# NDLOHGRP/pyReCoDe

Hardware: AMD Instinct MI355X
Metric: frames/sec + GB/s in, 4096x4096 uint16 @1% sparsity, 1/2/4/8 GPU (higher is better)
Workload: dtype u16; 1 GPU; 4096x4096 uint16, 1.00% sparsity, L1 + LZ4 frame, source_bit_depth 16, batch 64 frames/GPU/step, 256-frame stack/GPU in HBM; parallelism=dp1 (contiguous frame blocks per rank; single process: no collective), gather_every=0, gathers_issued_in_all=0, launch=single process, collective_ranks=1

## Files before the change

pyrecode_amd/csrc/rc_api.hip:

```cpp
#include "rc_host.h"
#include "rc_deflate_model.h"

thread_local std::string g_last_error;
WorkerPool *g_pool = new WorkerPool;
Util g_utils[RC_MAX_DEV];
thread_local Util *t_util = nullptr;


struct rc_ctx {
    int device = 0;
    hipStream_t own_stream = nullptr, stream = nullptr;
    uint32_t nx = 0, ny = 0, depth = 0, level = 0, op_mode = 0, scheme = 0, clevel = 0, max_batch = 0;
    uint32_t emit = rc::EMIT_RAW;
    rc::Scratch sets[2];
    int cur = 0;
    int last = 0;
    const rc::Scratch &geo() const { return sets[0]; }
    const rc::Scratch &recent() const { return sets[last]; }
    DevMem dmem, model_mem[2];
    PinMem hmem;
    hipStream_t pstream = nullptr;
    hipStream_t pstream_b = nullptr;
    hipStream_t last_ps = nullptr;
    bool two_chains = false;
    hipEvent_t ev_red[2] = {}, ev_post[2] = {}, ev_in[2] = {};
    bool post_pending[2] = {false, false};
    bool pipelined = false;
    bool thr_set = false;
    bool keep_bitmap = true;
    uint32_t src_bytes = 2;
    uint32_t *thr32 = nullptr;
    uint32_t last_n = 0;
    DevBuf d_frames, d_out, d_dark;
    uint64_t *d_rec_off = nullptr;
    uint32_t *d_md = nullptr;
    void *d_ztab = nullptr;
    rc::ValueStage values = rc::VALUES_NONE;
    bool values_on = false;
    bool modelled = false, model_ready = false;
    rc::ZstdModel *d_model = nullptr, *h_model = nullptr;
    rc::ZstdSample *d_sample = nullptr, *h_sample = nullptr;
    rc::DeflateModel *d_dzm = nullptr, *h_dzm = nullptr;
    uint32_t *d_dzhist = nullptr, *h_dzhist = nullptr;
    uint32_t l2_sum = 0;
    rc::u32x2 *d_l2_node[2] = {};
    uint16_t *d_l2_base[2] = {};
    rc::BatchStatus *h_status = nullptr;
    rc::BatchStatus *d_first_err = nullptr;
    uint32_t batch_seq = 0;
    const uint8_t *prev_out = nullptr, *prev_rec = nullptr, *prev_md = nullptr;
    uint64_t prev_out_cap = 0;
    uint32_t prev_n = 0;
    hipEvent_t ev[5] = {};
    float stage_ms[5] = {};
    bool profiling = false;
    uint32_t prof_every = 1, prof_phase = 0;
    bool profile_all = getenv("RC_PROFILE_ALL_STAGES") != nullptr;
    struct PipeSlot {
        uint8_t *d_in = nullptr;
        uint8_t *d_out = nullptr;
        uint64_t *d_rec = nullptr, *h_rec = nullptr;
        uint32_t *d_md = nullptr, *h_md = nullptr;
        rc::BatchStatus *h_stat = nullptr;
        hipEvent_t ev_h2d = nullptr, ev_done = nullptr, ev_fetch = nullptr, ev_val = nullptr;
        uint32_t *d_val = nullptr, *h_val = nullptr;
        bool has_val = false;
        uint32_t n = 0;
        bool zero_copy = false;
        enum State { FREE, SUBMITTED, RESULT_TAKEN, FETCHING } state = FREE;
    } pipe[RC_PIPE_SLOTS];
    hipStream_t copy_stream = nullptr, d2h_stream = nullptr;
    uint32_t val_gap = 0, val_x0 = 0, val_y0 = 0, val_w = 0, val_h = 0;
    std::vector<hipEvent_t> prof_ev;
    size_t prof_used = 0;
    double prof_sum_ms[5] = {};
    uint64_t prof_batches = 0;
};

RC_EXPORT int rc_abi_version(void) { return RC_ABI_VERSION; }

RC_EXPORT const char *rc_strerror(int status)
{
    switch (status) {
    case RC_OK: return "ok";
    case RC_ERR_BAD_ARG: return "bad argument";
    case RC_ERR_OUT_TOO_SMALL: return "output buffer too small";
    case RC_ERR_DEVICE: return "GPU / HIP error";
    case RC_ERR_UNSUPPORTED: return "not implemented on device";
    case RC_ERR_RECORD_TOO_LARGE: return "Buffer size smaller than compressed data size";
    case RC_ERR_CORRUPT: return "corrupt input stream";
    case RC_ERR_WORKSPACE: return "out of device memory for the ctx's workspace";
    default: return "unknown status";
    }
}
RC_EXPORT const char *rc_last_error(void) { return g_last_error.c_str(); }

RC_EXPORT int rc_device_count(int *count)
{
    if (!count) return fail(RC_ERR_BAD_ARG, "count is NULL");
    int n = 0;
    if (hipGetDeviceCount(&n) != hipSuccess) {
        (void)hipGetLastError();
        n = 0;
    }
    *count = n;
    return RC_OK;
}
RC_EXPORT int rc_scheme_on_device(uint32_t scheme)
{
    return (scheme == RC_SCHEME_LZ4 || scheme == RC_SCHEME_ZSTD || scheme == RC_SCHEME_BLOSC_LZ4 || scheme == RC_SCHEME_ZLIB_DEVICE) ? 1 : 0;
}

static int alloc_set(rc_ctx *c, rc::Scratch &sc, DevMem &model_mem)
{
    using namespace rc;
    DevMem &m = c->dmem;
    const uint64_t B = c->max_batch, T = sc.ntiles;
    RC_ALLOC(m, sc.bitmap, B * sc.nb_stride + 64);
    RC_ALLOC(m, sc.tile_cnt, B * T * 4);
    RC_ALLOC(m, sc.tile_off, B * T * 4);
    RC_ALLOC(m, sc.tile_next, B * T * 4);
    RC_ALLOC(m, sc.frame_nnz, B * 4);
    RC_ALLOC(m, sc.frame_cbytes, B * 4);
    RC_ALLOC(m, sc.scan_part, B * ((T + 255) / 256) * 32);
    RC_ALLOC(m, sc.status, sizeof(BatchStatus));
    if (c->level != 3) RC_ALLOC(m, sc.pix_slots, B * T * TILE_PX * 2 + 64);
    if (c->emit != EMIT_RAW) {
        if (c->level == 1) {
            sc.comb = c->emit == EMIT_ZSTD ? COMB_AT_BLK_SLOT : COMB_BEHIND_BLOCK;
            sc.blk_stride = 1536;
        }
        RC_ALLOC(m, sc.blk_slots, B * T * (uint64_t)sc.blk_stride + 256);
        RC_ALLOC(m, sc.blk_size, B * T * 4);
        RC_ALLOC(m, sc.blk_off, B * T * 4);
        if (c->emit == EMIT_DEFLATE) {
            RC_ALLOC(m, sc.blk_aux, B * T * 4);
            RC_ALLOC(m, sc.zl_acc, B * 32);
            HIP_TRY(hipMemset(sc.zl_acc, 0, B * 32));
        }
    }
    if (c->values != VALUES_NONE) {
        const ValueGeom g = value_geom(c->values);
        sc.pixraw_stride = ((sc.N * 2 + 15) & ~15ull) + 32;
        sc.nchunk_max = (uint32_t)((sc.N * 2 + g.chunk - 1) / g.chunk) + 1;
        RC_ALLOC(model_mem, sc.pixraw, B * sc.pixraw_stride + 64);
        RC_ALLOC(model_mem, sc.pix_chunks, B * (uint64_t)sc.nchunk_max * g.slot + 64);
        if (c->values == VALUES_DEFLATE_HUFF) RC_ALLOC(model_mem, sc.chunk_aux, B * (uint64_t)(sc.nchunk_max + 1) * 8);
        RC_ALLOC(model_mem, sc.chunk_size, B * (uint64_t)sc.nchunk_max * 4);
        RC_ALLOC(model_mem, sc.chunk_off, B * (uint64_t)sc.nchunk_max * 4);
        RC_ALLOC(model_mem, sc.frame_pbytes, B * 4);
        HIP_TRY(hipMemset(sc.frame_pbytes, 0, B * 4));
    }
    HIP_TRY(hipMemset(sc.frame_nnz, 0, B * 4));
    HIP_TRY(hipMemset(sc.frame_cbytes, 0, B * 4));
    HIP_TRY(hipMemset(sc.status, 0, sizeof(BatchStatus)));
    return RC_OK;
}

static void free_value_stage(rc_ctx *c)
{
    c->values = rc::VALUES_NONE;
    c->values_on = false;
    for (int k = 0; k < 2; ++k) {
        rc::Scratch &set = c->sets[k];
        c->model_mem[k].release_all();
        set.pixraw = nullptr; set.pix_chunks = nullptr; set.chunk_aux = nullptr; set.chunk_size = nullptr; set.chunk_off = nullptr;
        set.frame_pbytes = nullptr; set.pixraw_stride = 0; set.nchunk_max = 0;
    }
}

static int ctx_alloc(rc_ctx *c)
{
    using namespace rc;
    const uint64_t B = c->max_batch;
    RC_ON_DEVICE(c->device);
    HIP_TRY(hipStreamCreateWithFlags(&c->own_stream, hipStreamNonBlocking));
    HIP_TRY(hipStreamCreateWithFlags(&c->pstream, hipStreamNonBlocking));
    {
        int lo = 0, hi = 0;
        HIP_TRY(hipDeviceGetStreamPriorityRange(&lo, &hi));
        HIP_TRY(hipStreamCreateWithPriority(&c->pstream_b, hipStreamNonBlocking, hi));
    }
    c->last_ps = c->pstream;
    c->stream = c->own_stream;
    DevMem &m = c->dmem;
    int r;
    RC_ALLOC(m, c->sets[0].thr, c->geo().N * 2);
    RC_ALLOC(m, c->d_first_err, sizeof(BatchStatus));
    HIP_TRY(hipMemset(c->d_first_err, 0, sizeof(BatchStatus)));
    c->sets[0].first_err = c->d_first_err;
    c->sets[1] = c->sets[0];
    for (int k = 0; k < 2; ++k)
        if ((r = alloc_set(c, c->sets[k], c->model_mem[k])) != RC_OK) return r;
    c->two_chains = false;
    if (c->level == 2) {
        const uint64_t ids = (uint64_t)c->geo().ntiles * rc::TILE_PX;
        RC_ALLOC(m, c->d_l2_node[0], B * ids * 8);
        HIP_TRY(hipMemset(c->d_l2_node[0], 0, B * ids * 8));
        RC_ALLOC(m, c->d_l2_base[0], B * (uint64_t)c->geo().ntiles * 64 * 2);
        for (int i = 0; i < 2; ++i) {
            Scratch &set = c->sets[i];
            set.l2_node = c->d_l2_node[0]; set.l2_ids_per_frame = ids; set.l2_base = c->d_l2_base[0];
        }
    }
    if (c->emit == EMIT_ZSTD) {
        if ((r = zstd_encoder_tables(m, c->d_ztab)) != RC_OK) return r;
        c->modelled = c->clevel != 0;
        if (c->modelled) {
            RC_ALLOC(m, c->d_model, sizeof(ZstdModel));
            RC_ALLOC(m, c->d_sample, sizeof(ZstdSample));
            RC_ALLOC(c->hmem, c->h_model, sizeof(ZstdModel));
            RC_ALLOC(c->hmem, c->h_sample, sizeof(ZstdSample));
        }
    }
    if (c->values == VALUES_DEFLATE_HUFF) {
        RC_ALLOC(m, c->d_dzm, sizeof(DeflateModel));
        RC_ALLOC(m, c->d_dzhist, 256 * 4);
        RC_ALLOC(c->hmem, c->h_dzm, sizeof(DeflateModel));
        RC_ALLOC(c->hmem, c->h_dzhist, 256 * 4);
    }
    RC_ALLOC(m, c->d_rec_off, (B + 1) * 8);
    RC_ALLOC(m, c->d_md, B * 3 * 4);
    RC_ALLOC(c->hmem, c->h_status, 2 * sizeof(BatchStatus));
    for (auto &e : c->ev) HIP_TRY(hipEventCreate(&e));
    for (auto &e : c->ev_red) HIP_TRY(hipEventCreateWithFlags(&e, hipEventDisableTiming));
    for (auto &e : c->ev_post) HIP_TRY(hipEventCreateWithFlags(&e, hipEventDisableTiming));
    for (auto &e : c->ev_in) HIP_TRY(hipEventCreateWithFlags(&e, hipEventDisableTiming));
    return RC_OK;
}

RC_EXPORT rc_ctx *rc_ctx_create(uint32_t nx, uint32_t ny, uint32_t src_bit_depth, uint32_t reduction_level,
                                uint32_t op_mode, uint32_t scheme, uint32_t clevel, int device_id, uint32_t max_batch,
                                int *status)
{
    int dummy;
    if (!status) status = &dummy;
    *status = RC_OK;
    if (nx == 0 || ny == 0 || max_batch == 0 || max_batch > 65535u || op_mode > 1) {
        *status = fail(RC_ERR_BAD_ARG, "nx, ny, max_batch must be > 0, max_batch <= 65535 and op_mode 0 or 1");
        return nullptr;
    }
    if ((uint64_t)nx * ny >= (1ull << 32)) {
        *status = fail(RC_ERR_BAD_ARG, "nx*ny must be < 2^32");
        return nullptr;
    }
    if ((uint64_t)nx * ny * 2 >= (1ull << 32)) {
        *status = fail(RC_ERR_UNSUPPORTED, "a raw frame of 4 GiB or more (nx*ny*bytes_per_pixel >= 2^32) does not fit the format's u32 size fields");
        return nullptr;
    }
    if (reduction_level < 1 || reduction_level > 3) {
        *status = fail(RC_ERR_UNSUPPORTED, "reduction_level 4 (centroiding) is not implemented on device");
        return nullptr;
    }
    if (reduction_level == 2 && nx > 65535u) {
        *status = fail(RC_ERR_UNSUPPORTED, "reduction_level 2 needs nx <= 65535");
        return nullptr;
    }
    if (src_bit_depth < 1 || src_bit_depth > 32) {
        *status = fail(RC_ERR_UNSUPPORTED, "source_bit_depth must be 1..32 (uint8 / uint16 / uint32 source frames)");
        return nullptr;
    }
    int ndev = 0;
    if (hipGetDeviceCount(&ndev) != hipSuccess || device_id < 0 || device_id >= ndev) {
        (void)hipGetLastError();
        *status = fail(RC_ERR_DEVICE, "no such HIP device (this library has no CPU path)");
        return nullptr;
    }
    rc_ctx *c = new (std::nothrow) rc_ctx();
    if (!c) {
        *status = fail(RC_ERR_DEVICE, "out of host memory");
        return nullptr;
    }
    c->device = device_id;
    c->nx = nx; c->ny = ny; c->depth = src_bit_depth; c->level = reduction_level; c->op_mode = op_mode;
    c->scheme = scheme; c->clevel = clevel; c->max_batch = max_batch;
    c->emit = (op_mode == 1 && rc_scheme_on_device(scheme)) ? scheme : rc::EMIT_RAW;
    c->values = rc::value_stage_of(c->emit, clevel, reduction_level);
    rc::Scratch &sc = c->sets[0];
    sc.N = (uint64_t)nx * ny;
    sc.ntiles = (uint32_t)((sc.N + rc::TILE_PX - 1) / rc::TILE_PX);
    sc.nb = (sc.N + 7) / 8;
    sc.nb_stride = (uint64_t)sc.ntiles * rc::TILE_BM;
    sc.max_batch = max_batch;
    sc.guarded_loads = getenv("RC_REDUCE_GUARDED_LOADS") != nullptr;
    int rcode = ctx_alloc(c);
    if (rcode != RC_OK) {
        *status = rcode;
        std::string keep = g_last_error;
        rc_ctx_destroy(c);
        g_last_error = keep;
        return nullptr;
    }
    return c;
}

RC_EXPORT int rc_ctx_destroy(rc_ctx *c)
{
    if (!c) return RC_OK;
    DeviceGuard dev_guard_;
    (void)dev_guard_.enter(c->device);
    for (hipStream_t st : {c->stream, c->pstream, c->pstream_b, c->own_stream, c->copy_stream, c->d2h_stream})
        if (st) (void)hipStreamSynchronize(st);
    c->dmem.release_all();
    for (DevMem &m : c->model_mem) m.release_all();
    c->hmem.release_all();
    for (auto &p : c->pipe)
        for (hipEvent_t e : {p.ev_h2d, p.ev_done, p.ev_fetch, p.ev_val})
            if (e) (void)hipEventDestroy(e);
    for (hipEvent_t e : {c->ev_red[0], c->ev_red[1], c->ev_post[0], c->ev_post[1], c->ev_in[0], c->ev_in[1]})
        if (e) (void)hipEventDestroy(e);
    for (auto &e : c->ev)
        if (e) (void)hipEventDestroy(e);
    for (auto &e : c->prof_ev) (void)hipEventDestroy(e);
    for (hipStream_t st : {c->copy_stream, c->d2h_stream, c->pstream, c->pstream_b, c->own_stream})
        if (st) (void)hipStreamDestroy(st);
    delete c;
    return RC_OK;
}

RC_EXPORT int rc_ctx_set_stream(rc_ctx *c, void *hip_stream)
{
    if (!c) return fail(RC_ERR_BAD_ARG, "ctx is NULL");
    c->stream = hip_stream ? reinterpret_cast<hipStream_t>(hip_stream) : c->own_stream;
    return RC_OK;
}

RC_EXPORT int rc_set_threshold(rc_ctx *c, const void *thr)
{
    if (!c || !thr) return fail(RC_ERR_BAD_ARG, "ctx / thr is NULL");
    if (c->depth > 16 && c->src_bytes != 4) return fail(RC_ERR_BAD_ARG, "src_bit_depth > 16 means uint32 sources: rc_ctx_set_source_bytes(ctx, 4) first");
    RC_ON_DEVICE(c->device);
    HIP_TRY(hipMemcpyAsync(c->src_bytes == 4 ? (void *)c->thr32 : (void *)c->geo().thr, thr, c->geo().N * (c->src_bytes == 4 ? 4 : 2),
                           is_device_ptr(thr) ? hipMemcpyDeviceToDevice : hipMemcpyHostToDevice,
                           c->stream));
    HIP_TRY(hipStreamSynchronize(c->stream));
    c->thr_set = true;
    return RC_OK;
}

RC_EXPORT int rc_set_dark(rc_ctx *c, const void *dark, int64_t epsilon)
{
    if (!c || !dark) return fail(RC_ERR_BAD_ARG, "ctx / dark is NULL");
    RC_ON_DEVICE(c->device);
    const void *src = dark;
    const uint64_t bytes = c->geo().N * c->src_bytes;
    if (!is_device_ptr(dark)) {
        int r = c->d_dark.ensure(c->dmem, bytes);
        if (r != RC_OK) return r;
        HIP_TRY(hipMemcpyAsync(c->d_dark.p, dark, bytes, hipMemcpyHostToDevice, c->stream));
        src = c->d_dark.p;
    }
    if (c->depth > 16 && c->src_bytes != 4) return fail(RC_ERR_BAD_ARG, "src_bit_depth > 16 means uint32 sources: rc_ctx_set_source_bytes(ctx, 4) first");
    if (c->src_bytes == 4) rc::launch_threshold32(static_cast<const uint32_t *>(src), epsilon, c->geo().N, c->thr32, c->stream);
    else rc::launch_threshold(src, epsilon, c->geo().N, c->geo().thr, c->stream, c->src_bytes);
    HIP_TRY(hipGetLastError());
    HIP_TRY(hipStreamSynchronize(c->stream));
    c->thr_set = true;
    return RC_OK;
}

RC_EXPORT int rc_ctx_set_source_bytes(rc_ctx *c, uint32_t bytes_per_pixel)
{
    if (!c) return fail(RC_ERR_BAD_ARG, "ctx is NULL");
    if (bytes_per_pixel != 1 && bytes_per_pixel != 2 && bytes_per_pixel != 4) return fail(RC_ERR_BAD_ARG, "rc_ctx_set_source_bytes: 1 (uint8), 2 (uint16) or 4 (uint32)");
    if (bytes_per_pixel == 1 && c->depth > 8) return fail(RC_ERR_BAD_ARG, "rc_ctx_set_source_bytes: uint8 sources need src_bit_depth <= 8");
    if (bytes_per_pixel == 2 && c->depth > 16) return fail(RC_ERR_BAD_ARG, "rc_ctx_set_source_bytes: uint16 sources need src_bit_depth <= 16");
    if (c->batch_seq || c->thr_set) return fail(RC_ERR_BAD_ARG, "rc_ctx_set_source_bytes: call before rc_set_dark / rc_set_threshold and the first batch");
    if (c->geo().N * bytes_per_pixel >= (1ull << 32))
        return fail(RC_ERR_UNSUPPORTED, "rc_ctx_set_source_bytes: a raw frame of 4 GiB or more (nx*ny*bytes_per_pixel >= 2^32) does not fit the format's u32 size fields");
    if (bytes_per_pixel == 4) {
        if (c->depth <= 16) return fail(RC_ERR_BAD_ARG, "rc_ctx_set_source_bytes: uint32 sources are what source_bit_depth > 16 means (misc.py:41-49)");
        if (c->level == 2) return fail(RC_ERR_UNSUPPORTED, "rc_ctx_set_source_bytes: reduction level 2 is not implemented for uint32 sources");
        if (c->emit == rc::EMIT_DEFLATE) return fail(RC_ERR_UNSUPPORTED, "rc_ctx_set_source_bytes: the device DEFLATE encoder is not implemented for uint32 sources (use RC_SCHEME_ZLIB: the host's zlib)");
        RC_ON_DEVICE(c->device);
        uint32_t *thr32 = nullptr;
        uint16_t *slots[2] = {nullptr, nullptr};
        bool ok = c->dmem.try_alloc(thr32, c->geo().N * 4) == hipSuccess;
        for (int k = 0; ok && k < 2 && c->level != 3; ++k)
            ok = c->dmem.try_alloc(slots[k], (uint64_t)c->max_batch * c->geo().ntiles * rc::TILE_PX * 4 + 64) == hipSuccess;
        if (!ok) {
            (void)hipGetLastError();
            c->dmem.free_one(thr32);
            for (uint16_t *&p : slots) c->dmem.free_one(p);
            return fail(RC_ERR_DEVICE, "rc_ctx_set_source_bytes: out of device memory for the uint32 threshold / residual slots");
        }
        if (c->depth % 8 == 0) c->depth = 32;
        c->modelled = false;
        free_value_stage(c);
        c->thr32 = thr32;
        for (int k = 0; k < 2; ++k) {
            rc::Scratch *set = &c->sets[k];
            set->pix_slot_bytes = rc::TILE_PX * 4;
            set->comb = rc::COMB_OFF;
            if (c->level != 3) {
                c->dmem.free_one(set->pix_slots);
                set->pix_slots = slots[k];
            }
        }
    }
    c->src_bytes = bytes_per_pixel;
    return RC_OK;
}
RC_EXPORT uint32_t rc_ctx_source_bytes(const rc_ctx *c) { return c ? c->src_bytes : 0; }

RC_EXPORT uint64_t rc_out_capacity(const rc_ctx *c, uint32_t n) { return c ? (uint64_t)n * c->geo().N * c->src_bytes : 0; }

RC_EXPORT uint32_t rc_md_fields(const rc_ctx *c)
{
    if (!c) return 0;
    const bool comp = c->emit != rc::EMIT_RAW;
    if (c->level != 3) return comp ? 3 : 1;
    return comp ? 1 : 0;
}

static int fit_value_model(rc_ctx *c, const void *frames_dev, uint32_t n)
{
    using namespace rc;
    const bool dz = c->values == VALUES_DEFLATE_HUFF;
    hipStream_t s = c->stream;
    const Scratch &sc = c->sets[c->cur];
    const uint32_t ns = n < 2 ? n : 2;
    void *d_sample = dz ? (void *)c->d_dzhist : c->d_sample, *h_sample = dz ? (void *)c->h_dzhist : c->h_sample;
    void *d_model = dz ? (void *)c->d_dzm : c->d_model, *h_model = dz ? (void *)c->h_dzm : c->h_model;
    const size_t sample_bytes = dz ? 256 * 4 : sizeof(ZstdSample), model_bytes = dz ? sizeof(DeflateModel) : sizeof(ZstdModel);
    for (int k = 0; k < 2; ++k)
        if (c->post_pending[k]) HIP_TRY(hipStreamWaitEvent(s, c->ev_post[k], 0));
    HIP_TRY(hipMemsetAsync(d_sample, 0, sample_bytes, s));
    if (dz) {
        launch_reduce(sc, frames_dev, ns, 1u, CODEC_DEFLATE, true, c->depth, s, nullptr, c->src_bytes);
        launch_scans(sc, ns, true, true, s);
        RecordParams rp;
        rp.level = 1u; rp.emit = c->emit; rp.depth = c->depth; rp.first_frame_id = 0; rp.packed_slots = 1u;
        rp.frame_bytes = c->geo().N * c->src_bytes;
        rp.pix_mode = PIX_MODE_FLAT;
        launch_assemble(sc, rp, ns, nullptr, nullptr, c->batch_seq, s);
        launch_pd_hist(sc, ns, c->depth, c->d_dzhist, s);
    } else {
        launch_reduce(sc, frames_dev, ns, c->level == 3 ? 3u : 1u, CODEC_ZSTD_FAST, true, c->depth, s, nullptr, c->src_bytes);
        launch_zstd_sample(sc, ns, c->level == 1, c->depth, c->d_sample, s);
    }
    HIP_TRY(hipGetLastError());
    HIP_TRY(hipMemcpyAsync(h_sample, d_sample, sample_bytes, hipMemcpyDeviceToHost, s));
    HIP_TRY(hipStreamSynchronize(s));
    if (dz) {
        dm_build_model(c->h_dzhist, c->h_dzm);
        c->values_on = c->h_dzm->usable != 0;
    } else {
        zstd_model_from_sample(c->h_sample, c->h_model, c->clevel == 1 ? 50u : (c->clevel == 2 ? 20u : 0u));
        if (c->values == VALUES_NONE || !zm_code_pays(c->h_sample->pix, c->h_model->pix_code)) c->h_model->valid &= ~ZM_PIX_CODE;
        c->values_on = (c->h_model->valid & ZM_PIX_CODE) != 0;
    }
    HIP_TRY(hipMemcpyAsync(d_model, h_model, model_bytes, hipMemcpyHostToDevice, s));
    HIP_TRY(hipStreamSynchronize(s));
    for (Scratch &set : c->sets) {
        if (dz) { set.dz_model = c->d_dzm; continue; }
        const ZstdModel &M = *c->h_model;
        set.zm_model = c->d_model;
        set.zm_lit_code = c->d_model->lit_code;
        set.zm_valid = M.valid;
        set.zm_budget = zm_block_budget(M, BLK_SLOT);
        set.zm_seq_bits = (M.valid & ZM_SEQ_TABLES) ? M.seq.ll_log + M.seq.ml_log : 12u;
    }
    c->model_ready = true;
    return RC_OK;
}

static uint32_t fused_codec(uint32_t emit, uint32_t clevel, bool modelled, uint32_t src_bytes)
{
    using namespace rc;
    switch (emit) {
    case EMIT_ZSTD: return modelled && src_bytes != 4 ? CODEC_ZSTD_MODELLED : CODEC_ZSTD_FAST;
    case EMIT_LZ4: return clevel != 0 ? CODEC_LZ4_EVENTS : CODEC_LZ4_RUNS;
    case EMIT_BLOSC: return CODEC_BLOSC;
    case EMIT_DEFLATE: return CODEC_DEFLATE;
    default: return CODEC_NONE;
    }
}

static int enqueue_batch(rc_ctx *c, const void *frames_dev, uint32_t n, uint32_t first_frame_id, uint8_t *out_dev,
                         uint64_t out_cap, uint64_t *rec_off_dev, uint32_t *md_dev, bool timed)
{
    using namespace rc;
    hipStream_t s = c->stream;
    if ((c->modelled || c->values == VALUES_DEFLATE_HUFF) && !c->model_ready) {
        int r = fit_value_model(c, frames_dev, n);
        if (r != RC_OK) return r;
    }
    RecordParams rp;
    rp.level = c->level == 3 ? 3u : 1u;
    rp.emit = c->emit; rp.depth = c->depth; rp.first_frame_id = first_frame_id;
    rp.packed_slots = 1u;
    rp.frame_bytes = c->geo().N * c->src_bytes;
    hipEvent_t *ev = nullptr;
    if (timed) ev = c->ev;
    else if (c->profiling && (c->prof_phase++ % c->prof_every) == 0) {
        if (c->prof_used + 5 > c->prof_ev.size()) {
            for (int i = 0; i < 5; ++i) {
                hipEvent_t e;
                HIP_TRY(hipEventCreate(&e));
                c->prof_ev.push_back(e);
            }
        }
        ev = c->prof_ev.data() + c->prof_used;
        c->prof_used += 5;
    }
    const int k = c->cur;
    c->cur ^= 1;
    c->last = k;
    const rc::Scratch &sc = c->sets[k];
    const bool two = c->pipelined && c->two_chains;
    hipStream_t ps = two && k == 1 ? c->pstream_b : c->pstream;
    c->last_ps = ps;
    if (c->post_pending[k]) HIP_TRY(hipStreamWaitEvent(s, c->ev_post[k], 0));
    if (ev) HIP_TRY(hipEventRecord(ev[0], s));
    const bool fitted_seq = c->modelled && (c->h_model->valid & ZM_SEQ_TABLES);
    hipStream_t tail = nullptr;
    if (sc.N % TILE_PX) {
        HIP_TRY(hipEventRecord(c->ev_in[k], s));
        HIP_TRY(hipStreamWaitEvent(ps, c->ev_in[k], 0));
        tail = ps;
    }
    const uint32_t codec = fused_codec(c->emit, c->clevel, c->modelled, c->src_bytes);
    const bool keep_maps = c->keep_bitmap || c->emit == EMIT_RAW;
    if (c->src_bytes == 4)
        launch_reduce32(sc, static_cast<const uint32_t *>(frames_dev), c->thr32, n, c->level, c->depth, s, codec, keep_maps);
    else
        launch_reduce(sc, frames_dev, n, c->level, codec, keep_maps, c->depth, s, tail, c->src_bytes);
    const bool all_ev = ev && (timed || c->profile_all);
    hipEvent_t red = ev ? ev[1] : c->ev_red[k];
    HIP_TRY(hipEventRecord(red, s));
    HIP_TRY(hipStreamWaitEvent(ps, red, 0));
    if (c->level == 2) launch_l2(sc, n, c->nx, c->l2_sum, c->depth, ps);
    const bool lits_only = c->modelled && (c->h_model->valid & ZM_LITS_ONLY);
    if (c->emit == EMIT_ZSTD && !lits_only) launch_zstd_fse(sc, n, fitted_seq ? (const void *)&c->d_model->seq : c->d_ztab, fitted_seq, ps);
    if (all_ev) HIP_TRY(hipEventRecord(ev[2], ps));
    launch_scans(sc, n, c->level != 3, c->emit != EMIT_RAW, ps);
    if (all_ev) HIP_TRY(hipEventRecord(ev[3], ps));
    if (c->values_on) {
        rp.pix_mode = PIX_MODE_FLAT;
        launch_assemble(sc, rp, n, out_dev, rec_off_dev, c->batch_seq, ps);
        launch_values_encode(c->values, sc, n, c->depth, ps);
        launch_values_scan(c->values, sc, n, c->depth, ps);
        rp.pix_mode = PIX_MODE_SKIP;
    }
    if (two && c->post_pending[k ^ 1]) {
        auto overlap = [](const uint8_t *a, uint64_t an, const uint8_t *b, uint64_t bn) { return a && b && a < b + bn && b < a + an; };
        const uint8_t *rec8 = reinterpret_cast<const uint8_t *>(rec_off_dev), *md8 = reinterpret_cast<const uint8_t *>(md_dev);
        if (overlap(out_dev, out_cap, c->prev_out, c->prev_out_cap) || overlap(rec8, (uint64_t)(n + 1) * 8, c->prev_rec, (uint64_t)(c->prev_n + 1) * 8) ||
            overlap(md8, (uint64_t)n * 12, c->prev_md, (uint64_t)c->prev_n * 12))
            HIP_TRY(hipStreamWaitEvent(ps, c->ev_post[k ^ 1], 0));
    }
    c->prev_out = out_dev; c->prev_out_cap = out_cap; c->prev_n = n;
    c->prev_rec = reinterpret_cast<const uint8_t *>(rec_off_dev); c->prev_md = reinterpret_cast<const uint8_t *>(md_dev);
    launch_layout(sc, rp, n, out_cap, rec_off_dev, md_dev, ps);
    launch_assemble(sc, rp, n, out_dev, rec_off_dev, c->batch_seq, ps);
    ++c->batch_seq;
    if (c->values_on) launch_values_gather(c->values, sc, n, c->depth, 16, out_dev, rec_off_dev, ps);
    if (ev) HIP_TRY(hipEventRecord(ev[4], ps));
    if (two && c->post_pending[k ^ 1]) HIP_TRY(hipStreamWaitEvent(ps, c->ev_post[k ^ 1], 0));
    HIP_TRY(hipEventRecord(c->ev_post[k], ps));
    c->post_pending[k] = true;
    if (!c->pipelined) HIP_TRY(hipStreamWaitEvent(s, c->ev_post[k], 0));
    HIP_TRY(hipGetLastError());
    c->last_n = n;
    return RC_OK;
}

static int check_batch_args(rc_ctx *c, const void *frames, uint32_t n, const void *out, const void *rec, const void *md)
{
    if (!c || !frames || !out || !rec || !md) return fail(RC_ERR_BAD_ARG, "NULL argument");
    if (n == 0 || n > c->max_batch) return fail(RC_ERR_BAD_ARG, "n must be in 1..max_batch");
    if (!c->thr_set) return fail(RC_ERR_BAD_ARG, "threshold not set (rc_set_threshold / rc_set_dark)");
    return RC_OK;
}

RC_EXPORT int rc_reduce_compress_batch_async(rc_ctx *c, const void *frames_dev, uint32_t n, uint32_t first_frame_id,
                                             uint8_t *out_dev, uint64_t out_cap, uint64_t *rec_offsets_dev, uint32_t *md_dev)
{
    int r = check_batch_args(c, frames_dev, n, out_dev, rec_offsets_dev, md_dev);
    if (r != RC_OK) return r;
    RC_ON_DEVICE(c->device);
    return enqueue_batch(c, frames_dev, n, first_frame_id, out_dev, out_cap, rec_offsets_dev, md_dev, false);
}

static void l2_second_chain(rc_ctx *c)
{
    if (c->level != 2 || c->two_chains) return;
    const uint64_t B = c->max_batch, ids = (uint64_t)c->geo().ntiles * rc::TILE_PX;
    if (!c->d_l2_node[1]) {
        bool ok = c->dmem.try_alloc(c->d_l2_node[1], B * ids * 8) == hipSuccess && hipMemset(c->d_l2_node[1], 0, B * ids * 8) == hipSuccess &&
                  c->dmem.try_alloc(c->d_l2_base[1], B * (uint64_t)c->geo().ntiles * 64 * 2) == hipSuccess && hipDeviceSynchronize() == hipSuccess;
        if (!ok) {
            (void)hipGetLastError();
            c->dmem.free_one(c->d_l2_node[1]);
            c->dmem.free_one(c->d_l2_base[1]);
            return;
        }
    }
    c->sets[1].l2_node = c->d_l2_node[1];
    c->sets[1].l2_base = c->d_l2_base[1];
    c->two_chains = true;
}

RC_EXPORT int rc_ctx_set_pipelined(rc_ctx *c, int on)
{
    if (!c) return fail(RC_ERR_BAD_ARG, "ctx is NULL");
    RC_ON_DEVICE(c->device);
    HIP_TRY(hipStreamSynchronize(c->pstream));
    HIP_TRY(hipStreamSynchronize(c->pstream_b));
    if (on) l2_second_chain(c);
    c->pipelined = on != 0;
    return RC_OK;
}
RC_EXPORT int rc_ctx_wait_results(rc_ctx *c, void *hip_stream)
{
    if (!c) return fail(RC_ERR_BAD_ARG, "ctx is NULL");
    RC_ON_DEVICE(c->device);
    if (c->post_pending[c->last])
        HIP_TRY(hipStreamWaitEvent(hip_stream ? reinterpret_cast<hipStream_t>(hip_stream) : c->stream, c->ev_post[c->last], 0));
    return RC_OK;
}

RC_EXPORT int rc_ctx_sync(rc_ctx *c)
{
    if (!c) return fail(RC_ERR_BAD_ARG, "ctx is NULL");
    RC_ON_DEVICE(c->device);
    HIP_TRY(hipStreamSynchronize(c->pstream_b));
    HIP_TRY(hipMemcpyAsync(&c->h_status[0], c->recent().status, sizeof(rc::BatchStatus), hipMemcpyDeviceToHost, c->pstream));
    HIP_TRY(hipMemcpyAsync(&c->h_status[1], c->d_first_err, sizeof(rc::BatchStatus), hipMemcpyDeviceToHost, c->pstream));
    HIP_TRY(hipMemsetAsync(c->d_first_err, 0, sizeof(rc::BatchStatus), c->pstream));
    HIP_TRY(hipStreamSynchronize(c->pstream));
    HIP_TRY(hipStreamSynchronize(c->stream));
    const uint32_t n_batches = c->batch_seq;
    c->batch_seq = 0;
    for (size_t b = 0; b + 5 <= c->prof_used; b += 5) {
        float ms;
        if (!c->profile_all) {
            if (hipEventElapsedTime(&ms, c->prof_ev[b], c->prof_ev[b + 1]) == hipSuccess) c->prof_sum_ms[0] += ms;
        } else
        for (int i = 0; i < 4; ++i)
            if (hipEventElapsedTime(&ms, c->prof_ev[b + i], c->prof_ev[b + i + 1]) == hipSuccess) c->prof_sum_ms[i] += ms;
        if (hipEventElapsedTime(&ms, c->prof_ev[b], c->prof_ev[b + 4]) == hipSuccess) c->prof_sum_ms[4] += ms;
        ++c->prof_batches;
    }
    c->prof_used = 0;
    if (c->h_status[1].total != 0) c->h_status[1] = rc::first_err_decode(c->h_status[1].total);
    if (c->h_status[1].code != 0) {
        char msg[160];
        if (n_batches > 1)
            snprintf(msg, sizeof msg, "%s (frame %u of batch %llu of the %u enqueued since the last sync)", rc_strerror(c->h_status[1].code),
                     c->h_status[1].frame, (unsigned long long)c->h_status[1].total, n_batches);
        else
            snprintf(msg, sizeof msg, "%s (frame %u of the batch)", rc_strerror(c->h_status[1].code), c->h_status[1].frame);
        return fail(c->h_status[1].code, msg);
    }
    return RC_OK;
}

RC_EXPORT int rc_reduce_compress_batch(rc_ctx *c, const void *frames, uint32_t n, uint32_t first_frame_id, uint8_t *out,
                                       uint64_t out_cap, uint64_t *rec_offsets, uint32_t *md)
{
    int r = check_batch_args(c, frames, n, out, rec_offsets, md);
    if (r != RC_OK) return r;
    RC_ON_DEVICE(c->device);
    const uint64_t frame_bytes = c->geo().N * c->src_bytes;
    const void *fdev = frames;
    if (!is_device_ptr(frames)) {
        r = c->d_frames.ensure(c->dmem, (uint64_t)n * frame_bytes);
        if (r != RC_OK) return r;
        HIP_TRY(hipMemcpyAsync(c->d_frames.p, frames, (uint64_t)n * frame_bytes, hipMemcpyHostToDevice, c->stream));
        fdev = c->d_frames.p;
    }
    uint8_t *odev = out;
    uint64_t cap = out_cap;
    const bool out_host = !is_device_ptr(out);
    if (out_host) {
        const uint64_t worst = (uint64_t)n * frame_bytes;
        cap = out_cap < worst ? out_cap : worst;
        r = c->d_out.ensure(c->dmem, cap);
        if (r != RC_OK) return r;
        odev = c->d_out.p;
    }
    r = enqueue_batch(c, fdev, n, first_frame_id, odev, cap, c->d_rec_off, c->d_md, true);
    if (r != RC_OK) return r;
    r = rc_ctx_sync(c);
    for (int i = 0; i < 4; ++i) (void)hipEventElapsedTime(&c->stage_ms[i], c->ev[i], c->ev[i + 1]);
    (void)hipEventElapsedTime(&c->stage_ms[4], c->ev[0], c->ev[4]);
    if (r != RC_OK) return r;
    int r2 = copy_out(rec_offsets, c->d_rec_off, (uint64_t)(n + 1) * 8, c->stream);
    if (r2 == RC_OK) r2 = copy_out(md, c->d_md, (uint64_t)n * 12, c->stream);
    if (r2 == RC_OK && out_host) r2 = copy_out(out, c->d_out.p, c->h_status->total, c->stream);
    if (r2 != RC_OK) return r2;
    HIP_TRY(hipStreamSynchronize(c->stream));
    return RC_OK;
}

RC_EXPORT void *rc_host_alloc(uint64_t bytes)
{
    void *p = nullptr;
    if (hipHostMalloc(&p, bytes ? bytes : 16, hipHostMallocDefault) != hipSuccess) {
        (void)hipGetLastError();
        fail(RC_ERR_DEVICE, "hipHostMalloc failed");
        return nullptr;
    }
    return p;
}
RC_EXPORT int rc_host_free(void *p)
{
    if (p) HIP_TRY(hipHostFree(p));
    return RC_OK;
}
RC_EXPORT int rc_host_register(void *p, uint64_t bytes)
{
    if (!p || !bytes) return fail(RC_ERR_BAD_ARG, "NULL / zero argument");
    HIP_TRY(hipHostRegister(p, bytes, hipHostRegisterDefault));
    return RC_OK;
}
RC_EXPORT int rc_host_unregister(void *p)
{
    if (p) HIP_TRY(hipHostUnregister(p));
    return RC_OK;
}

static int pipe_slot_init(rc_ctx *c, rc_ctx::PipeSlot &p)
{
    const uint64_t B = c->max_batch;
    if (!c->copy_stream) HIP_TRY(hipStreamCreateWithFlags(&c->copy_stream, hipStreamNonBlocking));
    if (!c->d2h_stream) HIP_TRY(hipStreamCreateWithFlags(&c->d2h_stream, hipStreamNonBlocking));
    RC_ALLOC(c->dmem, p.d_in, B * c->geo().N * c->src_bytes + 64);
    RC_ALLOC(c->dmem, p.d_out, rc_out_capacity(c, (uint32_t)B) + 64);
    RC_ALLOC(c->dmem, p.d_rec, (B + 1) * 8);
    RC_ALLOC(c->dmem, p.d_md, B * 12);
    RC_ALLOC(c->hmem, p.h_rec, (B + 1) * 8);
    RC_ALLOC(c->hmem, p.h_md, B * 12);
    RC_ALLOC(c->hmem, p.h_stat, sizeof(rc::BatchStatus));
    HIP_TRY(hipEventCreateWithFlags(&p.ev_h2d, hipEventDisableTiming));
    HIP_TRY(hipEventCreateWithFlags(&p.ev_done, hipEventDisableTiming));
    HIP_TRY(hipEventCreateWithFlags(&p.ev_fetch, hipEventDisableTiming));
    HIP_TRY(hipEventCreateWithFlags(&p.ev_val, hipEventDisableTiming));
    RC_ALLOC(c->dmem, p.d_val, B * 4 + 64);
    RC_ALLOC(c->hmem, p.h_val, B * 4 + 64);
    return RC_OK;
}

RC_EXPORT int rc_ctx_set_validation(rc_ctx *c, uint32_t gap, uint32_t x0, uint32_t y0, uint32_t w, uint32_t h)
{
    if (!c) return fail(RC_ERR_BAD_ARG, "ctx is NULL");
    if (gap && (w == 0 || h == 0 || w > 128 || h > 128 || (uint64_t)x0 + w > c->nx || (uint64_t)y0 + h > c->ny))
        return fail(RC_ERR_BAD_ARG, "rc_ctx_set_validation: the region must lie inside the frame and hold at most 128 x 128 pixels");
    c->val_gap = gap; c->val_x0 = x0; c->val_y0 = y0; c->val_w = w; c->val_h = h;
    return RC_OK;
}

RC_EXPORT int rc_pipe_validation(rc_ctx *c, uint32_t slot, uint32_t *counts)
{
    if (!c || slot >= RC_PIPE_SLOTS || !counts) return fail(RC_ERR_BAD_ARG, "NULL argument / slot out of range");
    rc_ctx::PipeSlot &p = c->pipe[slot];
    if (p.state != p.SUBMITTED && p.state != p.RESULT_TAKEN) return fail(RC_ERR_BAD_ARG, "nothing submitted on this slot");
    if (!p.has_val) { for (uint32_t i = 0; i < p.n; ++i) counts[i] = 0xFFFFFFFFu; return RC_OK; }
    HIP_TRY(hipEventSynchronize(p.ev_val));
    memcpy(counts, p.h_val, (uint64_t)p.n * 4);
    return RC_OK;
}

RC_EXPORT int rc_pipe_submit(rc_ctx *c, uint32_t slot, const void *frames_host, uint32_t n, uint32_t first_frame_id)
{
    if (!c || !frames_host || slot >= RC_PIPE_SLOTS) return fail(RC_ERR_BAD_ARG, "NULL argument / slot out of range");
    if (n == 0 || n > c->max_batch) return fail(RC_ERR_BAD_ARG, "n must be in 1..max_batch");
    if (!c->thr_set) return fail(RC_ERR_BAD_ARG, "threshold not set (rc_set_threshold / rc_set_dark)");
    RC_ON_DEVICE(c->device);
    rc_ctx::PipeSlot &p = c->pipe[slot];
    if (p.state != p.FREE) return fail(RC_ERR_BAD_ARG, "slot is still in use (result / fetch_wait not called)");
    if (!p.d_in) {
        int r = pipe_slot_init(c, p);
        if (r != RC_OK) return r;
    }
    if (!c->pipelined) {
        HIP_TRY(hipStreamSynchronize(c->pstream));
        HIP_TRY(hipStreamSynchronize(c->pstream_b));
        l2_second_chain(c);
        c->pipelined = true;
    }
    const void *fdev = nullptr;
    hipPointerAttribute_t a;
    if (hipPointerGetAttributes(&a, frames_host) == hipSuccess) {
        if (a.type == hipMemoryTypeHost && a.devicePointer) fdev = a.devicePointer;
    } else (void)hipGetLastError();
    p.zero_copy = fdev != nullptr;
    if (!fdev) {
        HIP_TRY(hipMemcpyAsync(p.d_in, frames_host, (uint64_t)n * c->geo().N * c->src_bytes, hipMemcpyHostToDevice, c->copy_stream));
        HIP_TRY(hipEventRecord(p.ev_h2d, c->copy_stream));
        HIP_TRY(hipStreamWaitEvent(c->stream, p.ev_h2d, 0));
        fdev = p.d_in;
    }
    int r = enqueue_batch(c, fdev, n, first_frame_id, p.d_out, rc_out_capacity(c, c->max_batch), p.d_rec, p.d_md, false);
    if (r != RC_OK) return r;
    p.has_val = c->val_gap != 0;
    if (p.has_val) {
        rc::launch_roi_components(fdev, c->src_bytes == 4 ? (const void *)c->thr32 : (const void *)c->geo().thr, c->geo().N, c->nx, n, first_frame_id, c->val_gap, c->val_x0, c->val_y0, c->val_w, c->val_h, p.d_val, c->stream, c->src_bytes);
        HIP_TRY(hipGetLastError());
        HIP_TRY(hipMemcpyAsync(p.h_val, p.d_val, (uint64_t)n * 4, hipMemcpyDeviceToHost, c->stream));
        HIP_TRY(hipEventRecord(p.ev_val, c->stream));
    }
    if (p.zero_copy) HIP_TRY(hipEventRecord(p.ev_h2d, c->stream));
    hipStream_t ps = c->last_ps;
    HIP_TRY(hipMemcpyAsync(p.h_rec, p.d_rec, (uint64_t)(n + 1) * 8, hipMemcpyDeviceToHost, ps));
    HIP_TRY(hipMemcpyAsync(p.h_md, p.d_md, (uint64_t)n * 12, hipMemcpyDeviceToHost, ps));
    HIP_TRY(hipMemcpyAsync(p.h_stat, c->recent().status, sizeof(rc::BatchStatus), hipMemcpyDeviceToHost, ps));
    HIP_TRY(hipEventRecord(p.ev_done, ps));
    p.n = n;
    p.state = p.SUBMITTED;
    return RC_OK;
}

RC_EXPORT int rc_pipe_input_done(rc_ctx *c, uint32_t slot)
{
    if (!c || slot >= RC_PIPE_SLOTS) return fail(RC_ERR_BAD_ARG, "NULL argument / slot out of range");
    if (c->pipe[slot].state == rc_ctx::PipeSlot::FREE) return RC_OK;
    HIP_TRY(hipEventSynchronize(c->pipe[slot].ev_h2d));
    return RC_OK;
}

RC_EXPORT int rc_pipe_result(rc_ctx *c, uint32_t slot, uint64_t *rec_offsets, uint32_t *md, uint64_t *total)
{
    if (!c || slot >= RC_PIPE_SLOTS || !rec_offsets || !md || !total) return fail(RC_ERR_BAD_ARG, "NULL argument / slot out of range");
    rc_ctx::PipeSlot &p = c->pipe[slot];
    if (p.state != p.SUBMITTED) return fail(RC_ERR_BAD_ARG, "nothing submitted on this slot");
    HIP_TRY(hipEventSynchronize(p.ev_done));
    p.state = p.RESULT_TAKEN;
    if (p.h_stat->code != 0) {
        char msg[128];
        snprintf(msg, sizeof msg, "%s (frame %u of the batch)", rc_strerror(p.h_stat->code), p.h_stat->frame);
        p.state = p.FREE;
        return fail(p.h_stat->code, msg);
    }
    memcpy(rec_offsets, p.h_rec, (uint64_t)(p.n + 1) * 8);
    memcpy(md, p.h_md, (uint64_t)p.n * 12);
    *total = p.h_stat->total;
    return RC_OK;
}

RC_EXPORT int rc_pipe_fetch(rc_ctx *c, uint32_t slot, uint8_t *dst_host, uint64_t bytes)
{
    if (!c || slot >= RC_PIPE_SLOTS || (!dst_host && bytes)) return fail(RC_ERR_BAD_ARG, "NULL argument / slot out of range");
    rc_ctx::PipeSlot &p = c->pipe[slot];
    if (p.state != p.RESULT_TAKEN) return fail(RC_ERR_BAD_ARG, "rc_pipe_result has not been called for this slot");
    if (bytes > p.h_stat->total) return fail(RC_ERR_BAD_ARG, "more bytes than the batch's records hold");
    RC_ON_DEVICE(c->device);
    if (bytes) HIP_TRY(hipMemcpyAsync(dst_host, p.d_out, bytes, hipMemcpyDeviceToHost, c->d2h_stream));
    HIP_TRY(hipEventRecord(p.ev_fetch, c->d2h_stream));
    p.state = p.FETCHING;
    return RC_OK;
}

RC_EXPORT int rc_pipe_fetch_wait(rc_ctx *c, uint32_t slot)
{
    if (!c || slot >= RC_PIPE_SLOTS) return fail(RC_ERR_BAD_ARG, "NULL argument / slot out of range");
    rc_ctx::PipeSlot &p = c->pipe[slot];
    if (p.state == p.RESULT_TAKEN) { p.state = p.FREE; return RC_OK; }
    if (p.state != p.FETCHING) return fail(RC_ERR_BAD_ARG, "rc_pipe_fetch has not been called for this slot");
    HIP_TRY(hipEventSynchronize(p.ev_fetch));
    p.state = p.FREE;
    return RC_OK;
}

RC_EXPORT int rc_ctx_refit_model(rc_ctx *c)
{
    if (!c) return fail(RC_ERR_BAD_ARG, "ctx is NULL");
    c->model_ready = false;
    return RC_OK;
}

RC_EXPORT int rc_get_binary_map(rc_ctx *c, uint32_t i, uint8_t *bitmap_out)
{
    if (!c || !bitmap_out) return fail(RC_ERR_BAD_ARG, "NULL argument");
    if (i >= c->last_n) return fail(RC_ERR_BAD_ARG, "frame index outside the most recent batch");
    if (!c->keep_bitmap && c->emit != rc::EMIT_RAW && c->level != 2) return fail(RC_ERR_BAD_ARG, "binary maps are not kept (rc_ctx_keep_binary_maps(ctx, 0))");
    RC_ON_DEVICE(c->device);
    int r = copy_out(bitmap_out, c->recent().bitmap + (uint64_t)i * c->geo().nb_stride, c->geo().nb, c->stream);
    if (r != RC_OK) return r;
    HIP_TRY(hipStreamSynchronize(c->stream));
    return RC_OK;
}

RC_EXPORT int rc_ctx_set_profiling(rc_ctx *c, int on)
{
    if (!c) return fail(RC_ERR_BAD_ARG, "ctx is NULL");
    c->profiling = on != 0;
    c->prof_every = on > 1 ? (uint32_t)on : 1u;
    c->prof_phase = 0;
    for (double &v : c->prof_sum_ms) v = 0;
    c->prof_batches = 0;
    return RC_OK;
}
RC_EXPORT int rc_ctx_get_profile(rc_ctx *c, double sum_ms[5], uint64_t *batches)
{
    if (!c || !sum_ms || !batches) return fail(RC_ERR_BAD_ARG, "NULL argument");
    memcpy(sum_ms, c->prof_sum_ms, sizeof c->prof_sum_ms);
    *batches = c->prof_batches;
    return RC_OK;
}

RC_EXPORT int rc_ctx_set_l2_statistics(rc_ctx *c, uint32_t l2_statistics)
{
    if (!c || l2_statistics > 2) return fail(RC_ERR_BAD_ARG, "l2_statistics must be 0, 1 (max) or 2 (sum)");
    c->l2_sum = l2_statistics == 2 ? 1u : 0u;
    return RC_OK;
}

RC_EXPORT int rc_ctx_keep_binary_maps(rc_ctx *c, int on)
{
    if (!c) return fail(RC_ERR_BAD_ARG, "ctx is NULL");
    c->keep_bitmap = on != 0;
    return RC_OK;
}

RC_EXPORT int rc_get_stage_ms(rc_ctx *c, float ms[5])
{
    if (!c || !ms) return fail(RC_ERR_BAD_ARG, "NULL argument");
    memcpy(ms, c->stage_ms, sizeof c->stage_ms);
    return RC_OK;
}

RC_EXPORT int64_t rc_unpack_frame_sparse(uint32_t nx, uint32_t ny, uint32_t bit_depth, const uint8_t *bitmap,
                                         const uint8_t *pixvals, uint64_t pixvals_bytes, uint64_t *out,
                                         uint64_t out_cap_triplets, uint32_t reduction_level)
{
    if (!bitmap || nx == 0 || ny == 0 || (!out && out_cap_triplets)) return fail(RC_ERR_BAD_ARG, "NULL / zero argument");
    if (reduction_level == 1 && (bit_depth == 0 || bit_depth > 64)) return fail(RC_ERR_BAD_ARG, "bit_depth must be 1..64");
    if (reduction_level == 1 && !pixvals && pixvals_bytes) return fail(RC_ERR_BAD_ARG, "pixvals is NULL");
    UtilScope util_scope;
    int r = util_scope.enter();
    if (r != RC_OK) return r;
    Util &u = g_util;
    const uint64_t N = (uint64_t)nx * ny, nb = (N + 7) / 8, nb8 = (nb + 7) / 8;
    const uint32_t nblk = (uint32_t)((nb8 + rc::WG - 1) / rc::WG);
    const uint8_t *d_bm = nullptr, *d_px = nullptr;
    r = stage_in(bitmap, nb, u.a, d_bm, nb8 * 8 - nb + 8);
    if (r != RC_OK) return r;
    if (reduction_level == 1 && pixvals_bytes) {
        r = stage_in(pixvals, pixvals_bytes, u.b, d_px);
        if (r != RC_OK) return r;
    }
    r = u.w.ensure(u.dmem, (uint64_t)nblk * 8 + 16);
    if (r != RC_OK) return r;
    uint32_t *blk_cnt = u.w.as<uint32_t>(), *blk_off = blk_cnt + nblk;
    uint64_t *nnz_dev = reinterpret_cast<uint64_t *>(blk_cnt + 2 * (uint64_t)nblk);
    rc::launch_expand_count(d_bm, nb8, N, blk_cnt, blk_off, nnz_dev, u.stream);
    HIP_TRY(hipMemcpyAsync(u.h_scalar, nnz_dev, 8, hipMemcpyDeviceToHost, u.stream));
    HIP_TRY(hipStreamSynchronize(u.stream));
    const uint64_t nnz = *u.h_scalar;
    if (!out) return (int64_t)nnz;
    if (nnz > out_cap_triplets) return fail(RC_ERR_OUT_TOO_SMALL, "out holds fewer triplets than the bitmap has set bits");
    if (reduction_level == 1 && (nnz * bit_depth + 7) / 8 > pixvals_bytes)
        return fail(RC_ERR_CORRUPT, "pixvals shorter than popcount(bitmap) * bit_depth bits");
    if (nnz == 0) return 0;
    StagedOut so;
    if ((r = so.begin(out, nnz * 24)) != RC_OK) return r;
    rc::launch_expand_emit(d_bm, nb8, N, nx, blk_off, d_px, pixvals_bytes, bit_depth, reduction_level, nnz, so.as<uint64_t>(), u.stream);
    HIP_TRY(hipGetLastError());
    if ((r = so.finish(out, nnz * 24)) != RC_OK) return r;
    return (int64_t)nnz;
}

RC_EXPORT int rc_bit_pack(const uint16_t *pixvals, uint64_t n, uint32_t bit_depth, uint8_t *out, uint64_t out_n)
{
    if (!out || (!pixvals && n)) return fail(RC_ERR_BAD_ARG, "NULL argument");
    if (bit_depth == 0 || bit_depth > 32) return fail(RC_ERR_BAD_ARG, "bit_depth must be 1..32");
    if (out_n != (n * bit_depth + 7) / 8) return fail(RC_ERR_BAD_ARG, "out_n must be ceil(n*bit_depth/8)");
    if (out_n == 0) return RC_OK;
    UtilScope util_scope;
    int r = util_scope.enter();
    if (r != RC_OK) return r;
    Util &u = g_util;
    const uint16_t *d_in = nullptr;
    r = stage_in(pixvals, n * 2, u.a, d_in);
    if (r != RC_OK) return r;
    StagedOut so;
    if ((r = so.begin(out, out_n)) != RC_OK) return r;
    rc::launch_bit_pack(d_in, n, bit_depth, so.as<uint8_t>(), out_n, u.stream);
    HIP_TRY(hipGetLastError());
    return so.finish(out, out_n);
}

RC_EXPORT int rc_bit_unpack(const uint8_t *packed, uint64_t packed_bytes, uint64_t n, uint32_t bit_depth, uint64_t *out)
{
    if (!out || (!packed && packed_bytes)) return fail(RC_ERR_BAD_ARG, "NULL argument");
    if (bit_depth == 0 || bit_depth > 64) return fail(RC_ERR_BAD_ARG, "bit_depth must be 1..64");
    if ((n * bit_depth + 7) / 8 > packed_bytes) return fail(RC_ERR_CORRUPT, "packed shorter than n * bit_depth bits");
    if (n == 0) return RC_OK;
    UtilScope util_scope;
    int r = util_scope.enter();
    if (r != RC_OK) return r;
    Util &u = g_util;
    const uint8_t *d_in = nullptr;
    r = stage_in(packed, packed_bytes, u.a, d_in);
    if (r != RC_OK) return r;
    StagedOut so;
    if ((r = so.begin(out, n * 8)) != RC_OK) return r;
    rc::launch_bit_unpack(d_in, packed_bytes, n, bit_depth, so.as<uint64_t>(), u.stream);
    HIP_TRY(hipGetLastError());
    return so.finish(out, n * 8);
}

RC_EXPORT int rc_synth_dark(int device_id, uint32_t seed, uint64_t n_pixels, uint16_t *dark_dev)
{
    if (!dark_dev) return fail(RC_ERR_BAD_ARG, "NULL argument");
    RC_ON_DEVICE(device_id);
    rc::launch_synth_dark(seed, n_pixels, dark_dev, nullptr);
    HIP_TRY(hipGetLastError());
    HIP_TRY(hipDeviceSynchronize());
    return RC_OK;
}
RC_EXPORT int rc_synth_frames_clustered(int device_id, uint32_t seed, uint32_t first_frame, uint32_t n_frames, uint32_t nx, uint32_t ny,
                                        uint32_t seed_ppm, const uint16_t *dark_dev, uint16_t *frames_dev)
{
    if (!dark_dev || !frames_dev || n_frames == 0 || nx == 0 || ny == 0) return fail(RC_ERR_BAD_ARG, "NULL / zero argument");
    if ((uint64_t)nx * ny > 0xFFFFFFFFull) return fail(RC_ERR_BAD_ARG, "rc_synth_frames_clustered: nx * ny must fit 32 bits");
    RC_ON_DEVICE(device_id);
    rc::launch_synth_frames_clustered(seed, first_frame, n_frames, nx, ny, seed_ppm, dark_dev, frames_dev, nullptr);
    HIP_TRY(hipGetLastError());
    HIP_TRY(hipDeviceSynchronize());
    return RC_OK;
}
RC_EXPORT int rc_synth_frames(int device_id, uint32_t seed, uint32_t first_frame, uint32_t n_frames, uint64_t n_pixels,
                              uint32_t sparsity_ppm, const uint16_t *dark_dev, uint16_t *frames_dev)
{
    if (!dark_dev || !frames_dev || n_frames == 0) return fail(RC_ERR_BAD_ARG, "NULL / zero argument");
    RC_ON_DEVICE(device_id);
    rc::launch_synth_frames(seed, first_frame, n_frames, n_pixels, sparsity_ppm, dark_dev, frames_dev, nullptr);
    HIP_TRY(hipGetLastError());
    HIP_TRY(hipDeviceSynchronize());
    return RC_OK;
}
```

pyrecode_amd/csrc/rc_gather.hip:

```cpp
#include <cstdlib>

#include "rc_launch.h"
#include "rc_record.h"
#include "rc_deflate_block.h"

namespace rc {

struct GatherArgs {
    const uint8_t *blk_slots, *bitmap;
    const uint16_t *pix_slots;
    const uint32_t *blk_size, *blk_off, *tile_cnt, *tile_off, *tile_next, *frame_nnz, *frame_cbytes, *frame_pbytes;
    const uint32_t *blk_aux;
    uint32_t *zl_acc;
    uint8_t *pixraw;
    BatchStatus *status, *first_err;
    uint64_t nb, nb_stride, pixraw_stride;
    uint32_t ntiles, blk_stride, pix_slot_bytes, comb;
};

typedef u32x4 u32x4_u __attribute__((aligned(1)));
typedef u32x2 u32x2_u __attribute__((aligned(1)));
typedef uint32_t u32_u __attribute__((aligned(1)));
typedef uint16_t u16_u __attribute__((aligned(1)));

__device__ __forceinline__ uint32_t lane_get(uint32_t v, uint32_t src_lane)
{
    return (uint32_t)__builtin_amdgcn_ds_bpermute((int)(4u * src_lane), (int)v);
}

template <bool BITS>
__device__ __forceinline__ u32x4 shift_piece(const u32x4 &x, uint32_t e, uint32_t sh)
{
    u32x4 y = x;
    if (BITS) {
        y[0] = __builtin_amdgcn_alignbit(x[1], x[0], sh); y[1] = __builtin_amdgcn_alignbit(x[2], x[1], sh);
        y[2] = __builtin_amdgcn_alignbit(x[3], x[2], sh); y[3] = __builtin_amdgcn_alignbit(e, x[3], sh);
    }
    return y;
}
__device__ __forceinline__ void put_piece(uint8_t *p, const u32x4 &y, uint32_t valid)
{
    if (valid >= 16) { *reinterpret_cast<u32x4_u *>(p) = y; return; }
    uint32_t a0 = y[0], a1 = y[1];
    if (valid & 8u) { *reinterpret_cast<u32x2_u *>(p) = u32x2{a0, a1}; p += 8; a0 = y[2]; a1 = y[3]; }
    if (valid & 4u) { *reinterpret_cast<u32_u *>(p) = a0; p += 4; a0 = a1; }
    if (valid & 2u) { *reinterpret_cast<u16_u *>(p) = (uint16_t)a0; p += 2; a0 >>= 16; }
    if (valid & 1u) *p = (uint8_t)a0;
}

struct AdlerAcc { uint32_t A, W; };
__device__ __forceinline__ void adler_piece(AdlerAcc &acc, const u32x4 &y, uint32_t valid, uint32_t sp)
{
    uint32_t a = 0, q = 0;
#pragma unroll
    for (int k = 0; k < 4; ++k) {
        const uint32_t nb = valid > 4u * k ? min(valid - 4u * k, 4u) : 0u;
        const uint32_t v = y[k] & (nb >= 4u ? 0xFFFFFFFFu : ((1u << (8u * nb)) - 1u));
        a = __builtin_amdgcn_sad_u8(v, 0u, a);
        q = __builtin_amdgcn_udot4(v, 0x03020100u + 0x04040404u * (uint32_t)k, q, false);
    }
    acc.A += a;
    acc.W = (acc.W + (sp % ADLER_P) * a + q) % ADLER_P;
}
__device__ __forceinline__ void adler_byte(AdlerAcc &acc, uint32_t byte, uint32_t sp)
{
    acc.A += byte;
    acc.W = (acc.W + (sp % ADLER_P) * byte) % ADLER_P;
}

struct ResidGeom { uint32_t b_lo, n, ps0, avail; };
__device__ __forceinline__ ResidGeom resid_geom(uint32_t coff, uint32_t cnt, uint32_t d)
{
    const uint64_t dbit = (uint64_t)coff * d;
    const uint32_t nbits = cnt * d;
    const uint64_t b_lo = (dbit + 7) >> 3, b_hi = (dbit + nbits + 7) >> 3;
    ResidGeom g{(uint32_t)b_lo, (uint32_t)(b_hi - b_lo), (uint32_t)(8 * b_lo - dbit), (uint32_t)((dbit + nbits) & 7u)};
    if (g.avail && g.n) --g.n;
    else g.avail = 0;
    return g;
}

constexpr int GATHER_U = 4, GATHER_UB = 3;
constexpr int GATHER_WPE = 8;
template <bool BITS, int U, bool ADLER>
__global__ __launch_bounds__(64) __attribute__((amdgpu_waves_per_eu(GATHER_WPE))) void k_gather(GatherArgs sc, RecordParams rp, uint8_t *__restrict__ out, const uint64_t *__restrict__ rec_off,
                                               uint32_t lz4f_hdr_bitmap, uint32_t lz4f_hdr_pix, uint32_t batch_seq, uint32_t gpf, uint32_t nitems, uint32_t tpi)
{
    if (sc.status->code != 0) {
        if (blockIdx.x == 0 && threadIdx.x == 0 && sc.first_err)
            atomicMax(reinterpret_cast<unsigned long long *>(&sc.first_err->total), first_err_key(batch_seq, sc.status->code, sc.status->frame));
        return;
    }
    const uint32_t lane = (uint32_t)lane_id();
    const bool flat = rp.pix_mode == PIX_MODE_FLAT, skip_pix = rp.pix_mode == PIX_MODE_SKIP;
    const bool pixp = rp.level == 1 && rp.packed_slots && !skip_pix;
    const bool plain_pos = rp.emit == EMIT_RAW || flat;
    const uint32_t d = rp.depth;
    const FrameFmt ff = frame_fmt(rp.emit);
    const uint32_t bhdr = bitmap_hdr(ff, rp.emit, sc.ntiles);
    const uint8_t *pix_base = reinterpret_cast<const uint8_t *>(sc.pix_slots);
    for (uint32_t item = blockIdx.x; item < nitems; item += gridDim.x) {
        const uint32_t f = item / gpf, g = item - f * gpf, t0 = tpi * g, t = t0 + lane;
        const bool have = lane < tpi && t < sc.ntiles;
        const uint64_t frow = (uint64_t)f * sc.ntiles;
        uint8_t *rec = flat ? sc.pixraw + (uint64_t)f * sc.pixraw_stride : out + rec_off[f];
        const uint32_t nnz = rp.level == 1 ? sc.frame_nnz[f] : 0;
        const uint32_t npk = rp.level == 1 ? packed_bytes(nnz, d) : 0;
        uint64_t bitmap_pos = 0, pix_pos = 0;
        uint32_t cb = 0;
        if (!flat) {
            if (rp.emit == EMIT_RAW) { bitmap_pos = rp.level == 1 ? 8 : 4; pix_pos = bitmap_pos + sc.nb; }
            else { cb = bhdr + sc.frame_cbytes[f] + ff.end; bitmap_pos = rp.level == 1 ? 16 : 8; pix_pos = bitmap_pos + cb; }
        }
        if (g == 0 && lane == 0 && !flat) record_fixed_fields(sc, rp, f, rec, bitmap_pos, pix_pos, cb, npk, ff, skip_pix, lz4f_hdr_bitmap, lz4f_hdr_pix);
        uint8_t *pdst = rec + pix_pos;

        uint32_t word = 0, bsz = 0, bdst = 0, cnt = 0, rn = 0, rdst = 0, rs = 0xFFFFFFFFu, ps0 = 0, flags = 0, blo = 0;
        AdlerAcc ad{0u, 0u};
        if (have && rp.emit != EMIT_RAW && (!flat || (sc.comb == COMB_BEHIND_BLOCK && pixp))) word = sc.blk_size[frow + t];
        if (have && !flat) {
            if (rp.emit == EMIT_RAW) {
                const uint64_t b0 = (uint64_t)t * TILE_BM;
                bsz = (uint32_t)min((uint64_t)TILE_BM, sc.nb - b0);
                bdst = (uint32_t)(bitmap_pos + b0);
            } else {
                bsz = word;
                const uint32_t boff = bhdr + sc.blk_off[frow + t];
                bdst = (uint32_t)bitmap_pos + boff;
                if (rp.emit == EMIT_BLOSC) store_u32_le(rec + bitmap_pos + 16 + 4 * (uint64_t)t, boff);
            }
        }
        if (have && pixp) {
            cnt = sc.tile_cnt[frow + t];
            if (cnt) {
                const ResidGeom q = resid_geom(sc.tile_off[frow + t], cnt, d);
                ps0 = q.ps0;
                if (ADLER) blo = q.b_lo;
                if (sc.comb) {
                    const uint32_t ro16 = sc.comb == COMB_AT_BLK_SLOT ? (uint32_t)BLK_SLOT / 16 : (word + 15) >> 4, r16 = (cnt * d + 127) >> 7;
                    if (16 * (ro16 + r16) <= sc.blk_stride) rs = 16 * ro16;
                }
                if (q.n && !plain_pos && ((uint64_t)q.b_lo >> ff.chunk_shift) != (((uint64_t)q.b_lo + q.n - 1) >> ff.chunk_shift)) flags = 1u << 31;
                else rn = q.n;
                rdst = (uint32_t)(pix_pos + (plain_pos ? (uint64_t)q.b_lo : stored_pos(ff, q.b_lo)));
            }
        }
        uint32_t ext_cnt = 0, ext_first = 0;
        if (BITS && pixp && t0 + tpi < sc.ntiles) {
            ext_cnt = sc.tile_cnt[frow + t0 + tpi];
            if (ext_cnt)
                ext_first = *reinterpret_cast<const uint32_t *>(residual_src(sc, frow + t0 + tpi, sc.comb == COMB_BEHIND_BLOCK ? sc.blk_size[frow + t0 + tpi] : 0u, ext_cnt, d));
        }
        const uint8_t *slot = rp.emit == EMIT_RAW ? sc.bitmap + (uint64_t)f * sc.nb_stride + (uint64_t)t0 * TILE_BM : sc.blk_slots + (frow + t0) * sc.blk_stride;
        const uint32_t slot_stride = rp.emit == EMIT_RAW ? (uint32_t)TILE_BM : sc.blk_stride;
        const uint8_t *rslot = pix_base + (frow + t0) * sc.pix_slot_bytes;

        const uint32_t nb16 = (bsz + 15) >> 4, tot = nb16 + ((rn + 15) >> 4);
        const uint32_t incl = wave_incl_scan(tot), cum = incl - tot, T = wave_last(incl);
        const uint32_t packed = bsz | (ps0 << 10) | (rn << 13) | flags;
        for (uint32_t i0 = 0; 64u * i0 < T; i0 += U) {
            u32x4 x[U];
            uint32_t e[U], dsto[U], meta[U];
            uint32_t spos[ADLER ? U : 1];
#pragma unroll
            for (int u = 0; u < U; ++u) {
                const uint32_t P = 64u * (i0 + u) + lane;
                uint32_t k = 0;
#pragma unroll
                for (uint32_t step = 32; step; step >>= 1) {
                    const uint32_t c = lane_get(cum, k + step);
                    if (c <= P) k += step;
                }
                const uint32_t ck = lane_get(cum, k), pk = lane_get(packed, k), bd = lane_get(bdst, k), rd = lane_get(rdst, k), rsk = lane_get(rs, k);
                const uint32_t blk = ADLER ? lane_get(blo, k) : 0u;
                const uint32_t bsz_k = pk & 1023u, ps0_k = (pk >> 10) & 7u, rn_k = (pk >> 13) & 0x7FFFu;
                const uint32_t idx = P - ck, nbk = (bsz_k + 15) >> 4;
                const bool isb = idx < nbk;
                const uint32_t j = isb ? idx : idx - nbk;
                const uint32_t left = (isb ? bsz_k : rn_k) - 16u * j;
                const bool act = P < T;
                const uint8_t *src = isb ? slot + (uint64_t)k * slot_stride + 16u * j
                                         : (rsk == 0xFFFFFFFFu ? rslot + (uint64_t)k * sc.pix_slot_bytes : slot + (uint64_t)k * slot_stride + rsk) + 16u * j;
                dsto[u] = (isb ? bd : rd) + 16u * j;
                meta[u] = act ? (min(left, 16u) | ((isb ? 0u : ps0_k) << 8)) : 0u;
                if (ADLER) spos[u] = isb ? 0xFFFFFFFFu : blk + 16u * j;
                x[u] = u32x4{0u, 0u, 0u, 0u};
                e[u] = 0;
                if (act) {
                    x[u] = *reinterpret_cast<const u32x4 *>(src);
                    if (BITS && !isb && ps0_k) e[u] = *reinterpret_cast<const uint32_t *>(src + 16);
                }
            }
#pragma unroll
            for (int u = 0; u < U; ++u)
                if (meta[u] & 0xFFu) {
                    const u32x4 y = shift_piece<BITS>(x[u], e[u], meta[u] >> 8);
                    put_piece(rec + dsto[u], y, meta[u] & 0xFFu);
                    if (ADLER && spos[u] != 0xFFFFFFFFu) adler_piece(ad, y, meta[u] & 0xFFu, spos[u]);
                }
        }
        if (pixp) {
        ResidGeom q{0u, 0u, 0u, 0u};
        if (cnt) q = resid_geom(sc.tile_off[frow + t], cnt, d);
        for (uint64_t m = __builtin_amdgcn_ballot_w64((packed >> 31) != 0); m; m &= m - 1) {
            const uint32_t k = (uint32_t)__builtin_ctzll(m);
            const uint32_t n = lane_get(q.n, k), p0 = lane_get(q.ps0, k), b0 = lane_get(q.b_lo, k), rsk = lane_get(rs, k);
            const uint32_t *s32 = reinterpret_cast<const uint32_t *>(rsk == 0xFFFFFFFFu ? rslot + (uint64_t)k * sc.pix_slot_bytes : slot + (uint64_t)k * slot_stride + rsk);
            for (uint32_t i = lane; i < n; i += 64) {
                const uint32_t qb = 8 * i + p0;
                const uint32_t v = __builtin_amdgcn_alignbit(s32[(qb >> 5) + 1], s32[qb >> 5], qb & 31u) & 0xFFu;
                pdst[stored_pos(ff, (uint64_t)b0 + i)] = (uint8_t)v;
                if (ADLER) adler_byte(ad, v, b0 + i);
            }
        }
        if (BITS) {

        const uint32_t fin_avail = q.avail, fin_q = 8 * q.n + q.ps0, fin_b = q.b_lo + q.n;
        const uint8_t *psrc = rs == 0xFFFFFFFFu ? rslot + (uint64_t)lane * sc.pix_slot_bytes : slot + (uint64_t)lane * slot_stride + rs;
        const uint32_t first = cnt ? *reinterpret_cast<const uint32_t *>(psrc) : 0u;
        uint32_t byte = 0, got = 8;
        if (fin_avail) {
            byte = (*reinterpret_cast<const u32_u *>(psrc + (fin_q >> 3)) >> (fin_q & 7u)) & ((1u << fin_avail) - 1u);
            got = fin_avail;
        }
        const uint64_t nonempty = __builtin_amdgcn_ballot_w64(cnt != 0);
        uint32_t cur = lane;
        while (__builtin_amdgcn_ballot_w64(got < 8 && cur < 64) != 0) {
            const uint64_t higher = cur >= 63 ? 0ull : nonempty & (~0ull << (cur + 1));
            const uint32_t nxt = higher ? (uint32_t)__builtin_ctzll(higher) : 64u;
            const uint32_t cc = lane_get(cnt, nxt & 63u), fd = lane_get(first, nxt & 63u);
            if (got < 8 && cur < 64) {
                const bool in = nxt < 64;
                const uint32_t c2 = in ? cc : ext_cnt, f2 = in ? fd : ext_first;
                if (in || c2) {
                    const uint32_t take = min(8u - got, c2 * d);
                    byte |= (f2 & ((1u << take) - 1u)) << got;
                    got += take;
                    cur = nxt;
                } else cur = 65;
            }
        }
        if (got < 8) {
            uint32_t tt = cur == 65 ? (t0 + tpi - 1 < sc.ntiles ? sc.tile_next[frow + t0 + tpi - 1] : sc.ntiles) : (t0 + tpi < sc.ntiles ? sc.tile_next[frow + t0 + tpi] : sc.ntiles);
            while (tt < sc.ntiles) {
                const uint32_t cc = sc.tile_cnt[frow + tt];
                const uint32_t fd = *reinterpret_cast<const uint32_t *>(residual_src(sc, frow + tt, sc.comb == COMB_BEHIND_BLOCK ? sc.blk_size[frow + tt] : 0u, cc, d));
                const uint32_t take = min(8u - got, cc * d);
                byte |= (fd & ((1u << take) - 1u)) << got;
                got += take;
                if (got >= 8) break;
                tt = sc.tile_next[frow + tt];
            }
        }
        if (fin_avail) {
            pdst[plain_pos ? (uint64_t)fin_b : stored_pos(ff, fin_b)] = (uint8_t)byte;
            if (ADLER) adler_byte(ad, byte & 0xFFu, fin_b);
        }
        }
        }
        if (ADLER && !flat) {
            const uint32_t aux = have ? sc.blk_aux[frow + t] : 0u;
            const uint32_t tA0 = wave_last(wave_incl_scan(aux & 0xFFFFu)), tW0 = wave_last(wave_incl_scan(aux >> 16));
            const uint32_t tA1 = wave_last(wave_incl_scan(ad.A % ADLER_P)), tW1 = wave_last(wave_incl_scan(ad.W));
            if (lane == 0) {
                uint32_t *acc = sc.zl_acc + 8 * (uint64_t)f;
                if (tA0 | tW0) {
                    __hip_atomic_fetch_add(&acc[0], tA0 % ADLER_P, __ATOMIC_RELAXED, __HIP_MEMORY_SCOPE_AGENT);
                    __hip_atomic_fetch_add(&acc[1], tW0 % ADLER_P, __ATOMIC_RELAXED, __HIP_MEMORY_SCOPE_AGENT);
                }
                if (tA1 | tW1) {
                    __hip_atomic_fetch_add(&acc[2], tA1 % ADLER_P, __ATOMIC_RELAXED, __HIP_MEMORY_SCOPE_AGENT);
                    __hip_atomic_fetch_add(&acc[3], tW1 % ADLER_P, __ATOMIC_RELAXED, __HIP_MEMORY_SCOPE_AGENT);
                }
            }
        }
    }
}

__global__ __launch_bounds__(64) void k_zlib_finish(GatherArgs sc, RecordParams rp, uint8_t *__restrict__ out, const uint64_t *__restrict__ rec_off, uint32_t B)
{
    const uint32_t f = blockIdx.x * 64 + threadIdx.x;
    if (f >= B || sc.status->code != 0) return;
    const FrameFmt ff = frame_fmt(rp.emit);
    const uint32_t *acc = sc.zl_acc + 8 * (uint64_t)f;
    uint8_t *rec = out + rec_off[f];
    const uint32_t cb = bitmap_hdr(ff, rp.emit, sc.ntiles) + sc.frame_cbytes[f] + ff.end, bitmap_pos = rp.level == 1 ? 16u : 8u;
    store_u32_be(rec + bitmap_pos + cb - 4, adler_from_sums(sc.nb, acc[0], acc[1]));
    if (rp.level == 1 && rp.pix_mode != PIX_MODE_SKIP) {
        const uint32_t npk = packed_bytes(sc.frame_nnz[f], rp.depth);
        store_u32_be(rec + bitmap_pos + cb + stored_size(ff, npk) - 4, adler_from_sums(npk, acc[2], acc[3]));
    }
}


void launch_gather(const Scratch &sc, const RecordParams &rp, uint32_t B, uint8_t *out, const uint64_t *rec_off, uint32_t hdr_bitmap, uint32_t hdr_pix,
                   uint32_t batch_seq, hipStream_t s)
{
    uint32_t tpi = 64;
    while (tpi > 8 && (uint64_t)B * ((sc.ntiles + tpi - 1) / tpi) < 1024) tpi >>= 1;
    const uint32_t gpf = (sc.ntiles + tpi - 1) / tpi, nitems = gpf * B, wgs = nitems;
    const GatherArgs ga{sc.blk_slots, sc.bitmap, sc.pix_slots, sc.blk_size, sc.blk_off, sc.tile_cnt, sc.tile_off, sc.tile_next, sc.frame_nnz, sc.frame_cbytes,
                        sc.frame_pbytes, sc.blk_aux, sc.zl_acc, sc.pixraw, sc.status, sc.first_err, sc.nb, sc.nb_stride, sc.pixraw_stride, sc.ntiles, sc.blk_stride, sc.pix_slot_bytes, sc.comb};
    const bool bits = rp.level == 1 && rp.depth % 8 != 0;
    if (rp.emit == EMIT_DEFLATE) {
        if (bits) hipLaunchKernelGGL((k_gather<true, GATHER_UB - 1, true>), dim3(wgs), dim3(64), 0, s, ga, rp, out, rec_off, hdr_bitmap, hdr_pix, batch_seq, gpf, nitems, tpi);
        else hipLaunchKernelGGL((k_gather<false, GATHER_U, true>), dim3(wgs), dim3(64), 0, s, ga, rp, out, rec_off, hdr_bitmap, hdr_pix, batch_seq, gpf, nitems, tpi);
        if (rp.pix_mode != PIX_MODE_FLAT) hipLaunchKernelGGL(k_zlib_finish, dim3((B + 63) / 64), dim3(64), 0, s, ga, rp, out, rec_off, B);
    } else if (bits)
        hipLaunchKernelGGL((k_gather<true, GATHER_UB, false>), dim3(wgs), dim3(64), 0, s, ga, rp, out, rec_off, hdr_bitmap, hdr_pix, batch_seq, gpf, nitems, tpi);
    else
        hipLaunchKernelGGL((k_gather<false, GATHER_U, false>), dim3(wgs), dim3(64), 0, s, ga, rp, out, rec_off, hdr_bitmap, hdr_pix, batch_seq, gpf, nitems, tpi);
}

}
```

pyrecode_amd/csrc/rc_launch.h:

```cpp
#pragma once
#include <hip/hip_runtime.h>
#include <stdint.h>

#include "../../include/recode_hip.h"
#include "rc_device.h"

namespace rc {

struct ZstdModel;
struct DeflateModel;
struct InfStream;

constexpr uint32_t COMB_OFF = 0u;
constexpr uint32_t COMB_BEHIND_BLOCK = 1u;
constexpr uint32_t COMB_AT_BLK_SLOT = 2u;

struct Scratch {
    uint64_t N = 0;
    uint32_t ntiles = 0;
    uint64_t nb = 0;
    uint64_t nb_stride = 0;
    uint32_t max_batch = 0;
    bool guarded_loads = false;
    uint16_t *thr = nullptr;
    uint8_t *bitmap = nullptr;
    uint16_t *pix_slots = nullptr;
    uint32_t pix_slot_bytes = SLOT_PX * 2;
    uint32_t *tile_cnt = nullptr;
    uint32_t *tile_off = nullptr;
    uint32_t *tile_next = nullptr;
    uint8_t *blk_slots = nullptr;
    uint32_t blk_stride = BLK_SLOT;
    uint32_t comb = COMB_OFF;
    uint32_t *blk_size = nullptr;
    uint32_t *blk_aux = nullptr;
    uint32_t *zl_acc = nullptr;
    uint32_t *blk_off = nullptr;
    uint32_t *frame_nnz = nullptr;
    uint32_t *frame_cbytes = nullptr;
    uint32_t *scan_part = nullptr;
    BatchStatus *status = nullptr;
    BatchStatus *first_err = nullptr;
    uint8_t *pixraw = nullptr;
    uint64_t pixraw_stride = 0;
    uint8_t *pix_chunks = nullptr;
    uint32_t *chunk_size = nullptr;
    uint32_t *chunk_off = nullptr;
    uint32_t *frame_pbytes = nullptr;
    uint32_t nchunk_max = 0;
    const ZstdModel *zm_model = nullptr;
    const void *zm_lit_code = nullptr;
    uint32_t zm_valid = 0, zm_budget = 0, zm_seq_bits = 12;
    u32x2 *l2_node = nullptr;
    uint64_t l2_ids_per_frame = 0;
    uint16_t *l2_base = nullptr;
    uint32_t *chunk_aux = nullptr;
    const DeflateModel *dz_model = nullptr;
};

constexpr uint32_t EMIT_RAW = 0u;
constexpr uint32_t EMIT_ZSTD = 1u;
constexpr uint32_t EMIT_LZ4 = 2u;
constexpr uint32_t EMIT_BLOSC = 8u;
constexpr uint32_t EMIT_DEFLATE = 0x100u;
static_assert(EMIT_ZSTD == RC_SCHEME_ZSTD && EMIT_LZ4 == RC_SCHEME_LZ4 && EMIT_BLOSC == RC_SCHEME_BLOSC_LZ4 && EMIT_DEFLATE == RC_SCHEME_ZLIB_DEVICE,
              "rc_ctx_create assigns emit = compression_scheme");

constexpr int CODEC_NONE = 0;
constexpr int CODEC_ZSTD_FAST = 1;
constexpr int CODEC_LZ4_RUNS = 2;
constexpr int CODEC_ZSTD_MODELLED = 3;
constexpr int CODEC_LZ4_EVENTS = 4;
constexpr int CODEC_DEFLATE = 5;
constexpr int CODEC_BLOSC = 8;

constexpr uint32_t PIX_MODE_STORED = 0u;
constexpr uint32_t PIX_MODE_FLAT = 1u;
constexpr uint32_t PIX_MODE_SKIP = 2u;

struct RecordParams {
    uint32_t level;
    uint32_t emit;
    uint32_t depth;
    uint32_t packed_slots;
    uint32_t first_frame_id;
    uint64_t frame_bytes;
    uint32_t pix_mode = PIX_MODE_STORED;
};

void launch_threshold(const void *dark, int64_t eps, uint64_t N, uint16_t *thr, hipStream_t s, uint32_t src_bytes = 2);
void launch_reduce(const Scratch &sc, const void *frames, uint32_t B, uint32_t level, uint32_t codec, bool keep_bitmap,
                   uint32_t depth, hipStream_t s, hipStream_t s_tail = nullptr, uint32_t src_bytes = 2);
void launch_threshold32(const uint32_t *dark, int64_t eps, uint64_t N, uint32_t *thr, hipStream_t s);
void launch_reduce32(const Scratch &sc, const uint32_t *frames, const uint32_t *thr32, uint32_t B, uint32_t level, uint32_t depth, hipStream_t s,
                     uint32_t codec = CODEC_NONE, bool keep_bitmap = true);
void launch_l2(const Scratch &sc, uint32_t B, uint32_t nx, uint32_t use_sum, uint32_t depth, hipStream_t s);
void launch_scans(const Scratch &sc, uint32_t B, bool with_counts, bool with_blocks, hipStream_t s);
void launch_layout(const Scratch &sc, const RecordParams &rp, uint32_t B, uint64_t out_cap, uint64_t *rec_off,
                   uint32_t *md, hipStream_t s);
void launch_assemble(const Scratch &sc, const RecordParams &rp, uint32_t B, uint8_t *out, const uint64_t *rec_off,
                     uint32_t batch_seq, hipStream_t s);
void launch_gather(const Scratch &sc, const RecordParams &rp, uint32_t B, uint8_t *out, const uint64_t *rec_off, uint32_t hdr_bitmap, uint32_t hdr_pix,
                   uint32_t batch_seq, hipStream_t s);
enum ValueStage : uint32_t {
    VALUES_NONE = 0,
    VALUES_ZSTD_HUFF,
    VALUES_DEFLATE_HUFF,
};
inline ValueStage value_stage_of(uint32_t emit, uint32_t clevel, uint32_t level)
{
    if (level == 1 && emit == EMIT_ZSTD && clevel != 0) return VALUES_ZSTD_HUFF;
    return level == 1 && emit == EMIT_DEFLATE && clevel >= 2 ? VALUES_DEFLATE_HUFF : VALUES_NONE;
}
constexpr uint32_t PIX_CHUNK = 1008, PIX_SLOT = 1024, PD_CHUNK = 1u << 15, PD_SLOT = PD_CHUNK + 32;
struct ValueGeom { uint32_t chunk, slot; };
inline ValueGeom value_geom(ValueStage kind) { return kind == VALUES_DEFLATE_HUFF ? ValueGeom{PD_CHUNK, PD_SLOT} : ValueGeom{PIX_CHUNK, PIX_SLOT}; }
void launch_values_encode(ValueStage kind, const Scratch &sc, uint32_t B, uint32_t depth, hipStream_t s);
void launch_values_scan(ValueStage kind, const Scratch &sc, uint32_t B, uint32_t depth, hipStream_t s);
void launch_values_gather(ValueStage kind, const Scratch &sc, uint32_t B, uint32_t depth, uint32_t level1_hdr, uint8_t *out, const uint64_t *rec_off,
                          hipStream_t s);
void launch_pd_hist(const Scratch &sc, uint32_t B, uint32_t depth, uint32_t *hist_dev, hipStream_t s);
struct Lz4Block { uint64_t src_off; uint32_t size; uint32_t raw; };
void launch_lz4_encode_buffer(const Scratch &sc, hipStream_t s, bool events = false);
void launch_lz4_encode_rows(const Scratch &sc, uint32_t B, hipStream_t s, bool events);
void launch_lz4f_gather(const Scratch &sc, uint32_t hdr3, uint8_t *out, hipStream_t s);
void launch_lz4_decode(const uint8_t *src, const Lz4Block *blks, uint32_t nblk, uint32_t *sizes, const uint64_t *dst_off,
                       uint8_t *dst, uint64_t cap, int linked, int *err, hipStream_t s, uint32_t max_stored = 0);
uint32_t lz4f_descriptor(uint8_t bd);
void launch_blosc_encode_blocks(const Scratch &sc, uint32_t B, hipStream_t s);
void launch_blosc_gather(const Scratch &sc, uint8_t *out, hipStream_t s);
void launch_blosc_unshuffle(const uint8_t *in, uint8_t *out, uint64_t nbytes, uint32_t blocksize, uint32_t typesize,
                            uint32_t shuffle, hipStream_t s);
void launch_zstd_encode_blocks(const Scratch &sc, uint32_t B, const void *tables_dev, hipStream_t s);
void launch_zstd_tokenize_rows(const Scratch &sc, uint32_t B, hipStream_t s);
void launch_zstd_fse(const Scratch &sc, uint32_t B, const void *tables_dev, bool fitted, hipStream_t s);
void launch_zstd_sample(const Scratch &sc, uint32_t B, bool with_pix, uint32_t depth, void *sample_dev, hipStream_t s);
size_t zstd_model_bytes();
size_t zstd_sample_bytes();
void zstd_model_from_sample(const void *sample_host, void *model_host, uint32_t speed_permille = 0);
void launch_zstd_gather(const Scratch &sc, uint8_t *out, hipStream_t s);
size_t zstd_tables_bytes();
void zstd_tables_host(void *dst);

template <class S>
__host__ __device__ inline const uint8_t *residual_src(const S &sc, uint64_t ft, uint32_t bn, uint32_t cnt, uint32_t d)
{
    if (sc.comb) {
        const uint32_t ro16 = sc.comb == COMB_AT_BLK_SLOT ? (uint32_t)BLK_SLOT / 16 : (bn + 15) >> 4, r16 = (cnt * d + 127) >> 7;
        if (16 * (ro16 + r16) <= sc.blk_stride) return sc.blk_slots + ft * sc.blk_stride + 16 * ro16;
    }
    return reinterpret_cast<const uint8_t *>(sc.pix_slots) + ft * sc.pix_slot_bytes;
}

void launch_inflate(const uint8_t *data, const InfStream *streams, uint32_t n_map, uint32_t n_val, uint32_t map_cap_max, uint32_t map_units_max,
                    uint32_t val_cap_max, uint32_t val_units_max, uint32_t *cand_pos, uint32_t *ncand, uint32_t *link, uint32_t *unit_cand,
                    uint8_t *out, int *err, hipStream_t s);

void launch_roi_components(const void *frames, const void *thr, uint64_t N, uint32_t nx, uint32_t n, uint32_t first_frame_id, uint32_t gap,
                           uint32_t x0, uint32_t y0, uint32_t w, uint32_t h, uint32_t *counts, hipStream_t s, uint32_t src_bytes = 2);

constexpr uint32_t CALIB_LDS_MAX_FRAMES = 512;
void launch_calib_stats(const uint16_t *stack, uint32_t n, uint64_t N, uint32_t n_stats, float *median, float *sdev, int32_t *range2, hipStream_t s);
void launch_calib_hist(const uint16_t *frames, uint32_t n_stats, uint64_t N, const float *median, const double *edges, uint32_t n_bins,
                       uint64_t *counts, hipStream_t s);
void launch_calib_top(const uint16_t *stack, uint32_t n, uint64_t N, const float *median, uint32_t k, float *acc, uint64_t *n_undefined, hipStream_t s);
}
```

pyrecode_amd/csrc/rc_reduce.hip:

```cpp
#include <cstddef>
#include <cstdlib>
#include <type_traits>

#include "rc_launch.h"
#include "rc_values.h"
#include "rc_pack.h"
#ifdef RC_PHASE_TIMING
__device__ unsigned long long g_phase[16];
#define RC_LZ4_PHASE 1
#endif
#include "rc_lz4_block.h"
#include "rc_zstd_wave.h"
#include "rc_deflate_block.h"

namespace rc {

#ifdef RC_PHASE_TIMING
#define RC_PHASE_BEGIN unsigned long long ph_t_ = __builtin_amdgcn_s_memtime(); unsigned long long ph_a_[8] = {};
#define RC_PHASE(i) do { const unsigned long long ph_n_ = __builtin_amdgcn_s_memtime(); ph_a_[i] = ph_n_ - ph_t_; ph_t_ = ph_n_; \
        if ((i) == 6 && lane_id() == 0 && (blockIdx.x & 63u) == 0) { for (int q_ = 0; q_ < 7; ++q_) atomicAdd(&g_phase[q_], ph_a_[q_]); atomicAdd(&g_phase[7], 1ull); } } while (0)
#else
#define RC_PHASE_BEGIN
#define RC_PHASE(i) do { } while (0)
#endif
constexpr int REDUCE_BZ = 4;

__device__ __forceinline__ uint32_t pk_sub_sat_u16(uint32_t a, uint32_t b)
{
    uint32_t r;
    asm("v_pk_sub_u16 %0, %1, %2 clamp" : "=v"(r) : "v"(a), "v"(b));
    return r;
}
__device__ __forceinline__ uint32_t pk_add_u16(uint32_t a, uint32_t b)
{
    uint32_t r;
    asm("v_pk_add_u16 %0, %1, %2" : "=v"(r) : "v"(a), "v"(b));
    return r;
}
__device__ __forceinline__ uint32_t pk_min_u16(uint32_t a, uint32_t b)
{
    uint32_t r;
    asm("v_pk_min_u16 %0, %1, %2" : "=v"(r) : "v"(a), "v"(b));
    return r;
}

__global__ void k_threshold(const uint16_t *__restrict__ dark, uint32_t eps16, uint64_t N, uint16_t *__restrict__ thr)
{
    uint64_t i = (uint64_t)blockIdx.x * blockDim.x + threadIdx.x;
    const uint64_t stride = (uint64_t)gridDim.x * blockDim.x;
    for (; i < N; i += stride) thr[i] = (uint16_t)(dark[i] + eps16);
}

__global__ void k_threshold8(const uint8_t *__restrict__ dark, uint32_t eps8, uint64_t N, uint16_t *__restrict__ thr)
{
    uint64_t i = (uint64_t)blockIdx.x * blockDim.x + threadIdx.x;
    const uint64_t stride = (uint64_t)gridDim.x * blockDim.x;
    for (; i < N; i += stride) thr[i] = (uint16_t)(uint8_t)(dark[i] + eps8);
}

void launch_threshold(const void *dark, int64_t eps, uint64_t N, uint16_t *thr, hipStream_t s, uint32_t src_bytes)
{
    uint32_t blocks = (uint32_t)((N + 255) / 256);
    if (blocks > 4096) blocks = 4096;
    if (src_bytes == 1)
        hipLaunchKernelGGL(k_threshold8, dim3(blocks), dim3(256), 0, s, static_cast<const uint8_t *>(dark), (uint32_t)((uint64_t)eps & 0xFF), N, thr);
    else
        hipLaunchKernelGGL(k_threshold, dim3(blocks), dim3(256), 0, s, static_cast<const uint16_t *>(dark), (uint32_t)((uint64_t)eps & 0xFFFF), N, thr);
}

template <int SB> struct Src;
template <> struct Src<2> { typedef uint16_t T; typedef u32x4 X; };
template <> struct Src<1> { typedef uint8_t T; typedef u32x2 X; };
__device__ __forceinline__ u32x4 widen8(const u32x2 &v)
{
    return u32x4{__builtin_amdgcn_perm(0u, v[0], 0x0C010C00u), __builtin_amdgcn_perm(0u, v[0], 0x0C030C02u),
                 __builtin_amdgcn_perm(0u, v[1], 0x0C010C00u), __builtin_amdgcn_perm(0u, v[1], 0x0C030C02u)};
}
__device__ __forceinline__ u32x4 widen8(const u32x4 &v) { return v; }

template <bool ALIGNED, bool STREAM, int SB = 2>
__device__ __forceinline__ typename Src<SB>::X load8(const typename Src<SB>::T *__restrict__ base, uint64_t px0, uint64_t N, uint32_t fill)
{
    typedef typename Src<SB>::X X;
    constexpr int PER = 4 / SB;
    if (ALIGNED || px0 + 8 <= N) {
        if (px0 < N) {
            typedef X XU __attribute__((aligned(SB)));
            const XU *p = reinterpret_cast<const XU *>(base + px0);
            return STREAM ? __builtin_nontemporal_load(p) : *p;
        }
    }
    X v;
#pragma unroll
    for (int j = 0; j < 8 / PER; ++j) {
        uint32_t w = 0;
#pragma unroll
        for (int e = 0; e < PER; ++e) {
            const uint64_t k = px0 + (uint64_t)(PER * j + e);
            const uint32_t val = (!ALIGNED && k < N) ? (uint32_t)base[k] : fill;
            w |= val << (8 * SB * e);
        }
        v[j] = w;
    }
    return v;
}

struct Pending {
    bool valid;
    uint64_t ft;
    uint32_t f;
    uint32_t cnt;
    uint32_t csize;
    uint32_t staged;
    u32x2 own;
    uint64_t cown;
    uint32_t aux;
    bool last;
    uint32_t depth;
    uint16_t *buf;
};

__device__ __forceinline__ void vm_issue_loads(u32x4 (&x)[R], const uint16_t *lane_ptr)
{
    const uint8_t *p0 = reinterpret_cast<const uint8_t *>(lane_ptr), *p1 = p0 + 4096;
    asm volatile("global_load_dwordx4 %0, %4, off nt\n\t"
                 "global_load_dwordx4 %1, %4, off offset:1024 nt\n\t"
                 "global_load_dwordx4 %2, %4, off offset:2048 nt\n\t"
                 "global_load_dwordx4 %3, %4, off offset:3072 nt"
                 : "=&v"(x[0]), "=&v"(x[1]), "=&v"(x[2]), "=&v"(x[3]) : "v"(p0) : "memory");
    asm volatile("global_load_dwordx4 %0, %4, off nt\n\t"
                 "global_load_dwordx4 %1, %4, off offset:1024 nt\n\t"
                 "global_load_dwordx4 %2, %4, off offset:2048 nt\n\t"
                 "global_load_dwordx4 %3, %4, off offset:3072 nt"
                 : "=&v"(x[4]), "=&v"(x[5]), "=&v"(x[6]), "=&v"(x[7]) : "v"(p1) : "memory");
}
__device__ __forceinline__ void vm_issue_loads(u32x2 (&x)[R], const uint8_t *lane_ptr)
{
    asm volatile("global_load_dwordx2 %0, %8, off nt\n\t"
                 "global_load_dwordx2 %1, %8, off offset:512 nt\n\t"
                 "global_load_dwordx2 %2, %8, off offset:1024 nt\n\t"
                 "global_load_dwordx2 %3, %8, off offset:1536 nt\n\t"
                 "global_load_dwordx2 %4, %8, off offset:2048 nt\n\t"
                 "global_load_dwordx2 %5, %8, off offset:2560 nt\n\t"
                 "global_load_dwordx2 %6, %8, off offset:3072 nt\n\t"
                 "global_load_dwordx2 %7, %8, off offset:3584 nt"
                 : "=&v"(x[0]), "=&v"(x[1]), "=&v"(x[2]), "=&v"(x[3]), "=&v"(x[4]), "=&v"(x[5]), "=&v"(x[6]), "=&v"(x[7]) : "v"(lane_ptr) : "memory");
}
__device__ __forceinline__ void vm_issue_load1(u32x4 &xr, const uint16_t *lane_ptr, int r)
{
    const uint8_t *p = reinterpret_cast<const uint8_t *>(lane_ptr) + (r >= 4 ? 4096 : 0);
    switch (r & 3) {
    case 0: asm volatile("global_load_dwordx4 %0, %1, off nt" : "=&v"(xr) : "v"(p) : "memory"); break;
    case 1: asm volatile("global_load_dwordx4 %0, %1, off offset:1024 nt" : "=&v"(xr) : "v"(p) : "memory"); break;
    case 2: asm volatile("global_load_dwordx4 %0, %1, off offset:2048 nt" : "=&v"(xr) : "v"(p) : "memory"); break;
    default: asm volatile("global_load_dwordx4 %0, %1, off offset:3072 nt" : "=&v"(xr) : "v"(p) : "memory"); break;
    }
}
__device__ __forceinline__ void vm_issue_load1(u32x2 &xr, const uint8_t *p, int r)
{
    switch (r) {
    case 0: asm volatile("global_load_dwordx2 %0, %1, off nt" : "=&v"(xr) : "v"(p) : "memory"); break;
    case 1: asm volatile("global_load_dwordx2 %0, %1, off offset:512 nt" : "=&v"(xr) : "v"(p) : "memory"); break;
    case 2: asm volatile("global_load_dwordx2 %0, %1, off offset:1024 nt" : "=&v"(xr) : "v"(p) : "memory"); break;
    case 3: asm volatile("global_load_dwordx2 %0, %1, off offset:1536 nt" : "=&v"(xr) : "v"(p) : "memory"); break;
    case 4: asm volatile("global_load_dwordx2 %0, %1, off offset:2048 nt" : "=&v"(xr) : "v"(p) : "memory"); break;
    case 5: asm volatile("global_load_dwordx2 %0, %1, off offset:2560 nt" : "=&v"(xr) : "v"(p) : "memory"); break;
    case 6: asm volatile("global_load_dwordx2 %0, %1, off offset:3072 nt" : "=&v"(xr) : "v"(p) : "memory"); break;
    default: asm volatile("global_load_dwordx2 %0, %1, off offset:3584 nt" : "=&v"(xr) : "v"(p) : "memory"); break;
    }
}
template <class X>
__device__ __forceinline__ void vm_wait_loads(uint32_t later, X (&x)[R])
{
    switch (later) {
    case 1: asm volatile("s_waitcnt vmcnt(1)" ::: "memory"); break;
    case 2: asm volatile("s_waitcnt vmcnt(2)" ::: "memory"); break;
    case 3: asm volatile("s_waitcnt vmcnt(3)" ::: "memory"); break;
    case 4: asm volatile("s_waitcnt vmcnt(4)" ::: "memory"); break;
    case 5: asm volatile("s_waitcnt vmcnt(5)" ::: "memory"); break;
    case 6: asm volatile("s_waitcnt vmcnt(6)" ::: "memory"); break;
    case 7: asm volatile("s_waitcnt vmcnt(7)" ::: "memory"); break;
    case 8: asm volatile("s_waitcnt vmcnt(8)" ::: "memory"); break;
    default: asm volatile("s_waitcnt vmcnt(0)" ::: "memory"); break;
    }
    asm volatile("" : "+v"(x[0]), "+v"(x[1]), "+v"(x[2]), "+v"(x[3]), "+v"(x[4]), "+v"(x[5]), "+v"(x[6]), "+v"(x[7]) :: "memory");
}

constexpr int STAGE_CAP = 256;
struct __attribute__((aligned(16))) WaveStage {
    uint16_t val[TILE_PX];
    uint16_t out[STAGE_CAP];
};
static_assert(offsetof(WaveStage, out) == sizeof(uint16_t) * TILE_PX && STAGE_CAP >= 64, "compact_dense_in_place: `out` lies right behind `val`, an entry per lane");

__device__ __forceinline__ uint32_t store_lines2(const uint8_t *s0, uint8_t *d0, uint32_t q0, const uint8_t *s1, uint8_t *d1, uint32_t q1)
{
    const uint32_t total = q0 + q1, lane = (uint32_t)lane_id();
    for (uint32_t base = 0; base < total; base += 64) {
        const uint32_t i = base + lane;
        if (i < total) {
            const bool second = i >= q0;
            const uint32_t j = second ? i - q0 : i;
            const u32x4 v = *reinterpret_cast<const u32x4 *>((second ? s1 : s0) + 16 * j);
            *reinterpret_cast<u32x4 *>((second ? d1 : d0) + 16 * j) = v;
        }
    }
    return (total + 63u) >> 6;
}

template <bool LEVEL1, int CODEC, bool KEEP_BITMAP>
__device__ __forceinline__ uint32_t flush_pending(const Pending &p, uint32_t tile, uint32_t n_blk, uint8_t *__restrict__ bitmap,
                                                  uint64_t nb_stride, uint16_t *__restrict__ pix_slots, uint32_t *__restrict__ tile_cnt,
                                                  uint8_t *__restrict__ blk_slots, uint32_t *__restrict__ blk_size, Lz4Lds *lz,
                                                  const WaveStage *st, uint32_t blk_stride, uint32_t comb, uint32_t *__restrict__ blk_aux)
{
    if (!p.valid) return 0;
    const int lane = lane_id();
    uint32_t nst = 0;
    const uint8_t *s0 = nullptr, *s1 = nullptr;
    uint8_t *d0 = nullptr, *d1 = nullptr;
    uint32_t q0 = 0, q1 = 0, bsz = 0;
    if (LEVEL1) {
        s0 = reinterpret_cast<const uint8_t *>(p.buf);
        d0 = reinterpret_cast<uint8_t *>(pix_slots + p.ft * SLOT_PX);
        q0 = ((((p.cnt * p.depth + 31) >> 5) + 31u) & ~31u) >> 2;
    }
    if (CODEC == CODEC_LZ4_RUNS || CODEC == CODEC_LZ4_EVENTS || CODEC == CODEC_BLOSC) {
        const uint64_t bytes = CODEC != CODEC_BLOSC ? ((uint64_t)p.own[0] | ((uint64_t)p.own[1] << 32)) : p.cown;
        bsz = lz4_stage_slot(bytes, n_blk, p.csize, *lz, CODEC == CODEC_BLOSC);
    }
    if (CODEC == CODEC_ZSTD_FAST || CODEC == CODEC_ZSTD_MODELLED) {
        (void)zstd_stage_slot(n_blk, p.last, p.staged, *lz);
        bsz = p.staged ? p.staged : 4u;
    }
    if (CODEC == CODEC_DEFLATE) bsz = p.csize;
    if (CODEC) {
        s1 = lz->out;
        d1 = blk_slots + p.ft * blk_stride;
        q1 = min((((bsz + 3) >> 2) + 31u) & ~31u, (uint32_t)BLK_SLOT / 4) >> 2;
    }
    if (LEVEL1 && CODEC && comb) {
        const uint32_t ro16 = comb == COMB_AT_BLK_SLOT ? (uint32_t)BLK_SLOT / 16 : (bsz + 15) >> 4, r16 = (p.cnt * p.depth + 127) >> 7;
        if (16 * (ro16 + r16) <= blk_stride) {
            d0 = d1 + 16 * ro16;
            if (comb == COMB_AT_BLK_SLOT) q0 = (r16 + 7u) & ~7u;
            else { q1 = ro16; q0 = ((ro16 + r16 + 7u) & ~7u) - ro16; }
        }
    }
    if (q0 + q1) nst += store_lines2(s0, d0, q0, s1, d1, q1);
    if (KEEP_BITMAP) {
        *reinterpret_cast<u32x2 *>(bitmap + (uint64_t)p.f * nb_stride + (uint64_t)tile * TILE_BM + lane * 8) = p.own;
        nst += 1;
    }
    if (LEVEL1 || CODEC) {
        const uint32_t word = CODEC == CODEC_ZSTD_FAST || CODEC == CODEC_ZSTD_MODELLED ? p.csize : bsz;
        if (LEVEL1 && CODEC == CODEC_DEFLATE) {
            if (lane < 3) *(lane == 0 ? &tile_cnt[p.ft] : (lane == 1 ? &blk_size[p.ft] : &blk_aux[p.ft])) = lane == 0 ? p.cnt : (lane == 1 ? word : p.aux);
        } else if (LEVEL1 && CODEC) {
            if (lane < 2) *(lane == 0 ? &tile_cnt[p.ft] : &blk_size[p.ft]) = lane == 0 ? p.cnt : word;
        } else if (LEVEL1) {
            if (lane == 0) tile_cnt[p.ft] = p.cnt;
        } else if (CODEC == CODEC_DEFLATE) {
            if (lane < 2) *(lane == 0 ? &blk_size[p.ft] : &blk_aux[p.ft]) = lane == 0 ? word : p.aux;
        } else {
            if (lane == 0) blk_size[p.ft] = word;
        }
        nst += 1;
    }
    return (uint32_t)__builtin_amdgcn_readfirstlane((int)nst);
}

__device__ __forceinline__ void compact_dense_in_place(WaveStage *st, const uint8_t *bm)
{
    const int lane = lane_id();
    uint32_t inc[3], tot[3];
#pragma unroll
    for (int g = 0; g < 3; ++g) {
        uint32_t pk = 0;
#pragma unroll
        for (int k = 0; k < 3; ++k)
            if (3 * g + k < R) pk |= (uint32_t)__builtin_popcount((uint32_t)bm[(3 * g + k) * 64 + lane]) << (10 * k);
        inc[g] = wave_incl_scan(pk);
        tot[g] = wave_last(inc[g]);
    }
    uint32_t base = 0;
#pragma unroll
    for (int r = 0; r < R; ++r) {
        const uint32_t m = bm[r * 64 + lane];
        const uint32_t dst = base + ((inc[r / 3] >> (10 * (r % 3))) & 0x3FFu) - (uint32_t)__builtin_popcount(m);
        const u32x4 v = (reinterpret_cast<const u32x4 *>(st->val) + lane)[r * 64];
        __builtin_amdgcn_wave_barrier();
        uint16_t *const vo = st->val;
#pragma unroll
        for (int j = 0; j < 8; ++j) {
            const uint32_t a = (m >> j) & 1u ? dst + (uint32_t)__builtin_popcount(m & ((1u << j) - 1u)) : (uint32_t)TILE_PX + (uint32_t)lane;
            vo[a] = (uint16_t)(v[j >> 1] >> (16 * (j & 1)));
        }
        __builtin_amdgcn_wave_barrier();
        base += (tot[r / 3] >> (10 * (r % 3))) & 0x3FFu;
    }
}

constexpr uint32_t FUSED12_CAP = (uint32_t)(STAGE_CAP * 16 / 12);
__device__ __forceinline__ void compact_pack12(WaveStage *st, const u32x2 &own, uint32_t exc, uint32_t cnt)
{
    const int lane = lane_id();
    uint32_t *out32 = reinterpret_cast<uint32_t *>(st->out);
    *reinterpret_cast<u32x2 *>(out32 + 2 * lane) = u32x2{0u, 0u};
    __builtin_amdgcn_wave_barrier();
    const uint16_t *mine = st->val + 64 * lane;
    uint64_t q = (uint64_t)own[0] | ((uint64_t)own[1] << 32);
    uint32_t left = cnt, P = 12u * exc;
    do {
        uint32_t x[4];
#pragma unroll
        for (int k = 0; k < 4; ++k) {
            const uint32_t i = q ? (uint32_t)__builtin_ctzll(q) : 0u;
            q &= q - 1;
            x[k] = mine[i];
        }
#pragma unroll
        for (int k = 0; k < 4; ++k) x[k] = (uint32_t)k < left ? (x[k] & 0xFFFu) : 0u;
        const uint32_t lo = x[0] | (x[1] << 12) | (x[2] << 24), hi = (x[2] >> 8) | (x[3] << 4);
        const uint32_t w = P >> 5, sh = P & 31u;
        const uint64_t a = (uint64_t)lo << sh, b = (uint64_t)hi << sh;
        const uint32_t d0 = (uint32_t)a, d1 = (uint32_t)(a >> 32) | (uint32_t)b, d2 = (uint32_t)(b >> 32);
        if (left) {
            __hip_atomic_fetch_or(&out32[w], d0, __ATOMIC_RELAXED, __HIP_MEMORY_SCOPE_WAVEFRONT);
            if (d1) __hip_atomic_fetch_or(&out32[w + 1], d1, __ATOMIC_RELAXED, __HIP_MEMORY_SCOPE_WAVEFRONT);
            if (d2) __hip_atomic_fetch_or(&out32[w + 2], d2, __ATOMIC_RELAXED, __HIP_MEMORY_SCOPE_WAVEFRONT);
        }
        left = left > 4u ? left - 4u : 0u;
        P += 48u;
    } while (__builtin_amdgcn_ballot_w64(left != 0) != 0);
    __builtin_amdgcn_wave_barrier();
}

template <bool ALIGNED, bool ASMLOAD, bool LEVEL1, int CODEC, bool KEEP_BITMAP, bool RAWVAL, int SB>
__device__ __forceinline__ void reduce_one_frame(typename Src<SB>::X (&x)[R], const typename Src<SB>::T *__restrict__ cur, const typename Src<SB>::T *__restrict__ next, bool have_next,
                                                 const u32x4 (&t)[R], uint64_t lane_px0, uint64_t N, bool full,
                                                 uint32_t f, uint32_t tile, uint64_t ft, uint32_t n_blk, uint8_t *__restrict__ bitmap,
                                                 uint64_t nb_stride, uint16_t *__restrict__ pix_slots,
                                                 uint32_t *__restrict__ tile_cnt, uint8_t *__restrict__ blk_slots,
                                                 uint32_t *__restrict__ blk_size, Lz4Lds *s_lz, uint8_t *s_bm, WaveStage *st,
                                                 Pending &pend, uint32_t &stores_behind, const ZmParams &zp, uint32_t blk_stride, uint32_t comb,
                                                 uint32_t *__restrict__ blk_aux)
{
    const int lane = lane_id();
    RC_PHASE_BEGIN
    if (ASMLOAD) vm_wait_loads(stores_behind, x);
    else if (ALIGNED && full) {
        typedef typename Src<SB>::X XU __attribute__((aligned(SB)));
        const XU *p = reinterpret_cast<const XU *>(cur + lane_px0);
#pragma unroll
        for (int r = 0; r < R; ++r) x[r] = __builtin_nontemporal_load(p + r * (GROUP_PX / 8));
    } else {
#pragma unroll
        for (int r = 0; r < R; ++r) x[r] = load8<ALIGNED, true, SB>(cur, lane_px0 + (uint64_t)r * GROUP_PX, N, 0);
    }
    RC_PHASE(0);
    uint32_t m8[R];
#pragma unroll
    for (int r = 0; r < R; ++r) {
        const u32x4 tt = t[r];
        u32x4 xv = widen8(x[r]);
#pragma unroll
        for (int k = 0; k < 4; ++k) xv[k] = pk_sub_sat_u16(xv[k], tt[k]);
        const uint32_t one = 0x00010001u;
        uint32_t M = 0;
#pragma unroll
        for (int k = 3; k >= 0; --k)
            M = __builtin_amdgcn_udot2(__builtin_bit_cast(u16x2, pk_min_u16(xv[k], one)),
                                       __builtin_bit_cast(u16x2, (uint32_t)((1u << (2 * k)) | (2u << (2 * k + 16)))), M, false);
        m8[r] = M;
        if (LEVEL1) {
            u32x4 v = xv;
            if (RAWVAL) {
#pragma unroll
                for (int k = 0; k < 4; ++k) v[k] = pk_add_u16(v[k], tt[k]);
            }
            (reinterpret_cast<u32x4 *>(st->val) + lane)[r * 64] = v;
        }
        if (ASMLOAD && have_next) vm_issue_load1(x[r], next + lane_px0, r);
    }
    RC_PHASE(1);
    RC_PHASE(2);
    pend.valid = true;
    pend.ft = ft;
    pend.f = f;
    pend.cnt = 0;
    pend.csize = 0;
    pend.buf = st->out;
    if (LEVEL1 || KEEP_BITMAP || CODEC) {
        uint8_t *bm = CODEC ? s_lz->raw : s_bm;
#pragma unroll
        for (int r = 0; r < R; ++r) bm[r * 64 + lane] = (uint8_t)m8[r];
        __builtin_amdgcn_wave_barrier();
        pend.own = *reinterpret_cast<const u32x2 *>(&bm[lane * 8]);
    }
    RC_PHASE(3);
    if (LEVEL1) {
        const uint32_t cnt = (uint32_t)__builtin_popcount(pend.own[0]) + (uint32_t)__builtin_popcount(pend.own[1]);
        const uint32_t inc = wave_incl_scan(cnt);
        const uint32_t wave_total = wave_last(inc);
        bool packed = false;
        if (pend.depth == 12 && wave_total <= FUSED12_CAP) {
            if (wave_total) compact_pack12(st, pend.own, inc - cnt, cnt);
            packed = true;
        } else if (wave_total <= (uint32_t)STAGE_CAP) {
#pragma unroll
            for (int h = 0; h < 2; ++h) {
                const uint16_t *mine = st->val + 64 * lane + 32 * h;
                uint32_t qh = pend.own[h];
                uint32_t o = inc - cnt + (h ? (uint32_t)__builtin_popcount(pend.own[0]) : 0u);
                while (qh) {
                    const uint32_t i0 = (uint32_t)__builtin_ctz(qh);
                    qh &= qh - 1;
                    const bool two = qh != 0;
                    const uint32_t i1 = two ? (uint32_t)__builtin_ctz(qh) : i0;
                    qh &= qh - 1;
                    const uint16_t v0 = mine[i0], v1 = mine[i1];
                    st->out[o] = v0;
                    if (two) st->out[o + 1] = v1;
                    o += 2;
                }
            }
        } else {
            pend.buf = st->val;
            __builtin_amdgcn_wave_barrier();
            compact_dense_in_place(st, CODEC ? s_lz->raw : s_bm);
        }
        __builtin_amdgcn_wave_barrier();
        pend.cnt = wave_total;
        if (!packed && pend.depth < 16 && wave_total) pack_stage(pend.buf, wave_total, pend.depth);
    }
    RC_PHASE(4);
    if (CODEC == CODEC_LZ4_RUNS) {
        const uint64_t bytes = (uint64_t)pend.own[0] | ((uint64_t)pend.own[1] << 32);
        pend.csize = lz4_encode_block<false>(bytes, n_blk, *s_lz);
    }
    if (CODEC == CODEC_LZ4_EVENTS) {
        const uint64_t bytes = (uint64_t)pend.own[0] | ((uint64_t)pend.own[1] << 32);
        pend.csize = lz4_encode_block<true>(bytes, n_blk, *s_lz);
    }
    if (CODEC == CODEC_ZSTD_FAST) {
        const uint64_t bytes = (uint64_t)pend.own[0] | ((uint64_t)pend.own[1] << 32);
        pend.csize = zstd_tokenize_block(bytes, n_blk, pend.last, *s_lz, pend.staged);
    }
    if (CODEC == CODEC_ZSTD_MODELLED) {
        const uint64_t bytes = (uint64_t)pend.own[0] | ((uint64_t)pend.own[1] << 32);
        pend.csize = zstd_tokenize_block_m(bytes, n_blk, pend.last, *s_lz, pend.staged, zp);
    }
    if (CODEC == CODEC_DEFLATE) {
        const uint64_t bytes = (uint64_t)pend.own[0] | ((uint64_t)pend.own[1] << 32);
        pend.aux = deflate_adler_word(bytes, tile);
        pend.csize = deflate_encode_block<true>(bytes, n_blk, pend.last, *s_lz);
    }
    if (CODEC == CODEC_BLOSC) {
        const uint64_t bytes = (uint64_t)pend.own[0] | ((uint64_t)pend.own[1] << 32);
        pend.cown = bitshuffle_block(bytes, n_blk, *s_lz);
        pend.csize = lz4_encode_block(pend.cown, n_blk, *s_lz);
    }
    RC_PHASE(5);
    stores_behind = flush_pending<LEVEL1, CODEC, KEEP_BITMAP>(pend, tile, n_blk, bitmap, nb_stride, pix_slots, tile_cnt, blk_slots, blk_size, s_lz, st, blk_stride, comb, blk_aux);
    pend.valid = false;
    RC_PHASE(6);
}

template <int RWAVES, int BZ, bool ALIGNED, bool ASMLOAD, bool LEVEL1, int CODEC, bool KEEP_BITMAP, bool RAWVAL, int SB>
__global__ __launch_bounds__(64 * RWAVES) __attribute__((amdgpu_waves_per_eu((ALIGNED && ASMLOAD) ? ((RWAVES == 4 && LEVEL1) ? 3 : 4) : 1))) void k_reduce_tiles(const typename Src<SB>::T *__restrict__ frames,
                                                       const uint16_t *__restrict__ thr, uint64_t N, uint32_t ntiles,
                                                       uint32_t tile0, uint32_t tile_end,
                                                       uint32_t B, uint32_t ngroups, uint64_t nb,
                                                       uint8_t *__restrict__ bitmap, uint64_t nb_stride,
                                                       uint16_t *__restrict__ pix_slots, uint32_t *__restrict__ tile_cnt,
                                                       uint8_t *__restrict__ blk_slots, uint32_t *__restrict__ blk_size, uint32_t depth,
                                                       BatchStatus *__restrict__ status, ZmParams zm, uint32_t blk_stride, uint32_t comb,
                                                       uint32_t *__restrict__ blk_aux)
{
    if (blockIdx.x == 0 && threadIdx.x == 0) { status->code = 0; status->frame = 0; status->total = 0; }
    __shared__ uint16_t s_code[CODEC == CODEC_ZSTD_MODELLED ? 256 : 2];
    if (CODEC == CODEC_ZSTD_MODELLED) {
        for (uint32_t i = threadIdx.x; i < 128; i += 64 * RWAVES) reinterpret_cast<uint32_t *>(s_code)[i] = reinterpret_cast<const uint32_t *>(zm.lit_code)[i];
        __syncthreads();
        zm.lit_code = s_code;
    }
    __shared__ Lz4Lds s_lz[CODEC ? RWAVES : 1];
    __shared__ __attribute__((aligned(16))) uint8_t s_bm[CODEC ? 1 : RWAVES][CODEC ? 16 : TILE_BM];
    __shared__ WaveStage s_stage[LEVEL1 ? RWAVES : 1];

    const uint32_t xcd = blockIdx.x & 7u, j = blockIdx.x >> 3;
    const uint32_t grp = j % ngroups;
    const uint32_t tblock = (j / ngroups) * 8u + xcd;
    const int lane = lane_id();
    const int w = __builtin_amdgcn_readfirstlane((int)(threadIdx.x >> 6));
    const uint32_t tile = tile0 + tblock * RWAVES + w;
    if (tile >= tile_end) return;
    const uint64_t lane_px0 = (uint64_t)tile * TILE_PX + (uint64_t)lane * 8;
    const uint32_t f0 = grp * BZ;
    if (f0 >= B) return;
    const bool full = (uint64_t)(tile + 1) * TILE_PX <= N;

    typename Src<SB>::X xa[R];
    if (ASMLOAD) vm_issue_loads(xa, frames + (uint64_t)f0 * N + lane_px0);
    u32x4 t[R];
#pragma unroll
    for (int r = 0; r < R; ++r) t[r] = load8<ALIGNED, false, 2>(thr, lane_px0 + (uint64_t)r * GROUP_PX, N, 0xFFFF);
    const uint32_t n_blk = (uint32_t)min((uint64_t)TILE_BM, nb - (uint64_t)tile * TILE_BM);
    Lz4Lds *lz = &s_lz[CODEC ? w : 0];
    uint8_t *bm = s_bm[CODEC ? 0 : w];
    WaveStage *st = &s_stage[LEVEL1 ? w : 0];
    Pending pend;
    pend.valid = false;
    pend.ft = 0; pend.f = 0; pend.cnt = 0; pend.csize = 0; pend.own = u32x2{0u, 0u};
    pend.staged = 0; pend.last = tile + 1 == ntiles; pend.cown = 0; pend.aux = 0;
    pend.depth = (LEVEL1 && !RAWVAL) ? depth : 16u;
    pend.buf = nullptr;

    uint32_t stores_behind = 0;
#pragma unroll 1
    for (int z = 0; z < BZ; ++z) {
        const uint32_t f = f0 + z;
        if (f >= B) break;
        const bool nxt = z + 1 < BZ && f + 1 < B;
        reduce_one_frame<ALIGNED, ASMLOAD, LEVEL1, CODEC, KEEP_BITMAP, RAWVAL, SB>(xa, frames + (uint64_t)f * N, frames + (uint64_t)(f + 1) * N, nxt, t,
                                                                             lane_px0, N, full, f, tile, (uint64_t)f * ntiles + tile, n_blk,
                                                                             bitmap, nb_stride, pix_slots, tile_cnt, blk_slots,
                                                                             blk_size, lz, bm, st, pend, stores_behind, zm, blk_stride, comb, blk_aux);
        if (!nxt) break;
    }
    flush_pending<LEVEL1, CODEC, KEEP_BITMAP>(pend, tile, n_blk, bitmap, nb_stride, pix_slots, tile_cnt, blk_slots, blk_size, lz, st, blk_stride, comb, blk_aux);
}

template <int BZ, bool AL, bool L1, int CODEC, bool KEEP, bool RAW, int SB>
static void launch_reduce_t(const Scratch &sc, const typename Src<SB>::T *frames, uint32_t B, uint32_t depth, hipStream_t s, hipStream_t s_tail)
{
    const uint32_t ngroups = (B + BZ - 1) / BZ;
    const uint32_t nfull = AL ? (uint32_t)(sc.N / TILE_PX) : 0u;
    const ZmParams zm{reinterpret_cast<const uint16_t *>(sc.zm_lit_code), sc.zm_valid, sc.zm_budget, sc.zm_seq_bits};
    const uint32_t comb = (L1 && !RAW && CODEC) ? sc.comb : COMB_OFF;
    const bool three = L1 && !RAW && CODEC != CODEC_DEFLATE &&
                       (CODEC == CODEC_LZ4_RUNS || CODEC == CODEC_LZ4_EVENTS || sc.ntiles > 8192 || (CODEC == CODEC_ZSTD_MODELLED && (sc.zm_valid & ZM_LITS_ONLY)));
    auto go = [&](auto rw) {
        constexpr int RW = decltype(rw)::value;
        auto grid_for = [&](uint32_t nt) { return (((nt + RW - 1) / RW + 7) / 8) * 8 * ngroups; };
        if (nfull)
            hipLaunchKernelGGL((k_reduce_tiles<RW, BZ, AL, AL, L1, CODEC, KEEP, RAW, SB>), dim3(grid_for(nfull)), dim3(64 * RW), 0, s, frames, sc.thr, sc.N,
                               sc.ntiles, 0u, nfull, B, ngroups, sc.nb, sc.bitmap, sc.nb_stride, sc.pix_slots, sc.tile_cnt, sc.blk_slots,
                               sc.blk_size, depth, sc.status, zm, sc.blk_stride, comb, sc.blk_aux);
        if (nfull < sc.ntiles) {
            if (AL && sc.N % 8 != 0)
                hipLaunchKernelGGL((k_reduce_tiles<RW, BZ, false, false, L1, CODEC, KEEP, RAW, SB>), dim3(grid_for(sc.ntiles - nfull)), dim3(64 * RW), 0, nfull ? s_tail : s, frames,
                                   sc.thr, sc.N, sc.ntiles, nfull, sc.ntiles, B, ngroups, sc.nb, sc.bitmap, sc.nb_stride, sc.pix_slots, sc.tile_cnt,
                                   sc.blk_slots, sc.blk_size, depth, sc.status, zm, sc.blk_stride, comb, sc.blk_aux);
            else
                hipLaunchKernelGGL((k_reduce_tiles<RW, BZ, AL, false, L1, CODEC, KEEP, RAW, SB>), dim3(grid_for(sc.ntiles - nfull)), dim3(64 * RW), 0, nfull ? s_tail : s, frames,
                                   sc.thr, sc.N, sc.ntiles, nfull, sc.ntiles, B, ngroups, sc.nb, sc.bitmap, sc.nb_stride, sc.pix_slots, sc.tile_cnt,
                                   sc.blk_slots, sc.blk_size, depth, sc.status, zm, sc.blk_stride, comb, sc.blk_aux);
        }
    };
    if constexpr (SB == 2) {
        if (three) { go(int_c<3>{}); return; }
    }
    go(int_c<4>{});
}
template <int BZ, bool AL, bool L1, bool RAW, int SB>
static void launch_reduce_c(const Scratch &sc, const typename Src<SB>::T *frames, uint32_t B, uint32_t codec, bool keep, uint32_t depth, hipStream_t s, hipStream_t s_tail)
{
    if (RAW) keep = true;
#define RC_CODEC(C)                                                                                      \
    if (codec == C) {                                                                                    \
        if (keep) launch_reduce_t<BZ, AL, L1, C, true, RAW, SB>(sc, frames, B, depth, s, s_tail);        \
        else if (!RAW) launch_reduce_t<BZ, AL, L1, C, false, false, SB>(sc, frames, B, depth, s, s_tail); \
        return;                                                                                          \
    }
    RC_CODEC(CODEC_LZ4_RUNS) RC_CODEC(CODEC_LZ4_EVENTS) RC_CODEC(CODEC_ZSTD_FAST) RC_CODEC(CODEC_ZSTD_MODELLED) RC_CODEC(CODEC_BLOSC) RC_CODEC(CODEC_DEFLATE)
#undef RC_CODEC
    launch_reduce_t<BZ, AL, L1, CODEC_NONE, true, RAW, SB>(sc, frames, B, depth, s, s_tail);
}
template <int BZ, bool AL, int SB>
static void launch_reduce_a(const Scratch &sc, const typename Src<SB>::T *frames, uint32_t B, uint32_t level, uint32_t codec, bool keep,
                            uint32_t depth, hipStream_t s, hipStream_t s_tail)
{
    if (level == 2) launch_reduce_c<BZ, AL, true, true, SB>(sc, frames, B, codec, keep, depth, s, s_tail);
    else if (level == 1) launch_reduce_c<BZ, AL, true, false, SB>(sc, frames, B, codec, keep, depth, s, s_tail);
    else launch_reduce_c<BZ, AL, false, false, SB>(sc, frames, B, codec, keep, depth, s, s_tail);
}
#ifdef RC_PHASE_TIMING
extern "C" __attribute__((visibility("default"))) int rc_debug_phases(unsigned long long *out16)
{
    unsigned long long z[16] = {};
    if (hipDeviceSynchronize() != hipSuccess) return -1;
    if (hipMemcpyFromSymbol(out16, HIP_SYMBOL(g_phase), sizeof z) != hipSuccess) return -1;
    if (hipMemcpyToSymbol(HIP_SYMBOL(g_phase), z, sizeof z) != hipSuccess) return -1;
    return 0;
}
#endif
void launch_reduce(const Scratch &sc, const void *frames, uint32_t B, uint32_t level, uint32_t codec, bool keep_bitmap,
                   uint32_t depth, hipStream_t s, hipStream_t s_tail, uint32_t src_bytes)
{
    if (depth == 0 || depth > 16) depth = 16;
    if (!s_tail) s_tail = s;
    const bool aligned = !sc.guarded_loads;
    if (src_bytes == 1) {
        const uint8_t *f8 = static_cast<const uint8_t *>(frames);
        if (aligned) launch_reduce_a<REDUCE_BZ, true, 1>(sc, f8, B, level, codec, keep_bitmap, depth, s, s_tail);
        else launch_reduce_a<REDUCE_BZ, false, 1>(sc, f8, B, level, codec, keep_bitmap, depth, s, s_tail);
        return;
    }
    const uint16_t *f16 = static_cast<const uint16_t *>(frames);
    if (aligned) launch_reduce_a<REDUCE_BZ, true, 2>(sc, f16, B, level, codec, keep_bitmap, depth, s, s_tail);
    else launch_reduce_a<REDUCE_BZ, false, 2>(sc, f16, B, level, codec, keep_bitmap, depth, s, s_tail);
}

constexpr int SCAN_T = 256, SCAN_W = SCAN_T / 64;

__device__ __forceinline__ uint32_t scan_block_excl(uint32_t v, uint32_t *sm, uint32_t *total)
{
    const int w = threadIdx.x >> 6;
    const uint32_t inc = wave_incl_scan(v);
    if (lane_id() == 63) sm[w] = inc;
    __syncthreads();
    uint32_t base = 0, tot = 0;
#pragma unroll
    for (int i = 0; i < SCAN_W; ++i) {
        const uint32_t x = sm[i];
        if (i < w) base += x;
        tot += x;
    }
    __syncthreads();
    *total = tot;
    return base + inc - v;
}

template <int SCAN_I>
__device__ __forceinline__ void scan_row(uint32_t *__restrict__ row, uint32_t *__restrict__ orow, uint32_t n,
                                         uint32_t *__restrict__ total, uint32_t *sm, const uint32_t *adj = nullptr)
{
    uint32_t carry = 0;
    for (uint32_t t0 = 0; t0 < n; t0 += SCAN_T * SCAN_I) {
        const uint32_t t = t0 + threadIdx.x * SCAN_I;
        uint32_t v[SCAN_I], s = 0;
#pragma unroll
        for (int k = 0; k < SCAN_I; ++k) {
            v[k] = t + k < n ? row[t + k] : 0;
            if (adj) {
                v[k] &= 0xFFFFu;
                if (t + k == adj[0]) v[k] += adj[1];
                if (t + k == adj[2]) v[k] += adj[3];
                if (t + k < n) row[t + k] = v[k];
            }
            s += v[k];
        }
        uint32_t tot;
        uint32_t ex = carry + scan_block_excl(s, sm, &tot);
#pragma unroll
        for (int k = 0; k < SCAN_I; ++k) {
            if (t + k < n) orow[t + k] = ex;
            ex += v[k];
        }
        carry += tot;
    }
    if (threadIdx.x == 0) *total = carry;
}

__device__ __forceinline__ void zstd_rewrite_defs(const uint32_t *__restrict__ row, uint8_t *__restrict__ slots, uint32_t stride,
                                                  const uint8_t *__restrict__ tree, uint32_t tl, const uint8_t *__restrict__ sdesc, uint32_t sl,
                                                  uint32_t t_tree, uint32_t t_seq, uint32_t which, uint8_t *s_img, uint32_t *s_pos)
{
    for (int pass = 0; pass < 2; ++pass) {
        const uint32_t t = pass == 0 ? t_tree : t_seq;
        if (t == 0xFFFFFFFFu || (pass == 1 && t == t_tree) || !((which >> pass) & 1u)) continue;
        const uint32_t a_tl = pass == 0 ? tl : 0u, a_sl = (pass == 1 || t_seq == t_tree) ? sl : 0u;
        uint8_t *slot = slots + (uint64_t)t * stride;
        const uint32_t size = row[t] & 0xFFFFu;
        __syncthreads();
        for (uint32_t i = threadIdx.x; i < (size + 3) / 4; i += blockDim.x)
            reinterpret_cast<uint32_t *>(s_img)[i] = reinterpret_cast<const uint32_t *>(slot)[i];
        __syncthreads();
        if (threadIdx.x == 0) { uint32_t q; (void)zm_block_needs(s_img, &q); *s_pos = q; }
        __syncthreads();
        const uint32_t pos = *s_pos;
        for (uint32_t i = threadIdx.x; i < size + a_tl + a_sl; i += blockDim.x)
            slot[i] = zm_defs_byte(s_img, pos, tree, a_tl, sdesc, a_sl, i);
    }
    __syncthreads();
}

__device__ __forceinline__ void zstd_place_defs(const uint32_t *__restrict__ row, uint32_t n, uint8_t *__restrict__ slots, uint32_t stride,
                                                const uint8_t *__restrict__ tree, uint32_t tree_len, const uint8_t *__restrict__ sdesc,
                                                uint32_t sdesc_len, uint32_t *adj)
{
    __shared__ uint32_t s_first[2];
    __shared__ uint32_t s_pos;
    __shared__ __attribute__((aligned(16))) uint8_t s_img[PIX_SLOT + 16];
    if (threadIdx.x < 2) s_first[threadIdx.x] = 0xFFFFFFFFu;
    __syncthreads();
    const uint32_t w0 = row[0];
    const bool both0 = (w0 & ZW_TREE) && ((w0 & ZW_SEQ) || !sdesc_len);
    if (both0) {
        if (threadIdx.x == 0) { s_first[0] = 0; if (sdesc_len) s_first[1] = 0; }
    } else {
        uint32_t mt = 0xFFFFFFFFu, mq = 0xFFFFFFFFu;
        for (uint32_t t = threadIdx.x; t < n; t += SCAN_T) {
            const uint32_t w = row[t];
            if ((w & ZW_TREE) && t < mt) mt = t;
            if ((w & ZW_SEQ) && t < mq) mq = t;
        }
        if (mt != 0xFFFFFFFFu) atomicMin(&s_first[0], mt);
        if (mq != 0xFFFFFFFFu) atomicMin(&s_first[1], mq);
    }
    __syncthreads();
    const uint32_t t_tree = s_first[0], t_seq = s_first[1];
    const uint32_t tl = t_tree != 0xFFFFFFFFu ? tree_len : 0u, sl = t_seq != 0xFFFFFFFFu ? sdesc_len : 0u;
    if (threadIdx.x == 0) { adj[0] = t_tree; adj[1] = tl; adj[2] = t_seq; adj[3] = sl; }
    zstd_rewrite_defs(row, slots, stride, tree, tl, sdesc, sl, t_tree, t_seq, 3u, s_img, &s_pos);
}

__global__ __launch_bounds__(SCAN_T) void k_pix_scan(Scratch sc, uint32_t depth)
{
    __shared__ uint32_t sm[SCAN_W];
    __shared__ uint32_t s_adj[4];
    const uint32_t f = blockIdx.x;
    const ZstdModel *M = sc.zm_model;
    const uint32_t npk = packed_bytes(sc.frame_nnz[f], depth);
    const uint32_t nch = value_chunks(npk, PIX_CHUNK);
    uint32_t *row = sc.chunk_size + (uint64_t)f * sc.nchunk_max;
    zstd_place_defs(row, nch, sc.pix_chunks + (uint64_t)f * sc.nchunk_max * PIX_SLOT, PIX_SLOT, M->pix_desc, M->pix_desc_len, nullptr, 0, s_adj);
    scan_row<16>(row, sc.chunk_off + (uint64_t)f * sc.nchunk_max, nch, sc.frame_pbytes + f, sm, s_adj);
}
void launch_pix_scan(const Scratch &sc, uint32_t B, uint32_t depth, hipStream_t s)
{
    hipLaunchKernelGGL(k_pix_scan, dim3(B), dim3(SCAN_T), 0, s, sc, depth);
}

template <int SCAN_I>
__global__ __launch_bounds__(SCAN_T) void k_scan_frames(Scratch sc, int with_counts, int with_blocks)
{
    __shared__ uint32_t sm[SCAN_W];
    __shared__ uint32_t s_carry;
    __shared__ uint32_t s_adj[4];
    const uint32_t f = blockIdx.x, n = sc.ntiles;
    const uint64_t fr = (uint64_t)f * n;
    if (with_blocks) {
        if (sc.zm_model) {
            const ZstdModel *M = sc.zm_model;
            zstd_place_defs(sc.blk_size + fr, n, sc.blk_slots + fr * sc.blk_stride, sc.blk_stride, M->lit_desc, M->lit_desc_len, M->seq_desc,
                            M->seq_desc_len, s_adj);
        }
        scan_row<SCAN_I>(sc.blk_size + fr, sc.blk_off + fr, n, sc.frame_cbytes + f, sm, sc.zm_model ? s_adj : nullptr);
    }
    if (!with_counts) return;
    uint32_t *row = sc.tile_cnt + fr;
    scan_row<SCAN_I>(row, sc.tile_off + fr, n, sc.frame_nnz + f, sm);
    uint32_t *nrow = sc.tile_next + fr;
    if (threadIdx.x == 0) s_carry = n;
    __syncthreads();
    const uint32_t per_round = SCAN_T * SCAN_I;
    const uint32_t nrounds = (n + per_round - 1) / per_round;
    for (uint32_t c = nrounds; c-- > 0;) {
        const uint32_t t = c * per_round + threadIdx.x * SCAN_I;
        uint32_t v[SCAN_I];
        uint32_t first = 0xFFFFFFFFu;
#pragma unroll
        for (int k = SCAN_I - 1; k >= 0; --k) {
            v[k] = t + k < n ? row[t + k] : 0;
            if (v[k]) first = t + k;
        }
        uint32_t m = first;
#pragma unroll
        for (int d = 1; d < 64; d <<= 1) {
            const uint32_t y = __shfl_down(m, d);
            if (lane_id() + d < 64) m = min(m, y);
        }
        const int w = threadIdx.x >> 6;
        if (lane_id() == 0) sm[w] = m;
        __syncthreads();
        uint32_t right = s_carry;
#pragma unroll
        for (int i = SCAN_W - 1; i >= 0; --i)
            if (i > w) right = min(right, sm[i]);
        uint32_t excl = __shfl_down(m, 1);
        if (lane_id() == 63) excl = 0xFFFFFFFFu;
        uint32_t nxt = min(excl, right);
#pragma unroll
        for (int k = SCAN_I - 1; k >= 0; --k) {
            if (t + k < n) nrow[t + k] = nxt;
            if (v[k]) nxt = t + k;
        }
        __syncthreads();
        if (threadIdx.x == 0) {
            uint32_t all = s_carry;
#pragma unroll
            for (int i = 0; i < SCAN_W; ++i) all = min(all, sm[i]);
            s_carry = all;
        }
        __syncthreads();
    }
}

constexpr int SEG_I = 16, SEG = SCAN_T * SEG_I;
struct ScanPart { uint32_t blk_sum, cnt_sum, first_nonempty, first_tree, first_seq, pad[3]; };

__global__ __launch_bounds__(SCAN_T) void k_scan_seg(Scratch sc, int with_counts, int with_blocks)
{
    __shared__ uint32_t sm[SCAN_W];
    __shared__ uint32_t s_min[3];
    const uint32_t seg = blockIdx.x, f = blockIdx.y, n = sc.ntiles, nseg = gridDim.x;
    const uint64_t fr = (uint64_t)f * n;
    const uint32_t t = seg * SEG + threadIdx.x * SEG_I;
    ScanPart *part = reinterpret_cast<ScanPart *>(sc.scan_part) + (uint64_t)f * nseg + seg;
    if (threadIdx.x < 3) s_min[threadIdx.x] = 0xFFFFFFFFu;
    __syncthreads();
    uint32_t blk_sum = 0, cnt_sum = 0;
    if (with_blocks) {
        uint32_t *row = sc.blk_size + fr, *orow = sc.blk_off + fr;
        const bool zm = sc.zm_model != nullptr;
        uint32_t v[SEG_I], sum = 0, mt = 0xFFFFFFFFu, mq = 0xFFFFFFFFu;
#pragma unroll
        for (int k = 0; k < SEG_I; ++k) {
            const uint32_t w = t + k < n ? row[t + k] : 0;
            if (zm) {
                if ((w & ZW_TREE) && mt == 0xFFFFFFFFu) mt = t + k;
                if ((w & ZW_SEQ) && mq == 0xFFFFFFFFu) mq = t + k;
                v[k] = w & 0xFFFFu;
                if (t + k < n) row[t + k] = v[k];
            } else v[k] = w;
            sum += v[k];
        }
        if (mt != 0xFFFFFFFFu) atomicMin(&s_min[1], mt);
        if (mq != 0xFFFFFFFFu) atomicMin(&s_min[2], mq);
        uint32_t ex = scan_block_excl(sum, sm, &blk_sum);
#pragma unroll
        for (int k = 0; k < SEG_I; ++k) {
            if (t + k < n) orow[t + k] = ex;
            ex += v[k];
        }
    }
    if (with_counts) {
        const uint32_t *row = sc.tile_cnt + fr;
        uint32_t *orow = sc.tile_off + fr, *nrow = sc.tile_next + fr;
        uint32_t v[SEG_I], sum = 0, first = 0xFFFFFFFFu;
#pragma unroll
        for (int k = SEG_I - 1; k >= 0; --k) {
            v[k] = t + k < n ? row[t + k] : 0;
            if (v[k]) first = t + k;
            sum += v[k];
        }
        uint32_t ex = scan_block_excl(sum, sm, &cnt_sum);
#pragma unroll
        for (int k = 0; k < SEG_I; ++k) {
            if (t + k < n) orow[t + k] = ex;
            ex += v[k];
        }
        uint32_t m = first;
#pragma unroll
        for (int d = 1; d < 64; d <<= 1) {
            const uint32_t y = __shfl_down(m, d);
            if (lane_id() + d < 64) m = min(m, y);
        }
        const int w = threadIdx.x >> 6;
        __syncthreads();
        if (lane_id() == 0) sm[w] = m;
        __syncthreads();
        uint32_t right = 0xFFFFFFFFu;
#pragma unroll
        for (int i = SCAN_W - 1; i >= 0; --i)
            if (i > w) right = min(right, sm[i]);
        uint32_t excl = __shfl_down(m, 1);
        if (lane_id() == 63) excl = 0xFFFFFFFFu;
        uint32_t nxt = min(excl, right);
#pragma unroll
        for (int k = SEG_I - 1; k >= 0; --k) {
            if (t + k < n) nrow[t + k] = nxt;
            if (v[k]) nxt = t + k;
        }
        if (first != 0xFFFFFFFFu) atomicMin(&s_min[0], first);
    }
    __syncthreads();
    if (threadIdx.x == 0) {
        if (with_blocks) { part->blk_sum = blk_sum; part->first_tree = s_min[1]; part->first_seq = s_min[2]; }
        if (with_counts) { part->cnt_sum = cnt_sum; part->first_nonempty = s_min[0]; }
    }
}

__global__ __launch_bounds__(SCAN_T) void k_scan_fix(Scratch sc, int with_counts, int with_blocks)
{
    __shared__ uint32_t s_v[8];
    __shared__ uint32_t s_pos;
    __shared__ __attribute__((aligned(16))) uint8_t s_img[PIX_SLOT + 16];
    const uint32_t seg = blockIdx.x, f = blockIdx.y, n = sc.ntiles, nseg = gridDim.x;
    const uint64_t fr = (uint64_t)f * n;
    const ScanPart *parts = reinterpret_cast<const ScanPart *>(sc.scan_part) + (uint64_t)f * nseg;
    if (threadIdx.x == 0) {
        uint32_t bb = 0, cb = 0, bt = 0, ct = 0, nx = n, tt = 0xFFFFFFFFu, tq = 0xFFFFFFFFu;
        for (uint32_t i = 0; i < nseg; ++i) {
            const ScanPart p = parts[i];
            if (i < seg) { bb += p.blk_sum; cb += p.cnt_sum; }
            bt += p.blk_sum; ct += p.cnt_sum;
            if (i > seg && p.first_nonempty < nx) nx = p.first_nonempty;
            tt = min(tt, p.first_tree); tq = min(tq, p.first_seq);
        }
        s_v[0] = bb; s_v[1] = cb; s_v[2] = nx; s_v[3] = tt; s_v[4] = tq; s_v[5] = bt; s_v[6] = ct;
    }
    __syncthreads();
    const uint32_t lo = seg * SEG, hi = min(lo + (uint32_t)SEG, n);
    if (with_blocks) {
        uint32_t tl = 0, sl = 0;
        const uint32_t t_tree = s_v[3], t_seq = s_v[4];
        if (sc.zm_model) {
            const ZstdModel *M = sc.zm_model;
            tl = t_tree != 0xFFFFFFFFu ? M->lit_desc_len : 0u;
            sl = t_seq != 0xFFFFFFFFu ? M->seq_desc_len : 0u;
            const uint32_t mine = (t_tree >= lo && t_tree < hi ? 1u : 0u) | (t_seq >= lo && t_seq < hi ? 2u : 0u);
            if (mine) {
                zstd_rewrite_defs(sc.blk_size + fr, sc.blk_slots + fr * sc.blk_stride, sc.blk_stride, M->lit_desc, tl, M->seq_desc, sl, t_tree, t_seq, mine, s_img, &s_pos);
                if (threadIdx.x == 0) {
                    if (mine & 1u) sc.blk_size[fr + t_tree] += tl;
                    if (mine & 2u) sc.blk_size[fr + t_seq] += sl;
                }
            }
        }
        uint32_t *orow = sc.blk_off + fr;
        const uint32_t base = s_v[0];
        for (uint32_t t = lo + threadIdx.x; t < hi; t += SCAN_T)
            orow[t] += base + (t > t_tree ? tl : 0u) + (t > t_seq ? sl : 0u);
        if (seg == 0 && threadIdx.x == 0) sc.frame_cbytes[f] = s_v[5] + tl + sl;
    }
    if (with_counts) {
        uint32_t *orow = sc.tile_off + fr, *nrow = sc.tile_next + fr;
        const uint32_t base = s_v[1], nx = s_v[2];
        for (uint32_t t = lo + threadIdx.x; t < hi; t += SCAN_T) {
            orow[t] += base;
            if (nrow[t] == 0xFFFFFFFFu) nrow[t] = nx;
        }
        if (seg == 0 && threadIdx.x == 0) sc.frame_nnz[f] = s_v[6];
    }
}

void launch_scans(const Scratch &sc, uint32_t B, bool with_counts, bool with_blocks, hipStream_t s)
{
    if (!with_counts && !with_blocks) return;
    if (sc.ntiles > (uint32_t)SEG && sc.scan_part) {
        const dim3 grid((sc.ntiles + SEG - 1) / SEG, B);
        hipLaunchKernelGGL(k_scan_seg, grid, dim3(SCAN_T), 0, s, sc, with_counts ? 1 : 0, with_blocks ? 1 : 0);
        hipLaunchKernelGGL(k_scan_fix, grid, dim3(SCAN_T), 0, s, sc, with_counts ? 1 : 0, with_blocks ? 1 : 0);
        return;
    }
    if (sc.ntiles > 8192) hipLaunchKernelGGL(k_scan_frames<32>, dim3(B), dim3(SCAN_T), 0, s, sc, with_counts ? 1 : 0, with_blocks ? 1 : 0);
    else hipLaunchKernelGGL(k_scan_frames<16>, dim3(B), dim3(SCAN_T), 0, s, sc, with_counts ? 1 : 0, with_blocks ? 1 : 0);
}

constexpr int LWG = WG;
__global__ __launch_bounds__(LWG) void k_layout(const uint32_t *__restrict__ frame_nnz,
                                                 const uint32_t *__restrict__ frame_cbytes, const uint32_t *__restrict__ frame_pbytes,
                                                 RecordParams rp, uint64_t nb,
                                                 uint32_t ntiles, uint32_t B, uint64_t out_cap, uint64_t *__restrict__ rec_off,
                                                 uint32_t *__restrict__ md, BatchStatus *__restrict__ st, u32x4 *__restrict__ zl_acc)
{
    __shared__ uint64_t s_part[LWG];
    __shared__ uint32_t s_bad;
    if (threadIdx.x == 0) s_bad = 0xFFFFFFFFu;
    __syncthreads();
    const uint32_t per = (B + LWG - 1) / LWG;
    const uint32_t lo = threadIdx.x * per;
    const uint32_t hi = min(lo + per, B);
    uint64_t sum = 0;
    for (uint32_t f = lo; f < hi; ++f) {
        const uint32_t nnz = rp.level == 1 ? frame_nnz[f] : 0;
        const uint32_t npk = rp.level == 1 ? packed_bytes(nnz, rp.depth) : 0;
        uint64_t sz;
        uint32_t m0 = 0, m1 = 0, m2 = 0;
        if (rp.emit == EMIT_RAW) {
            if (rp.level == 1) { sz = 8 + nb + npk; m0 = npk; }
            else sz = 4 + nb;
        } else {
            const FrameFmt ff = frame_fmt(rp.emit);
            const uint32_t cb = bitmap_hdr(ff, rp.emit, ntiles) + frame_cbytes[f] + ff.end;
            if (rp.level == 1) {
                const uint32_t cp = rp.pix_mode == PIX_MODE_SKIP ? ff.hdr + frame_pbytes[f] : stored_size(ff, npk);
                sz = 16 + (uint64_t)cb + cp; m0 = cb; m1 = cp; m2 = npk;
            } else { sz = 8 + (uint64_t)cb; m0 = cb; }
        }
        md[3 * f] = m0; md[3 * f + 1] = m1; md[3 * f + 2] = m2;
        if (zl_acc) { zl_acc[2 * f] = u32x4{0u, 0u, 0u, 0u}; zl_acc[2 * f + 1] = u32x4{0u, 0u, 0u, 0u}; }
        if (sz > rp.frame_bytes) atomicMin(&s_bad, f);
        rec_off[f + 1] = sz;
        sum += sz;
    }
    s_part[threadIdx.x] = sum;
    __syncthreads();
    uint64_t base = 0;
    for (uint32_t i = 0; i < threadIdx.x; ++i) base += s_part[i];
    for (uint32_t f = lo; f < hi; ++f) {
        const uint64_t sz = rec_off[f + 1];
        base += sz;
        rec_off[f + 1] = base;
    }
    if (threadIdx.x == 0) rec_off[0] = 0;
    __syncthreads();
    if (threadIdx.x == LWG - 1) {
        uint64_t total = 0;
        for (uint32_t i = 0; i < LWG; ++i) total += s_part[i];
        st->total = total;
        if (s_bad != 0xFFFFFFFFu) { st->code = -5; st->frame = s_bad; }
        else if (total > out_cap) { st->code = -2; st->frame = 0; }
    }
}

void launch_layout(const Scratch &sc, const RecordParams &rp, uint32_t B, uint64_t out_cap, uint64_t *rec_off,
                   uint32_t *md, hipStream_t s)
{
    hipLaunchKernelGGL(k_layout, dim3(1), dim3(LWG), 0, s, sc.frame_nnz, sc.frame_cbytes, sc.frame_pbytes, rp, sc.nb, sc.ntiles, B, out_cap,
                       rec_off, md, sc.status, reinterpret_cast<u32x4 *>(sc.zl_acc));
}

static uint32_t xxh32_small(const uint8_t *p, size_t n)
{
    const uint32_t P1 = 2654435761u, P2 = 2246822519u, P3 = 3266489917u, P4 = 668265263u, P5 = 374761393u;
    (void)P1; (void)P4;
    uint32_t h = 0  + P5 + (uint32_t)n;
    for (size_t i = 0; i < n; ++i) {
        h += p[i] * P5;
        h = ((h << 11) | (h >> 21)) * P1;
    }
    h ^= h >> 15; h *= P2; h ^= h >> 13; h *= P3; h ^= h >> 16;
    return h;
}
uint32_t lz4f_descriptor(uint8_t bd)
{
    const uint8_t desc[2] = {0x60 , bd};
    const uint8_t hc = (uint8_t)((xxh32_small(desc, 2) >> 8) & 0xFF);
    return desc[0] | ((uint32_t)desc[1] << 8) | ((uint32_t)hc << 16);
}

void launch_assemble(const Scratch &sc, const RecordParams &rp, uint32_t B, uint8_t *out, const uint64_t *rec_off,
                     uint32_t batch_seq, hipStream_t s)
{
    static const uint32_t hdr_bitmap = lz4f_descriptor(0x40);
    static const uint32_t hdr_pix = lz4f_descriptor(0x70);
    launch_gather(sc, rp, B, out, rec_off, hdr_bitmap, hdr_pix, batch_seq, s);
}

}
```

pyrecode_amd/csrc/rc_zstd.hip:

```cpp
#include <algorithm>
#include <cstring>

#include <cstdlib>
#include "rc_launch.h"
#include "rc_zstd_block.h"
#include "rc_zstd_model.h"
#include "rc_zstd_wave.h"

namespace rc {

__global__ __launch_bounds__(WG) void k_zstd_buffer(Scratch sc)
{
    __shared__ Lz4Lds s_lz[WAVES];
    const int w = __builtin_amdgcn_readfirstlane((int)(threadIdx.x >> 6)), lane = lane_id();
    const uint32_t t = blockIdx.x * WAVES + w, f = blockIdx.y;
    if (t >= sc.ntiles) return;
    const uint64_t b0 = (uint64_t)t * TILE_BM;
    const uint32_t n = (uint32_t)min((uint64_t)TILE_BM, sc.nb - b0);
    const u32x2 v = reinterpret_cast<const u32x2 *>(sc.bitmap + (uint64_t)f * sc.nb_stride + b0)[lane];
    const uint64_t own = (uint64_t)v[0] | ((uint64_t)v[1] << 32);
    const bool last = t + 1 == sc.ntiles;
    uint32_t staged;
    const uint32_t word = zstd_tokenize_block(own, n, last, s_lz[w], staged);
    const uint64_t ft = (uint64_t)f * sc.ntiles + t;
    zstd_store_block(sc.blk_slots + ft * sc.blk_stride, n, last, word, staged, s_lz[w]);
    if (lane == 0) sc.blk_size[ft] = word;
}

constexpr int FSE_ROW = 48;
constexpr int FSE_T = 128;

__global__ __launch_bounds__(FSE_T) void k_zstd_fse(Scratch sc, uint32_t nslots, const ZstdTables *__restrict__ tables, uint32_t fitted)
{
    __shared__ ZstdTables T;
    __shared__ uint32_t s_row[FSE_T][FSE_ROW + 1];
    {
        const uint32_t *src = reinterpret_cast<const uint32_t *>(tables);
        uint32_t *dst = reinterpret_cast<uint32_t *>(&T);
        for (uint32_t i = threadIdx.x; i < sizeof(ZstdTables) / 4; i += FSE_T) dst[i] = src[i];
    }
    __syncthreads();
    const uint32_t ft = blockIdx.x * FSE_T + threadIdx.x;
    if (ft >= nslots) return;
    const uint32_t word = sc.blk_size[ft];
    if (word & ZW_FINAL) { sc.blk_size[ft] = word & (0xFFFFu | ZW_TREE); return; }
    const uint32_t P = word & 0xFFFFu, nseq = (word >> 16) & 0xFFu;
    uint32_t *slot32 = reinterpret_cast<uint32_t *>(sc.blk_slots + (uint64_t)ft * sc.blk_stride);
    const ZW4 *tok4 = reinterpret_cast<const ZW4 *>(slot32 + (zstd_token_offset(P) >> 2));
    const uint32_t w0 = P >> 2, nb0 = 8 * (P & 3u);
    const uint64_t acc0 = nb0 ? (uint64_t)(slot32[w0] & ((1u << nb0) - 1u)) : 0ull;
    uint32_t *row = s_row[threadIdx.x];
    uint32_t o = 0;
    uint64_t acc = acc0;
    uint32_t nb = fse_chain(tok4, nseq, acc, nb0, T, [&](uint32_t v) { if (o < (uint32_t)FSE_ROW) row[o] = v; ++o; });
    uint32_t ndw = o + ((nb + 31) >> 5);
    const uint32_t end = 4 * (w0 + o) + ((nb + 7) >> 3);
    if (ndw <= (uint32_t)FSE_ROW) {
        if (nb) { row[o] = (uint32_t)acc; if (nb > 32) row[o + 1] = (uint32_t)(acc >> 32); }
        for (uint32_t i = 0; i < ndw; ++i) slot32[w0 + i] = row[i];
    } else {
        o = 0;
        acc = acc0;
        nb = fse_chain(tok4, nseq, acc, nb0, T, [&](uint32_t v) { slot32[w0 + o] = v; ++o; });
        if (nb) { slot32[w0 + o] = (uint32_t)acc; if (nb > 32) slot32[w0 + o + 1] = (uint32_t)(acc >> 32); }
    }
    const uint32_t content = end - 3;
    const uint32_t lastbit = (ft % sc.ntiles) + 1 == sc.ntiles ? 1u : 0u;
    slot32[0] |= lastbit | (2u << 1) | (content << 3);
    sc.blk_size[ft] = end | (word & ZW_TREE) | (fitted ? ZW_SEQ : 0u);
}
void launch_zstd_fse(const Scratch &sc, uint32_t B, const void *tables_dev, bool fitted, hipStream_t s)
{
    const uint32_t nslots = B * sc.ntiles;
    hipLaunchKernelGGL(k_zstd_fse, dim3((nslots + FSE_T - 1) / FSE_T), dim3(FSE_T), 0, s, sc, nslots,
                       reinterpret_cast<const ZstdTables *>(tables_dev), fitted ? 1u : 0u);
}

void launch_zstd_tokenize_rows(const Scratch &sc, uint32_t B, hipStream_t s)
{
    hipLaunchKernelGGL(k_zstd_buffer, dim3((sc.ntiles + WAVES - 1) / WAVES, B), dim3(WG), 0, s, sc);
}

void launch_zstd_encode_blocks(const Scratch &sc, uint32_t B, const void *tables_dev, hipStream_t s)
{
    hipLaunchKernelGGL(k_zstd_buffer, dim3((sc.ntiles + WAVES - 1) / WAVES, B), dim3(WG), 0, s, sc);
    launch_zstd_fse(sc, B, tables_dev, false, s);
}

__global__ __launch_bounds__(WG) void k_zstd_sample(Scratch sc, uint32_t B, uint32_t with_pix, uint32_t depth, ZstdSample *__restrict__ h)
{
    __shared__ ZstdSample s_h;
    constexpr uint32_t NW = sizeof(ZstdSample) / 4;
    for (uint32_t i = threadIdx.x; i < NW; i += WG) reinterpret_cast<uint32_t *>(&s_h)[i] = 0;
    __syncthreads();
    const uint32_t f = blockIdx.y;
    const int lane = lane_id();
    for (uint32_t t = blockIdx.x * WAVES + (threadIdx.x >> 6); t < sc.ntiles && f < B; t += gridDim.x * WAVES) {
        const uint64_t ft = (uint64_t)f * sc.ntiles + t;
        const uint32_t word = sc.blk_size[ft];
        if (!(word & ZW_FINAL)) {
            const uint8_t *slot = sc.blk_slots + ft * sc.blk_stride;
            const uint32_t P = word & 0xFFFFu, nseq = word >> 16;
            const uint32_t b3 = slot[3];
            const uint32_t lh = (b3 & 4u) ? 2u : 1u;
            const uint32_t nlit = lh == 1 ? (b3 >> 3) : ((b3 >> 4) | ((uint32_t)slot[4] << 4));
            for (uint32_t i = lane; i < nlit; i += 64) atomicAdd(&s_h.lit[slot[3 + lh + i]], 1u);
            const uint32_t *tok = reinterpret_cast<const uint32_t *>(slot + zstd_token_offset(P));
            for (uint32_t i = lane; i < nseq; i += 64) {
                const uint32_t k = tok[i];
                atomicAdd(&s_h.ll[k & 63u], 1u);
                atomicAdd(&s_h.ml[(k >> 6) & 63u], 1u);
            }
        }
        if ((word & 0xFFFFu) != 4u || !(word & ZW_FINAL)) {
            const uint64_t b0 = (uint64_t)t * TILE_BM;
            const uint32_t nbm = (uint32_t)(sc.nb - b0 < (uint64_t)TILE_BM ? sc.nb - b0 : (uint64_t)TILE_BM);
            const uint8_t *bm = sc.bitmap + (uint64_t)f * sc.nb_stride + b0;
            for (uint32_t i = lane; i < nbm; i += 64) atomicAdd(&s_h.all[bm[i]], 1u);
            if (lane == 0) atomicAdd(&s_h.nblk, 1u);
        }
        if (with_pix) {
            const uint32_t nbytes = (sc.tile_cnt[ft] * depth + 7) >> 3;
            const uint8_t *p = residual_src(sc, ft, 0u, sc.tile_cnt[ft], depth);
            for (uint32_t i = lane; i < nbytes; i += 64) atomicAdd(&s_h.pix[p[i]], 1u);
        }
    }
    __syncthreads();
    for (uint32_t i = threadIdx.x; i < NW; i += WG) {
        const uint32_t v = reinterpret_cast<uint32_t *>(&s_h)[i];
        if (v) atomicAdd(reinterpret_cast<uint32_t *>(h) + i, v);
    }
}
void launch_zstd_sample(const Scratch &sc, uint32_t B, bool with_pix, uint32_t depth, void *sample_dev, hipStream_t s)
{
    const uint32_t gx = std::min<uint32_t>((sc.ntiles + WAVES - 1) / WAVES, 512u);
    hipLaunchKernelGGL(k_zstd_sample, dim3(gx, B), dim3(WG), 0, s, sc, B, with_pix ? 1u : 0u, depth,
                       reinterpret_cast<ZstdSample *>(sample_dev));
}
size_t zstd_model_bytes() { return sizeof(ZstdModel); }
size_t zstd_sample_bytes() { return sizeof(ZstdSample); }
void zstd_model_from_sample(const void *sample_host, void *model_host, uint32_t speed_permille)
{
    ZstdSample h = *reinterpret_cast<const ZstdSample *>(sample_host);
    if (getenv("RC_ZSTD_SEQ_ALWAYS")) h.nblk = 0;
    if (getenv("RC_ZSTD_LITS_ALWAYS")) { for (auto &v : h.ll) v = 0x100000; h.nblk = h.nblk ? h.nblk : 1; }
    zm_build_model(h, *reinterpret_cast<ZstdModel *>(model_host), speed_permille);
}

size_t zstd_tables_bytes() { return sizeof(ZstdTables); }
void zstd_tables_host(void *dst)
{
    ZstdTables t;
    zstd_build_tables(t);
    memcpy(dst, &t, sizeof t);
}

__global__ __launch_bounds__(WG) void k_zstd_gather(Scratch sc, uint8_t *__restrict__ out)
{
    const uint32_t t = blockIdx.x * WAVES + (threadIdx.x >> 6);
    if (t >= sc.ntiles) return;
    if (t == 0 && lane_id() == 0) {
        out[0] = 0x28; out[1] = 0xB5; out[2] = 0x2F; out[3] = 0xFD;
        out[4] = 0x00;
        out[5] = 0x00;
    }
    const uint8_t *src = sc.blk_slots + (uint64_t)t * BLK_SLOT;
    uint8_t *dst = out + 6 + sc.blk_off[t];
    const uint32_t n = sc.blk_size[t];
    for (uint32_t i = lane_id(); i < n; i += 64) dst[i] = src[i];
}
void launch_zstd_gather(const Scratch &sc, uint8_t *out, hipStream_t s)
{
    hipLaunchKernelGGL(k_zstd_gather, dim3((sc.ntiles + WAVES - 1) / WAVES), dim3(WG), 0, s, sc, out);
}

}
```

Measured before the change: 148,000 frames/s.

## Store per-tile count and block-size words in a wave-interleaved order

Per-tile metadata words (tile_cnt, blk_size, blk_aux) are now laid out in an order indexed by the reduce kernel's wave/tile mapping: tiles are split into eight segments by tile-block index, with padding up to 32-word boundaries. The aim is for the stores that concurrent waves make in the reduce kernel to land in contiguous or less conflicting memory, rather than being strided across the row. Every consumer (scans, gather, zstd FSE/sample, def rewriting) now has to translate tile indices through tile_word, which adds index arithmetic and makes reads in the scan and gather kernels non-contiguous. The allocation grows slightly to hold the padded row.

Result: no change. 148,900 frames/s (median of 3 runs) (+0.7%).

```diff
diff --git a/pyrecode_amd/csrc/rc_api.hip b/pyrecode_amd/csrc/rc_api.hip
--- a/pyrecode_amd/csrc/rc_api.hip
+++ b/pyrecode_amd/csrc/rc_api.hip
@@ -117,7 +117,8 @@
     DevMem &m = c->dmem;
     const uint64_t B = c->max_batch, T = sc.ntiles;
     RC_ALLOC(m, sc.bitmap, B * sc.nb_stride + 64);
-    RC_ALLOC(m, sc.tile_cnt, B * T * 4);
+    const uint64_t W = tile_word_row_max(sc.ntiles);
+    RC_ALLOC(m, sc.tile_cnt, B * W * 4);
     RC_ALLOC(m, sc.tile_off, B * T * 4);
     RC_ALLOC(m, sc.tile_next, B * T * 4);
     RC_ALLOC(m, sc.frame_nnz, B * 4);
@@ -131,10 +132,10 @@
             sc.blk_stride = 1536;
         }
         RC_ALLOC(m, sc.blk_slots, B * T * (uint64_t)sc.blk_stride + 256);
-        RC_ALLOC(m, sc.blk_size, B * T * 4);
+        RC_ALLOC(m, sc.blk_size, B * W * 4);
         RC_ALLOC(m, sc.blk_off, B * T * 4);
         if (c->emit == EMIT_DEFLATE) {
-            RC_ALLOC(m, sc.blk_aux, B * T * 4);
+            RC_ALLOC(m, sc.blk_aux, B * W * 4);
             RC_ALLOC(m, sc.zl_acc, B * 32);
             HIP_TRY(hipMemset(sc.zl_acc, 0, B * 32));
         }
@@ -418,7 +419,7 @@
     using namespace rc;
     const bool dz = c->values == VALUES_DEFLATE_HUFF;
     hipStream_t s = c->stream;
-    const Scratch &sc = c->sets[c->cur];
+    Scratch sc = c->sets[c->cur];
     const uint32_t ns = n < 2 ? n : 2;
     void *d_sample = dz ? (void *)c->d_dzhist : c->d_sample, *h_sample = dz ? (void *)c->h_dzhist : c->h_sample;
     void *d_model = dz ? (void *)c->d_dzm : c->d_model, *h_model = dz ? (void *)c->h_dzm : c->h_model;
@@ -427,6 +428,7 @@
         if (c->post_pending[k]) HIP_TRY(hipStreamWaitEvent(s, c->ev_post[k], 0));
     HIP_TRY(hipMemsetAsync(d_sample, 0, sample_bytes, s));
     if (dz) {
+        sc.rw = reduce_word_order(sc, 1u, CODEC_DEFLATE, c->src_bytes);
         launch_reduce(sc, frames_dev, ns, 1u, CODEC_DEFLATE, true, c->depth, s, nullptr, c->src_bytes);
         launch_scans(sc, ns, true, true, s);
         RecordParams rp;
@@ -436,6 +438,7 @@
         launch_assemble(sc, rp, ns, nullptr, nullptr, c->batch_seq, s);
         launch_pd_hist(sc, ns, c->depth, c->d_dzhist, s);
     } else {
+        sc.rw = reduce_word_order(sc, c->level == 3 ? 3u : 1u, CODEC_ZSTD_FAST, c->src_bytes);
         launch_reduce(sc, frames_dev, ns, c->level == 3 ? 3u : 1u, CODEC_ZSTD_FAST, true, c->depth, s, nullptr, c->src_bytes);
         launch_zstd_sample(sc, ns, c->level == 1, c->depth, c->d_sample, s);
     }
@@ -507,7 +510,7 @@
     const int k = c->cur;
     c->cur ^= 1;
     c->last = k;
-    const rc::Scratch &sc = c->sets[k];
+    rc::Scratch sc = c->sets[k];
     const bool two = c->pipelined && c->two_chains;
     hipStream_t ps = two && k == 1 ? c->pstream_b : c->pstream;
     c->last_ps = ps;
@@ -522,6 +525,7 @@
     }
     const uint32_t codec = fused_codec(c->emit, c->clevel, c->modelled, c->src_bytes);
     const bool keep_maps = c->keep_bitmap || c->emit == EMIT_RAW;
+    sc.rw = reduce_word_order(sc, c->level, codec, c->src_bytes);
     if (c->src_bytes == 4)
         launch_reduce32(sc, static_cast<const uint32_t *>(frames_dev), c->thr32, n, c->level, c->depth, s, codec, keep_maps);
     else
diff --git a/pyrecode_amd/csrc/rc_gather.hip b/pyrecode_amd/csrc/rc_gather.hip
--- a/pyrecode_amd/csrc/rc_gather.hip
+++ b/pyrecode_amd/csrc/rc_gather.hip
@@ -16,6 +16,7 @@
     BatchStatus *status, *first_err;
     uint64_t nb, nb_stride, pixraw_stride;
     uint32_t ntiles, blk_stride, pix_slot_bytes, comb;
+    uint32_t rw;
 };
 
 typedef u32x4 u32x4_u __attribute__((aligned(1)));
@@ -103,6 +104,9 @@
         const uint32_t f = item / gpf, g = item - f * gpf, t0 = tpi * g, t = t0 + lane;
         const bool have = lane < tpi && t < sc.ntiles;
         const uint64_t frow = (uint64_t)f * sc.ntiles;
+        const uint32_t wseg = sc.rw ? tile_word_seg(sc.ntiles, sc.rw) : 0u;
+        const uint64_t wrow = (uint64_t)f * tile_word_row(sc.ntiles, sc.rw);
+        const uint64_t wt = wrow + tile_word(t, sc.rw, wseg);
         uint8_t *rec = flat ? sc.pixraw + (uint64_t)f * sc.pixraw_stride : out + rec_off[f];
         const uint32_t nnz = rp.level == 1 ? sc.frame_nnz[f] : 0;
         const uint32_t npk = rp.level == 1 ? packed_bytes(nnz, d) : 0;
@@ -117,7 +121,7 @@
 
         uint32_t word = 0, bsz = 0, bdst = 0, cnt = 0, rn = 0, rdst = 0, rs = 0xFFFFFFFFu, ps0 = 0, flags = 0, blo = 0;
         AdlerAcc ad{0u, 0u};
-        if (have && rp.emit != EMIT_RAW && (!flat || (sc.comb == COMB_BEHIND_BLOCK && pixp))) word = sc.blk_size[frow + t];
+        if (have && rp.emit != EMIT_RAW && (!flat || (sc.comb == COMB_BEHIND_BLOCK && pixp))) word = sc.blk_size[wt];
         if (have && !flat) {
             if (rp.emit == EMIT_RAW) {
                 const uint64_t b0 = (uint64_t)t * TILE_BM;
@@ -131,7 +135,7 @@
             }
         }
         if (have && pixp) {
-            cnt = sc.tile_cnt[frow + t];
+            cnt = sc.tile_cnt[wt];
             if (cnt) {
                 const ResidGeom q = resid_geom(sc.tile_off[frow + t], cnt, d);
                 ps0 = q.ps0;
@@ -147,9 +151,10 @@
         }
         uint32_t ext_cnt = 0, ext_first = 0;
         if (BITS && pixp && t0 + tpi < sc.ntiles) {
-            ext_cnt = sc.tile_cnt[frow + t0 + tpi];
+            const uint64_t we = wrow + tile_word(t0 + tpi, sc.rw, wseg);
+            ext_cnt = sc.tile_cnt[we];
             if (ext_cnt)
-                ext_first = *reinterpret_cast<const uint32_t *>(residual_src(sc, frow + t0 + tpi, sc.comb == COMB_BEHIND_BLOCK ? sc.blk_size[frow + t0 + tpi] : 0u, ext_cnt, d));
+                ext_first = *reinterpret_cast<const uint32_t *>(residual_src(sc, frow + t0 + tpi, sc.comb == COMB_BEHIND_BLOCK ? sc.blk_size[we] : 0u, ext_cnt, d));
         }
         const uint8_t *slot = rp.emit == EMIT_RAW ? sc.bitmap + (uint64_t)f * sc.nb_stride + (uint64_t)t0 * TILE_BM : sc.blk_slots + (frow + t0) * sc.blk_stride;
         const uint32_t slot_stride = rp.emit == EMIT_RAW ? (uint32_t)TILE_BM : sc.blk_stride;
@@ -243,8 +248,9 @@
         if (got < 8) {
             uint32_t tt = cur == 65 ? (t0 + tpi - 1 < sc.ntiles ? sc.tile_next[frow + t0 + tpi - 1] : sc.ntiles) : (t0 + tpi < sc.ntiles ? sc.tile_next[frow + t0 + tpi] : sc.ntiles);
             while (tt < sc.ntiles) {
-                const uint32_t cc = sc.tile_cnt[frow + tt];
-                const uint32_t fd = *reinterpret_cast<const uint32_t *>(residual_src(sc, frow + tt, sc.comb == COMB_BEHIND_BLOCK ? sc.blk_size[frow + tt] : 0u, cc, d));
+                const uint64_t wn = wrow + tile_word(tt, sc.rw, wseg);
+                const uint32_t cc = sc.tile_cnt[wn];
+                const uint32_t fd = *reinterpret_cast<const uint32_t *>(residual_src(sc, frow + tt, sc.comb == COMB_BEHIND_BLOCK ? sc.blk_size[wn] : 0u, cc, d));
                 const uint32_t take = min(8u - got, cc * d);
                 byte |= (fd & ((1u << take) - 1u)) << got;
                 got += take;
@@ -259,7 +265,7 @@
         }
         }
         if (ADLER && !flat) {
-            const uint32_t aux = have ? sc.blk_aux[frow + t] : 0u;
+            const uint32_t aux = have ? sc.blk_aux[wt] : 0u;
             const uint32_t tA0 = wave_last(wave_incl_scan(aux & 0xFFFFu)), tW0 = wave_last(wave_incl_scan(aux >> 16));
             const uint32_t tA1 = wave_last(wave_incl_scan(ad.A % ADLER_P)), tW1 = wave_last(wave_incl_scan(ad.W));
             if (lane == 0) {
@@ -300,7 +306,7 @@
     while (tpi > 8 && (uint64_t)B * ((sc.ntiles + tpi - 1) / tpi) < 1024) tpi >>= 1;
     const uint32_t gpf = (sc.ntiles + tpi - 1) / tpi, nitems = gpf * B, wgs = nitems;
     const GatherArgs ga{sc.blk_slots, sc.bitmap, sc.pix_slots, sc.blk_size, sc.blk_off, sc.tile_cnt, sc.tile_off, sc.tile_next, sc.frame_nnz, sc.frame_cbytes,
-                        sc.frame_pbytes, sc.blk_aux, sc.zl_acc, sc.pixraw, sc.status, sc.first_err, sc.nb, sc.nb_stride, sc.pixraw_stride, sc.ntiles, sc.blk_stride, sc.pix_slot_bytes, sc.comb};
+                        sc.frame_pbytes, sc.blk_aux, sc.zl_acc, sc.pixraw, sc.status, sc.first_err, sc.nb, sc.nb_stride, sc.pixraw_stride, sc.ntiles, sc.blk_stride, sc.pix_slot_bytes, sc.comb, sc.rw};
     const bool bits = rp.level == 1 && rp.depth % 8 != 0;
     if (rp.emit == EMIT_DEFLATE) {
         if (bits) hipLaunchKernelGGL((k_gather<true, GATHER_UB - 1, true>), dim3(wgs), dim3(64), 0, s, ga, rp, out, rec_off, hdr_bitmap, hdr_pix, batch_seq, gpf, nitems, tpi);
diff --git a/pyrecode_amd/csrc/rc_launch.h b/pyrecode_amd/csrc/rc_launch.h
--- a/pyrecode_amd/csrc/rc_launch.h
+++ b/pyrecode_amd/csrc/rc_launch.h
@@ -4,6 +4,7 @@
 
 #include "../../include/recode_hip.h"
 #include "rc_device.h"
+#include "rc_tile_order.h"
 
 namespace rc {
 
@@ -56,7 +57,14 @@
     uint16_t *l2_base = nullptr;
     uint32_t *chunk_aux = nullptr;
     const DeflateModel *dz_model = nullptr;
+    uint32_t rw = 0;
 };
+
+template <class S>
+__host__ __device__ inline uint64_t tile_word_at(const S &sc, uint32_t f, uint32_t t)
+{
+    return sc.rw ? (uint64_t)f * (8u * tile_word_seg(sc.ntiles, sc.rw)) + tile_word(t, sc.rw, tile_word_seg(sc.ntiles, sc.rw)) : (uint64_t)f * sc.ntiles + t;
+}
 
 constexpr uint32_t EMIT_RAW = 0u;
 constexpr uint32_t EMIT_ZSTD = 1u;
@@ -89,6 +97,7 @@
 };
 
 void launch_threshold(const void *dark, int64_t eps, uint64_t N, uint16_t *thr, hipStream_t s, uint32_t src_bytes = 2);
+uint32_t reduce_word_order(const Scratch &sc, uint32_t level, uint32_t codec, uint32_t src_bytes);
 void launch_reduce(const Scratch &sc, const void *frames, uint32_t B, uint32_t level, uint32_t codec, bool keep_bitmap,
                    uint32_t depth, hipStream_t s, hipStream_t s_tail = nullptr, uint32_t src_bytes = 2);
 void launch_threshold32(const uint32_t *dark, int64_t eps, uint64_t N, uint32_t *thr, hipStream_t s);
diff --git a/pyrecode_amd/csrc/rc_reduce.hip b/pyrecode_amd/csrc/rc_reduce.hip
--- a/pyrecode_amd/csrc/rc_reduce.hip
+++ b/pyrecode_amd/csrc/rc_reduce.hip
@@ -1,3 +1,4 @@
+#include <assert.h>
 #include <cstddef>
 #include <cstdlib>
 #include <type_traits>
@@ -212,7 +213,8 @@
 __device__ __forceinline__ uint32_t flush_pending(const Pending &p, uint32_t tile, uint32_t n_blk, uint8_t *__restrict__ bitmap,
                                                   uint64_t nb_stride, uint16_t *__restrict__ pix_slots, uint32_t *__restrict__ tile_cnt,
                                                   uint8_t *__restrict__ blk_slots, uint32_t *__restrict__ blk_size, Lz4Lds *lz,
-                                                  const WaveStage *st, uint32_t blk_stride, uint32_t comb, uint32_t *__restrict__ blk_aux)
+                                                  const WaveStage *st, uint32_t blk_stride, uint32_t comb, uint32_t *__restrict__ blk_aux,
+                                                  uint32_t wrow, uint32_t wslot)
 {
     if (!p.valid) return 0;
     const int lane = lane_id();
@@ -253,17 +255,18 @@
         nst += 1;
     }
     if (LEVEL1 || CODEC) {
+        const uint64_t fw = (uint64_t)p.f * wrow + wslot;
         const uint32_t word = CODEC == CODEC_ZSTD_FAST || CODEC == CODEC_ZSTD_MODELLED ? p.csize : bsz;
         if (LEVEL1 && CODEC == CODEC_DEFLATE) {
-            if (lane < 3) *(lane == 0 ? &tile_cnt[p.ft] : (lane == 1 ? &blk_size[p.ft] : &blk_aux[p.ft])) = lane == 0 ? p.cnt : (lane == 1 ? word : p.aux);
+            if (lane < 3) *(lane == 0 ? &tile_cnt[fw] : (lane == 1 ? &blk_size[fw] : &blk_aux[fw])) = lane == 0 ? p.cnt : (lane == 1 ? word : p.aux);
         } else if (LEVEL1 && CODEC) {
-            if (lane < 2) *(lane == 0 ? &tile_cnt[p.ft] : &blk_size[p.ft]) = lane == 0 ? p.cnt : word;
+            if (lane < 2) *(lane == 0 ? &tile_cnt[fw] : &blk_size[fw]) = lane == 0 ? p.cnt : word;
         } else if (LEVEL1) {
-            if (lane == 0) tile_cnt[p.ft] = p.cnt;
+            if (lane == 0) tile_cnt[fw] = p.cnt;
         } else if (CODEC == CODEC_DEFLATE) {
-            if (lane < 2) *(lane == 0 ? &blk_size[p.ft] : &blk_aux[p.ft]) = lane == 0 ? word : p.aux;
+            if (lane < 2) *(lane == 0 ? &blk_size[fw] : &blk_aux[fw]) = lane == 0 ? word : p.aux;
         } else {
-            if (lane == 0) blk_size[p.ft] = word;
+            if (lane == 0) blk_size[fw] = word;
         }
         nst += 1;
     }
@@ -344,7 +347,7 @@
                                                  uint32_t *__restrict__ tile_cnt, uint8_t *__restrict__ blk_slots,
                                                  uint32_t *__restrict__ blk_size, Lz4Lds *s_lz, uint8_t *s_bm, WaveStage *st,
                                                  Pending &pend, uint32_t &stores_behind, const ZmParams &zp, uint32_t blk_stride, uint32_t comb,
-                                                 uint32_t *__restrict__ blk_aux)
+                                                 uint32_t *__restrict__ blk_aux, uint32_t wrow, uint32_t wslot)
 {
     const int lane = lane_id();
     RC_PHASE_BEGIN
@@ -462,7 +465,7 @@
         pend.csize = lz4_encode_block(pend.cown, n_blk, *s_lz);
     }
     RC_PHASE(5);
-    stores_behind = flush_pending<LEVEL1, CODEC, KEEP_BITMAP>(pend, tile, n_blk, bitmap, nb_stride, pix_slots, tile_cnt, blk_slots, blk_size, s_lz, st, blk_stride, comb, blk_aux);
+    stores_behind = flush_pending<LEVEL1, CODEC, KEEP_BITMAP>(pend, tile, n_blk, bitmap, nb_stride, pix_slots, tile_cnt, blk_slots, blk_size, s_lz, st, blk_stride, comb, blk_aux, wrow, wslot);
     pend.valid = false;
     RC_PHASE(6);
 }
@@ -476,7 +479,7 @@
                                                        uint16_t *__restrict__ pix_slots, uint32_t *__restrict__ tile_cnt,
                                                        uint8_t *__restrict__ blk_slots, uint32_t *__restrict__ blk_size, uint32_t depth,
                                                        BatchStatus *__restrict__ status, ZmParams zm, uint32_t blk_stride, uint32_t comb,
-                                                       uint32_t *__restrict__ blk_aux)
+                                                       uint32_t *__restrict__ blk_aux, uint32_t wseg)
 {
     if (blockIdx.x == 0 && threadIdx.x == 0) { status->code = 0; status->frame = 0; status->total = 0; }
     __shared__ uint16_t s_code[CODEC == CODEC_ZSTD_MODELLED ? 256 : 2];
@@ -496,6 +499,7 @@
     const int w = __builtin_amdgcn_readfirstlane((int)(threadIdx.x >> 6));
     const uint32_t tile = tile0 + tblock * RWAVES + w;
     if (tile >= tile_end) return;
+    const uint32_t wrow = wseg ? 8u * wseg : ntiles, wslot = tile_word(tile, wseg ? (uint32_t)RWAVES : 0u, wseg);
     const uint64_t lane_px0 = (uint64_t)tile * TILE_PX + (uint64_t)lane * 8;
     const uint32_t f0 = grp * BZ;
     if (f0 >= B) return;
@@ -526,10 +530,21 @@
         reduce_one_frame<ALIGNED, ASMLOAD, LEVEL1, CODEC, KEEP_BITMAP, RAWVAL, SB>(xa, frames + (uint64_t)f * N, frames + (uint64_t)(f + 1) * N, nxt, t,
                                                                              lane_px0, N, full, f, tile, (uint64_t)f * ntiles + tile, n_blk,
                                                                              bitmap, nb_stride, pix_slots, tile_cnt, blk_slots,
-                                                                             blk_size, lz, bm, st, pend, stores_behind, zm, blk_stride, comb, blk_aux);
+                                                                             blk_size, lz, bm, st, pend, stores_behind, zm, blk_stride, comb, blk_aux, wrow, wslot);
         if (!nxt) break;
     }
-    flush_pending<LEVEL1, CODEC, KEEP_BITMAP>(pend, tile, n_blk, bitmap, nb_stride, pix_slots, tile_cnt, blk_slots, blk_size, lz, st, blk_stride, comb, blk_aux);
+    flush_pending<LEVEL1, CODEC, KEEP_BITMAP>(pend, tile, n_blk, bitmap, nb_stride, pix_slots, tile_cnt, blk_slots, blk_size, lz, st, blk_stride, comb, blk_aux, wrow, wslot);
+}
+
+static bool three_wave_workgroups(const Scratch &sc, bool l1, bool raw, uint32_t codec, uint32_t src_bytes)
+{
+    return src_bytes == 2 && l1 && !raw && codec != CODEC_DEFLATE &&
+           (codec == CODEC_LZ4_RUNS || codec == CODEC_LZ4_EVENTS || sc.ntiles > 8192 || (codec == CODEC_ZSTD_MODELLED && (sc.zm_valid & ZM_LITS_ONLY)));
+}
+uint32_t reduce_word_order(const Scratch &sc, uint32_t level, uint32_t codec, uint32_t src_bytes)
+{
+    if (level == 2 || src_bytes > 2) return 0u;
+    return three_wave_workgroups(sc, level == 1, false, codec, src_bytes) ? 3u : 4u;
 }
 
 template <int BZ, bool AL, bool L1, int CODEC, bool KEEP, bool RAW, int SB>
@@ -539,24 +554,25 @@
     const uint32_t nfull = AL ? (uint32_t)(sc.N / TILE_PX) : 0u;
     const ZmParams zm{reinterpret_cast<const uint16_t *>(sc.zm_lit_code), sc.zm_valid, sc.zm_budget, sc.zm_seq_bits};
     const uint32_t comb = (L1 && !RAW && CODEC) ? sc.comb : COMB_OFF;
-    const bool three = L1 && !RAW && CODEC != CODEC_DEFLATE &&
-                       (CODEC == CODEC_LZ4_RUNS || CODEC == CODEC_LZ4_EVENTS || sc.ntiles > 8192 || (CODEC == CODEC_ZSTD_MODELLED && (sc.zm_valid & ZM_LITS_ONLY)));
+    const bool three = three_wave_workgroups(sc, L1, RAW, CODEC, SB);
     auto go = [&](auto rw) {
         constexpr int RW = decltype(rw)::value;
+        assert(sc.rw == 0 || (!RAW && sc.rw == (uint32_t)RW));
+        const uint32_t wseg = sc.rw ? tile_word_seg(sc.ntiles, RW) : 0u;
         auto grid_for = [&](uint32_t nt) { return (((nt + RW - 1) / RW + 7) / 8) * 8 * ngroups; };
         if (nfull)
             hipLaunchKernelGGL((k_reduce_tiles<RW, BZ, AL, AL, L1, CODEC, KEEP, RAW, SB>), dim3(grid_for(nfull)), dim3(64 * RW), 0, s, frames, sc.thr, sc.N,
                                sc.ntiles, 0u, nfull, B, ngroups, sc.nb, sc.bitmap, sc.nb_stride, sc.pix_slots, sc.tile_cnt, sc.blk_slots,
-                               sc.blk_size, depth, sc.status, zm, sc.blk_stride, comb, sc.blk_aux);
+                               sc.blk_size, depth, sc.status, zm, sc.blk_stride, comb, sc.blk_aux, wseg);
         if (nfull < sc.ntiles) {
             if (AL && sc.N % 8 != 0)
                 hipLaunchKernelGGL((k_reduce_tiles<RW, BZ, false, false, L1, CODEC, KEEP, RAW, SB>), dim3(grid_for(sc.ntiles - nfull)), dim3(64 * RW), 0, nfull ? s_tail : s, frames,
                                    sc.thr, sc.N, sc.ntiles, nfull, sc.ntiles, B, ngroups, sc.nb, sc.bitmap, sc.nb_stride, sc.pix_slots, sc.tile_cnt,
-                                   sc.blk_slots, sc.blk_size, depth, sc.status, zm, sc.blk_stride, comb, sc.blk_aux);
+                                   sc.blk_slots, sc.blk_size, depth, sc.status, zm, sc.blk_stride, comb, sc.blk_aux, wseg);
             else
                 hipLaunchKernelGGL((k_reduce_tiles<RW, BZ, AL, false, L1, CODEC, KEEP, RAW, SB>), dim3(grid_for(sc.ntiles - nfull)), dim3(64 * RW), 0, nfull ? s_tail : s, frames,
                                    sc.thr, sc.N, sc.ntiles, nfull, sc.ntiles, B, ngroups, sc.nb, sc.bitmap, sc.nb_stride, sc.pix_slots, sc.tile_cnt,
-                                   sc.blk_slots, sc.blk_size, depth, sc.status, zm, sc.blk_stride, comb, sc.blk_aux);
+                                   sc.blk_slots, sc.blk_size, depth, sc.status, zm, sc.blk_stride, comb, sc.blk_aux, wseg);
         }
     };
     if constexpr (SB == 2) {
@@ -635,7 +651,7 @@
 
 template <int SCAN_I>
 __device__ __forceinline__ void scan_row(uint32_t *__restrict__ row, uint32_t *__restrict__ orow, uint32_t n,
-                                         uint32_t *__restrict__ total, uint32_t *sm, const uint32_t *adj = nullptr)
+                                         uint32_t *__restrict__ total, uint32_t *sm, const uint32_t *adj = nullptr, uint32_t rw = 0, uint32_t seg = 0)
 {
     uint32_t carry = 0;
     for (uint32_t t0 = 0; t0 < n; t0 += SCAN_T * SCAN_I) {
@@ -643,12 +659,13 @@
         uint32_t v[SCAN_I], s = 0;
 #pragma unroll
         for (int k = 0; k < SCAN_I; ++k) {
-            v[k] = t + k < n ? row[t + k] : 0;
+            const uint32_t wk = tile_word(t + k, rw, seg);
+            v[k] = t + k < n ? row[wk] : 0;
             if (adj) {
                 v[k] &= 0xFFFFu;
                 if (t + k == adj[0]) v[k] += adj[1];
                 if (t + k == adj[2]) v[k] += adj[3];
-                if (t + k < n) row[t + k] = v[k];
+                if (t + k < n) row[wk] = v[k];
             }
             s += v[k];
         }
@@ -666,14 +683,15 @@
 
 __device__ __forceinline__ void zstd_rewrite_defs(const uint32_t *__restrict__ row, uint8_t *__restrict__ slots, uint32_t stride,
                                                   const uint8_t *__restrict__ tree, uint32_t tl, const uint8_t *__restrict__ sdesc, uint32_t sl,
-                                                  uint32_t t_tree, uint32_t t_seq, uint32_t which, uint8_t *s_img, uint32_t *s_pos)
+                                                  uint32_t t_tree, uint32_t t_seq, uint32_t which, uint8_t *s_img, uint32_t *s_pos,
+                                                  uint32_t rw = 0, uint32_t seg = 0)
 {
     for (int pass = 0; pass < 2; ++pass) {
         const uint32_t t = pass == 0 ? t_tree : t_seq;
         if (t == 0xFFFFFFFFu || (pass == 1 && t == t_tree) || !((which >> pass) & 1u)) continue;
         const uint32_t a_tl = pass == 0 ? tl : 0u, a_sl = (pass == 1 || t_seq == t_tree) ? sl : 0u;
         uint8_t *slot = slots + (uint64_t)t * stride;
-        const uint32_t size = row[t] & 0xFFFFu;
+        const uint32_t size = row[tile_word(t, rw, seg)] & 0xFFFFu;
         __syncthreads();
         for (uint32_t i = threadIdx.x; i < (size + 3) / 4; i += blockDim.x)
             reinterpret_cast<uint32_t *>(s_img)[i] = reinterpret_cast<const uint32_t *>(slot)[i];
@@ -689,7 +707,7 @@
 
 __device__ __forceinline__ void zstd_place_defs(const uint32_t *__restrict__ row, uint32_t n, uint8_t *__restrict__ slots, uint32_t stride,
                                                 const uint8_t *__restrict__ tree, uint32_t tree_len, const uint8_t *__restrict__ sdesc,
-                                                uint32_t sdesc_len, uint32_t *adj)
+                                                uint32_t sdesc_len, uint32_t *adj, uint32_t rw = 0, uint32_t seg = 0)
 {
     __shared__ uint32_t s_first[2];
     __shared__ uint32_t s_pos;
@@ -703,7 +721,7 @@
     } else {
         uint32_t mt = 0xFFFFFFFFu, mq = 0xFFFFFFFFu;
         for (uint32_t t = threadIdx.x; t < n; t += SCAN_T) {
-            const uint32_t w = row[t];
+            const uint32_t w = row[tile_word(t, rw, seg)];
             if ((w & ZW_TREE) && t < mt) mt = t;
             if ((w & ZW_SEQ) && t < mq) mq = t;
         }
@@ -714,7 +732,7 @@
     const uint32_t t_tree = s_first[0], t_seq = s_first[1];
     const uint32_t tl = t_tree != 0xFFFFFFFFu ? tree_len : 0u, sl = t_seq != 0xFFFFFFFFu ? sdesc_len : 0u;
     if (threadIdx.x == 0) { adj[0] = t_tree; adj[1] = tl; adj[2] = t_seq; adj[3] = sl; }
-    zstd_rewrite_defs(row, slots, stride, tree, tl, sdesc, sl, t_tree, t_seq, 3u, s_img, &s_pos);
+    zstd_rewrite_defs(row, slots, stride, tree, tl, sdesc, sl, t_tree, t_seq, 3u, s_img, &s_pos, rw, seg);
 }
 
 __global__ __launch_bounds__(SCAN_T) void k_pix_scan(Scratch sc, uint32_t depth)
@@ -742,17 +760,19 @@
     __shared__ uint32_t s_adj[4];
     const uint32_t f = blockIdx.x, n = sc.ntiles;
     const uint64_t fr = (uint64_t)f * n;
+    const uint32_t rw = sc.rw, seg = rw ? tile_word_seg(n, rw) : 0u;
+    const uint64_t wr = (uint64_t)f * tile_word_row(n, rw);
     if (with_blocks) {
         if (sc.zm_model) {
             const ZstdModel *M = sc.zm_model;
-            zstd_place_defs(sc.blk_size + fr, n, sc.blk_slots + fr * sc.blk_stride, sc.blk_stride, M->lit_desc, M->lit_desc_len, M->seq_desc,
-                            M->seq_desc_len, s_adj);
-        }
-        scan_row<SCAN_I>(sc.blk_size + fr, sc.blk_off + fr, n, sc.frame_cbytes + f, sm, sc.zm_model ? s_adj : nullptr);
+            zstd_place_defs(sc.blk_size + wr, n, sc.blk_slots + fr * sc.blk_stride, sc.blk_stride, M->lit_desc, M->lit_desc_len, M->seq_desc,
+                            M->seq_desc_len, s_adj, rw, seg);
+        }
+        scan_row<SCAN_I>(sc.blk_size + wr, sc.blk_off + fr, n, sc.frame_cbytes + f, sm, sc.zm_model ? s_adj : nullptr, rw, seg);
     }
     if (!with_counts) return;
-    uint32_t *row = sc.tile_cnt + fr;
-    scan_row<SCAN_I>(row, sc.tile_off + fr, n, sc.frame_nnz + f, sm);
+    uint32_t *row = sc.tile_cnt + wr;
+    scan_row<SCAN_I>(row, sc.tile_off + fr, n, sc.frame_nnz + f, sm, nullptr, rw, seg);
     uint32_t *nrow = sc.tile_next + fr;
     if (threadIdx.x == 0) s_carry = n;
     __syncthreads();
@@ -764,7 +784,7 @@
         uint32_t first = 0xFFFFFFFFu;
 #pragma unroll
         for (int k = SCAN_I - 1; k >= 0; --k) {
-            v[k] = t + k < n ? row[t + k] : 0;
+            v[k] = t + k < n ? row[tile_word(t + k, rw, seg)] : 0;
             if (v[k]) first = t + k;
         }
         uint32_t m = first;
@@ -808,23 +828,26 @@
     __shared__ uint32_t s_min[3];
     const uint32_t seg = blockIdx.x, f = blockIdx.y, n = sc.ntiles, nseg = gridDim.x;
     const uint64_t fr = (uint64_t)f * n;
+    const uint32_t rw = sc.rw, wseg = rw ? tile_word_seg(n, rw) : 0u;
+    const uint64_t wr = (uint64_t)f * tile_word_row(n, rw);
     const uint32_t t = seg * SEG + threadIdx.x * SEG_I;
     ScanPart *part = reinterpret_cast<ScanPart *>(sc.scan_part) + (uint64_t)f * nseg + seg;
     if (threadIdx.x < 3) s_min[threadIdx.x] = 0xFFFFFFFFu;
     __syncthreads();
     uint32_t blk_sum = 0, cnt_sum = 0;
     if (with_blocks) {
-        uint32_t *row = sc.blk_size + fr, *orow = sc.blk_off + fr;
+        uint32_t *row = sc.blk_size + wr, *orow = sc.blk_off + fr;
         const bool zm = sc.zm_model != nullptr;
         uint32_t v[SEG_I], sum = 0, mt = 0xFFFFFFFFu, mq = 0xFFFFFFFFu;
 #pragma unroll
         for (int k = 0; k < SEG_I; ++k) {
-            const uint32_t w = t + k < n ? row[t + k] : 0;
+            const uint32_t wk = tile_word(t + k, rw, wseg);
+            const uint32_t w = t + k < n ? row[wk] : 0;
             if (zm) {
                 if ((w & ZW_TREE) && mt == 0xFFFFFFFFu) mt = t + k;
                 if ((w & ZW_SEQ) && mq == 0xFFFFFFFFu) mq = t + k;
                 v[k] = w & 0xFFFFu;
-                if (t + k < n) row[t + k] = v[k];
+                if (t + k < n) row[wk] = v[k];
             } else v[k] = w;
             sum += v[k];
         }
@@ -838,12 +861,12 @@
         }
     }
     if (with_counts) {
-        const uint32_t *row = sc.tile_cnt + fr;
+        const uint32_t *row = sc.tile_cnt + wr;
         uint32_t *orow = sc.tile_off + fr, *nrow = sc.tile_next + fr;
         uint32_t v[SEG_I], sum = 0, first = 0xFFFFFFFFu;
 #pragma unroll
         for (int k = SEG_I - 1; k >= 0; --k) {
-            v[k] = t + k < n ? row[t + k] : 0;
+            v[k] = t + k < n ? row[tile_word(t + k, rw, wseg)] : 0;
             if (v[k]) first = t + k;
             sum += v[k];
         }
@@ -914,10 +937,12 @@
             sl = t_seq != 0xFFFFFFFFu ? M->seq_desc_len : 0u;
             const uint32_t mine = (t_tree >= lo && t_tree < hi ? 1u : 0u) | (t_seq >= lo && t_seq < hi ? 2u : 0u);
             if (mine) {
-                zstd_rewrite_defs(sc.blk_size + fr, sc.blk_slots + fr * sc.blk_stride, sc.blk_stride, M->lit_desc, tl, M->seq_desc, sl, t_tree, t_seq, mine, s_img, &s_pos);
+                const uint32_t rw = sc.rw, wseg = rw ? tile_word_seg(n, rw) : 0u;
+                uint32_t *row = sc.blk_size + (uint64_t)f * tile_word_row(n, rw);
+                zstd_rewrite_defs(row, sc.blk_slots + fr * sc.blk_stride, sc.blk_stride, M->lit_desc, tl, M->seq_desc, sl, t_tree, t_seq, mine, s_img, &s_pos, rw, wseg);
                 if (threadIdx.x == 0) {
-                    if (mine & 1u) sc.blk_size[fr + t_tree] += tl;
-                    if (mine & 2u) sc.blk_size[fr + t_seq] += sl;
+                    if (mine & 1u) row[tile_word(t_tree, rw, wseg)] += tl;
+                    if (mine & 2u) row[tile_word(t_seq, rw, wseg)] += sl;
                 }
             }
         }
diff --git a/pyrecode_amd/csrc/rc_tile_order.h b/pyrecode_amd/csrc/rc_tile_order.h
--- /dev/null
+++ b/pyrecode_amd/csrc/rc_tile_order.h
@@ -0,0 +1,32 @@
+#pragma once
+#include <stdint.h>
+
+#if defined(__HIPCC__) || defined(__CUDACC__)
+#define RC_ORDER_HD __host__ __device__ inline
+#else
+#define RC_ORDER_HD inline
+#endif
+
+namespace rc {
+
+RC_ORDER_HD uint32_t tile_word_seg(uint32_t ntiles, uint32_t rw)
+{
+    return ((((ntiles + rw - 1) / rw + 7u) >> 3) * rw + 31u) & ~31u;
+}
+RC_ORDER_HD uint32_t tile_word_row(uint32_t ntiles, uint32_t rw)
+{
+    return rw ? 8u * tile_word_seg(ntiles, rw) : ntiles;
+}
+RC_ORDER_HD uint32_t tile_word(uint32_t tile, uint32_t rw, uint32_t seg)
+{
+    if (!rw) return tile;
+    const uint32_t tb = tile / rw;
+    return (tb & 7u) * seg + (tb >> 3) * rw + (tile - tb * rw);
+}
+RC_ORDER_HD uint32_t tile_word_row_max(uint32_t ntiles)
+{
+    const uint32_t a = tile_word_row(ntiles, 3), b = tile_word_row(ntiles, 4), m = a > b ? a : b;
+    return m > ntiles ? m : ntiles;
+}
+
+}
diff --git a/pyrecode_amd/csrc/rc_zstd.hip b/pyrecode_amd/csrc/rc_zstd.hip
--- a/pyrecode_amd/csrc/rc_zstd.hip
+++ b/pyrecode_amd/csrc/rc_zstd.hip
@@ -42,8 +42,9 @@
     __syncthreads();
     const uint32_t ft = blockIdx.x * FSE_T + threadIdx.x;
     if (ft >= nslots) return;
-    const uint32_t word = sc.blk_size[ft];
-    if (word & ZW_FINAL) { sc.blk_size[ft] = word & (0xFFFFu | ZW_TREE); return; }
+    uint32_t *size_word = sc.blk_size + tile_word_at(sc, ft / sc.ntiles, ft % sc.ntiles);
+    const uint32_t word = *size_word;
+    if (word & ZW_FINAL) { *size_word = word & (0xFFFFu | ZW_TREE); return; }
     const uint32_t P = word & 0xFFFFu, nseq = (word >> 16) & 0xFFu;
     uint32_t *slot32 = reinterpret_cast<uint32_t *>(sc.blk_slots + (uint64_t)ft * sc.blk_stride);
     const ZW4 *tok4 = reinterpret_cast<const ZW4 *>(slot32 + (zstd_token_offset(P) >> 2));
@@ -67,7 +68,7 @@
     const uint32_t content = end - 3;
     const uint32_t lastbit = (ft % sc.ntiles) + 1 == sc.ntiles ? 1u : 0u;
     slot32[0] |= lastbit | (2u << 1) | (content << 3);
-    sc.blk_size[ft] = end | (word & ZW_TREE) | (fitted ? ZW_SEQ : 0u);
+    *size_word = end | (word & ZW_TREE) | (fitted ? ZW_SEQ : 0u);
 }
 void launch_zstd_fse(const Scratch &sc, uint32_t B, const void *tables_dev, bool fitted, hipStream_t s)
 {
@@ -96,8 +97,8 @@
     const uint32_t f = blockIdx.y;
     const int lane = lane_id();
     for (uint32_t t = blockIdx.x * WAVES + (threadIdx.x >> 6); t < sc.ntiles && f < B; t += gridDim.x * WAVES) {
-        const uint64_t ft = (uint64_t)f * sc.ntiles + t;
-        const uint32_t word = sc.blk_size[ft];
+        const uint64_t ft = (uint64_t)f * sc.ntiles + t, wt = tile_word_at(sc, f, t);
+        const uint32_t word = sc.blk_size[wt];
         if (!(word & ZW_FINAL)) {
             const uint8_t *slot = sc.blk_slots + ft * sc.blk_stride;
             const uint32_t P = word & 0xFFFFu, nseq = word >> 16;
@@ -120,8 +121,8 @@
             if (lane == 0) atomicAdd(&s_h.nblk, 1u);
         }
         if (with_pix) {
-            const uint32_t nbytes = (sc.tile_cnt[ft] * depth + 7) >> 3;
-            const uint8_t *p = residual_src(sc, ft, 0u, sc.tile_cnt[ft], depth);
+            const uint32_t nbytes = (sc.tile_cnt[wt] * depth + 7) >> 3;
+            const uint8_t *p = residual_src(sc, ft, 0u, sc.tile_cnt[wt], depth);
             for (uint32_t i = lane; i < nbytes; i += 64) atomicAdd(&s_h.pix[p[i]], 1u);
         }
     }
```
